# dgaddy/silent_speech

Measured on AMD Instinct MI355X. Metric: EMG frames/s training (transduction_model.py), higher is better.
Workload: dtype bf16

## Files before the change

include/silent_speech_hip.h:

```cpp
#ifndef SILENT_SPEECH_HIP_H
#define SILENT_SPEECH_HIP_H
#include <stdint.h>
#ifdef __cplusplus
extern "C" {
#endif

#define SS_F32 0
#define SS_BF16 1
#define SS_F32X3 3

const char* ss_last_error(void);
#define SS_ABI_VERSION 10
int ss_abi_version(void);
const char* ss_target_arch(void);

typedef struct ss_rowmap {
    int64_t base;
    int64_t batch_stride;
    int64_t row_stride;
    int32_t rows_per_batch;
} ss_rowmap;

typedef struct ss_gemm_epilogue {
    const float* bias;
    const void* gate;
    float gate_scale;
    float alpha;
    int32_t relu;
    float dropout_p;
    uint64_t seed;
    uint32_t rng_stream;
    int32_t mode;
    int32_t col_mod, col_mul, col_div_mul;
    float log_clamp;
    void* c2;
    ss_rowmap cmap2;
    int64_t col_stride2;
    float* col_sum;
    float* col_sumsq;
    const float* col_shift;
    void* planes_hi;
    void* planes_lo;
    int32_t planes_only;
    void* sign_out;
    int64_t sign_pitch;
    const void* gate_bits;
    int64_t gate_bits_pitch;
} ss_gemm_epilogue;

#define SS_OP_KC 0
#define SS_OP_OC 1

int ss_gemm(int dtype_in, int dtype_out, int a_mode, int b_mode, const void* A, const void* B, void* C,
            int M, int N, int K, const ss_rowmap* amap, const ss_rowmap* bmap, const ss_rowmap* cmap,
            const ss_gemm_epilogue* epilogue, int split_k, void* stream);

int ss_split_planes(const float* x, void* hi, void* lo, int64_t n, void* stream);
int ss_gemm_planes(int dtype_out, const void* A_hi, const void* A_lo, const void* B_hi, const void* B_lo, void* C, int M, int N, int K,
                   const ss_rowmap* amap, const ss_rowmap* bmap, const ss_rowmap* cmap, const ss_gemm_epilogue* epilogue, void* stream);
int ss_gemm_sign_bits_supported(int dtype_in, int dtype_out, int a_mode, int b_mode, const void* C, int M, int N, int K, const ss_rowmap* amap,
                                const ss_rowmap* bmap, const ss_rowmap* cmap, const ss_gemm_epilogue* epilogue, int split_k);
int ss_gemm_planes_supported(int dtype_out, const void* C, int M, int N, int K, const ss_rowmap* amap, const ss_rowmap* bmap, const ss_rowmap* cmap,
                             const ss_gemm_epilogue* epilogue);

int ss_gemm_set_blocks_per_cu(int n);
int ss_gemm_last_kernel(void);
int ss_gemm_fuses_column_stats(int dtype_in, int dtype_out, int a_mode, int b_mode, const void* C, int M, int N, int K, const ss_rowmap* amap,
                               const ss_rowmap* bmap, const ss_rowmap* cmap, const ss_gemm_epilogue* epilogue, int split_k);
int ss_gemm_set_option(int what, int value);

typedef struct ss_dw_job {
    const void* A;
    const void* B;
    float* C;
    ss_rowmap amap, bmap;
    int64_t ldc;
    int32_t M, N, K;
    int32_t flags;
} ss_dw_job;
int ss_gemm_dw_grouped(int n_jobs, const ss_dw_job* jobs , void* stream);
int ss_gemm_dw_set_option(int what, int value);

int ss_permute3d(const void* in, int in_dtype, void* out, int out_dtype, int d0, int d1, int d2,
                 int64_t s0, int64_t s1, int64_t s2, int valid1, int valid2, float scale, int accumulate,
                 void* stream);

int ss_permute3d_batch(const void* jobs_dev, const int32_t* job_of_block_dev, int total_blocks, int all_f32, void* stream);

int ss_dtw_source(int n, int m, int64_t stride_i, int64_t stride_j);
int64_t ss_dtw_workspace_bytes(int n, int m, int64_t* sk_bytes, int64_t* dirs_bytes, int64_t* bnd_bytes);
int ss_dtw_align(const float* costs, const int64_t* desc_dev, int n, int max_n, int max_m, void* workspace,
                 int32_t* results, void* stream);
int ss_dtw_align_skewed(const int64_t* desc_dev, int n, void* workspace, int32_t* results, void* stream);
int ss_dtw_cumulative(int dtype, const void* costs, int64_t stride_i, int64_t stride_j, int N, int M, void* dtw_out,
                      int32_t* results, void* stream);

int64_t ss_bn_scratch_floats(int B, int T, int C);
int ss_bn_stats_sums(int dtype, const void* x, int B, int T, int C, int pad, float* scratch, const float* shift, float* sums, void* stream);
int ss_bn_finalize(const float* sums, double n_total, int C, float* mean, float* invstd, float* running_mean, float* running_var,
                   float momentum, float eps, int training, void* stream);
int ss_bn_finalize_shift(const float* sums, const float* shift, double n_total, int C, float* mean, float* invstd, float* running_mean,
                         float* running_var, float momentum, float eps, int training, void* stream);
int ss_bn_apply(int dtype, const void* xa, const float* mean_a, const float* invstd_a, const float* gamma_a, const float* beta_a, int pad_xa,
                const void* xb, const float* mean_b, const float* invstd_b, const float* gamma_b, const float* beta_b, int pad_xb,
                void* y, int pad_y, int B, int T, int C, int relu, void* stream);
int ss_bn_backward_sums(int dtype, const void* dy, int pad_dy, const void* y, int pad_y,
                        const void* xa, int pad_xa, const float* mean_a, const float* invstd_a,
                        const void* xb, int pad_xb, const float* mean_b, const float* invstd_b,
                        float* dgamma_a, float* dbeta_a, float* dgamma_b, float* dbeta_b,
                        float* scratch, float* sums, int B, int T, int C, int relu,
                        const float* gate_gamma_a, const float* gate_beta_a, const float* gate_gamma_b, const float* gate_beta_b, void* stream);
int ss_bn_backward_apply(int dtype, const void* dy, int pad_dy, const void* y, int pad_y,
                         const void* xa, int pad_xa, const float* mean_a, const float* invstd_a, const float* gamma_a,
                         const void* xb, int pad_xb, const float* mean_b, const float* invstd_b, const float* gamma_b,
                         const float* sums, double n_total, void* dxa, int pad_dxa, void* dxb, int pad_dxb,
                         int B, int T, int C, int relu, const float* gate_beta_a, const float* gate_beta_b, void* stream);
int64_t ss_colsum_scratch_floats(int rows, int C);
int ss_colsum(int dtype, const void* x, int rows, int C, int64_t ld, float* scratch, float* out_accum, void* stream);

int ss_add_dropout_layernorm_forward(int dtype, const void* x, void* branch_inout, const float* gamma, const float* beta, void* y,
                                     float* mean, float* rstd, int rows, int C, float eps, float dropout_p, uint64_t seed,
                                     uint32_t rng_stream, void* stream);
int ss_layernorm_backward(int dtype, const void* dy, const void* z, const float* mean, const float* rstd, const float* gamma,
                          void* dres, void* dbranch, float* dgamma, float* dbeta, int rows, int C, float dropout_p, uint64_t seed,
                          uint32_t rng_stream, void* stream);

int ss_layernorm_backward_bias(int dtype, const void* dy, const void* z, const float* mean, const float* rstd, const float* gamma,
                               void* dres, void* dbranch, float* dgamma, float* dbeta, float* dbranch_colsum, int rows, int C, float dropout_p,
                               uint64_t seed, uint32_t rng_stream, void* stream);
int64_t ss_layernorm_backward_scratch_floats(int rows, int C);
int ss_layernorm_backward_ws(int dtype, const void* dy, const void* z, const float* mean, const float* rstd, const float* gamma,
                             void* dres, void* dbranch, float* dgamma, float* dbeta, float* dbranch_colsum, float* scratch, int64_t scratch_floats,
                             int rows, int C, float dropout_p, uint64_t seed, uint32_t rng_stream, void* stream);
int ss_add_dropout_layernorm_forward_planes(int dtype, const void* x, void* branch_inout, const float* gamma, const float* beta, void* y, void* y_hi, void* y_lo,
                                            float* mean, float* rstd, int rows, int C, float eps, float dropout_p, uint64_t seed, uint32_t rng_stream, void* stream);
int ss_layernorm_backward_ws_planes(int dtype, const void* dy, const void* z, const float* mean, const float* rstd, const float* gamma,
                                    void* dres, void* dbranch, void* dbranch_hi, void* dbranch_lo, float* dgamma, float* dbeta, float* dbranch_colsum, float* scratch,
                                    int64_t scratch_floats, int rows, int C, float dropout_p, uint64_t seed, uint32_t rng_stream, void* stream);

int ss_emg_prepare(int dtype, const float* x_raw, void* out_padded, float* shifted_copy, int B, int T0, int Cin, int shift, void* stream);

int ss_loss_index_tables(const int64_t* utt_dev, int n_utt, int32_t* vo_pred, int32_t* vo_tgt, int32_t* si_tgt, int32_t* si_base,
                         int32_t* si_res, void* stream);
int ss_frame_lse(const float* head, int64_t ld, int col0, int ncls, int rows, float* lse, int32_t* argmax, void* stream);
int ss_voiced_loss(const float* head, int64_t ld, int n_mel, int n_phone, const float* lse, const int32_t* argmax, const float* Y,
                   const int64_t* phones, const int32_t* pred_row, const int32_t* tgt_row, int nframes, float lam, float inv_total,
                   float* dhead, float* loss_accum, int32_t* correct_accum, void* stream);
int ss_silent_cost_skewed(const float* head, int64_t ld, int n_mel, const float* lse, const float* Y, const int64_t* phones,
                          const int64_t* desc_dev, int n, int max_n, int max_m, float lam, void* workspace, int32_t* results, void* stream);
int ss_silent_loss(const float* head, int64_t ld, int n_mel, int n_phone, const float* lse, const int32_t* argmax, const float* Y,
                   const int64_t* phones, const int32_t* results, const int32_t* tgt_row, const int32_t* pred_base,
                   const int32_t* res_idx, int nframes, float lam, float inv_total, float* dhead, float* loss_accum,
                   int32_t* correct_accum, void* stream);
int ss_phoneme_confusion(const int32_t* argmax, const int64_t* phones, const int32_t* results, const int32_t* vo_pred, const int32_t* vo_tgt,
                         int n_voiced, const int32_t* si_tgt, const int32_t* si_base, const int32_t* si_res, int n_silent_frames,
                         int32_t* confusion, int n_phone, void* stream);

int ss_ctc_loss(const float* logits, int64_t ld, int V, int blank, const float* lse, const int64_t* desc_dev, int n_utt, int max_target_len,
                int64_t rows, const int32_t* targets, float* alpha_ws, float* beta_ws, float* nll, float* dlogits, float* loss, void* stream);

int ss_adamw_step(float* p, const float* g, float* m, float* v, int64_t n, float lr, float beta1, float beta2, float eps,
                  float weight_decay, int step, float grad_scale, void* stream);
int ss_cast_f32(const float* in, void* out, int out_dtype, int64_t n, void* stream);
int ss_soft_clip(const float* x, float* out, int64_t n, int C, const float* mean, const float* stdv, float pre_div, float limit, void* stream);

int ss_concat_pad(const void* table_dev, int n, void* out, int64_t total_bytes, int granule, void* stream);

int ss_reflect_pad(const float* y, float* out, int B, int L, int pad, int64_t ld_out, void* stream);
int ss_reflect_pad_ragged(const float* y, const int64_t* offsets_dev, const int32_t* lengths_dev, float* out, int B, int min_len,
                          int pad, int64_t ld_out, int clip, void* stream);
int ss_stft_magnitude(const float* spec, int64_t ld_spec, int n_bins, float* mag, int64_t ld_mag, int rows, void* stream);
int ss_stft_logmel_fft(const float* y, const int64_t* offsets_dev, const int32_t* lengths_dev, int64_t uniform_len, int B, int F, int pad, int clip,
                       int n_fft, int hop, const float* window,
                       const int32_t* band_lo, const int32_t* band_cnt, const int32_t* band_off, const float* band_w, const int32_t* lane_bands, int n_mels, int n_w,
                       float log_clamp, float* out, int64_t stride_b, int64_t stride_f, int64_t stride_m, void* stream);

int ss_relpos_attention_needs_transposed(int dtype, int T, int dp, int D);
int ss_relpos_attention_family(int dtype, int T, int dp, int D);
int64_t ss_relpos_attention_table_bytes(int H, int dp, int D);
int ss_relpos_attention_prepare_tables(const float* emb, void* tab, int H, int D, int dh, int dp, float scale, void* stream);
int ss_relpos_attention_forward(int dtype, const void* qkv, const void* qkvT, const void* E, const void* tab, void* out, float* lse,
                                int B, int H, int T, int Tp, int dp, int D, float scale, float dropout_p, uint64_t seed,
                                uint32_t rng_stream, void* stream);
int ss_relpos_attention_backward(int dtype, const void* qkv, const void* qkvT, const void* E, const void* ET, const void* tab, const void* out,
                                 const float* lse, const void* dO, const void* dOT, float* Dscratch, void* dqkv,
                                 int B, int H, int T, int Tp, int dp, int D, float scale, float dropout_p, uint64_t seed,
                                 uint32_t rng_stream, void* stream);

int64_t ss_relpos_attention_saved_bytes(int dtype, int B, int H, int T, int dp, int D);
int ss_relpos_attention_forward_p(int dtype, const void* qkv, const void* qkvT, const void* E, const void* tab, void* out, float* lse, void* pimg,
                                  int B, int H, int T, int Tp, int dp, int D, float scale, float dropout_p, uint64_t seed,
                                  uint32_t rng_stream, void* stream);
int ss_relpos_attention_backward_p(int dtype, const void* qkv, const void* qkvT, const void* E, const void* ET, const void* tab, const void* out,
                                   const float* lse, const void* dO, const void* dOT, float* Dscratch, void* dqkv, const void* pimg,
                                   int B, int H, int T, int Tp, int dp, int D, float scale, float dropout_p, uint64_t seed,
                                   uint32_t rng_stream, void* stream);

int ss_relpos_attention_x3_supported(int T, int dp, int D);
int64_t ss_relpos_attention_x3_saved_bytes(int B, int H, int T, int dp, int D);
int64_t ss_relpos_attention_x3_table_bytes(int H, int dp, int D);
int ss_relpos_attention_x3_prepare_tables(const float* emb, void* tab, int H, int D, int dh, int dp, float scale, void* stream);
int ss_relpos_attention_x3_forward(const void* qkv_hi, const void* qkv_lo, const void* tab, void* out_hi, void* out_lo, float* lse, void* pimg,
                                   int B, int H, int T, int dp, int D, float scale, float dropout_p, uint64_t seed, uint32_t rng_stream, void* stream);
int ss_relpos_attention_x3_backward(const void* qkv_hi, const void* qkv_lo, const void* tab, const void* out_hi, const void* out_lo, const void* dO_hi, const void* dO_lo,
                                    float* Dscratch, void* dqkv_hi, void* dqkv_lo, const void* pimg,
                                    int B, int H, int T, int dp, int D, float scale, float dropout_p, uint64_t seed, uint32_t rng_stream, void* stream);

int64_t ss_iir_filtfilt_workspace_bytes(int T, int C, int max_padlen);
int ss_iir_filtfilt(const double* x, double* y, int T, int C, int n_filt, const double* coef, void* workspace, int64_t workspace_bytes, void* stream);
int ss_linear_resample(const double* x, double* y, int T, int C, double old_freq, double new_freq, int T_out, void* stream);
int64_t ss_iir_filtfilt_batch_workspace_bytes(const int32_t* lengths_host, int R, int C, int max_padlen, int n_filt);
int ss_iir_filtfilt_batch(const double* x, double* y, const int32_t* lengths_host, int R, int C, int n_filt, const double* coef,
                          void* workspace, int64_t workspace_bytes, void* stream);
int ss_linear_resample_batch(const double* x, double* y, const int64_t* table_dev, int R, int C, double old_freq, double new_freq,
                             int64_t total_out_rows, void* stream);
int ss_emg_features_batch(const double* x, float* out, const int64_t* table_dev, int R, int C, int64_t total_frames, void* stream);

typedef struct ss_model_dims {
    int32_t d_model, n_layers, n_head, d_qkv, dp , max_rel , ff;
    int32_t n_head_cols , dtype;
    float ln_eps;
} ss_model_dims;
typedef struct ss_plan ss_plan;
typedef double (*ss_reduce_hook)(void* user, float* sums_dev, int n_floats, double n_local, void* stream);
typedef void (*ss_event_hook)(void* user, int what, void* stream);
ss_plan* ss_plan_create(const ss_model_dims* dims);
void ss_plan_destroy(ss_plan* plan);
int ss_plan_slot_count(const ss_plan* plan);
const char* ss_plan_slot_name(const ss_plan* plan, int slot);
int ss_plan_bind(ss_plan* plan, int slot, void* device_ptr_or_value);
int ss_plan_set_option(ss_plan* plan, int what, int value);
int ss_plan_set_reduce_hook(ss_plan* plan, ss_reduce_hook fn, void* user);
int ss_plan_set_event_hook(ss_plan* plan, ss_event_hook fn, void* user);
int64_t ss_plan_ctx_bytes(void);
int64_t ss_plan_workspace_bytes(ss_plan* plan, int B, int T0, int training);
int ss_plan_forward(ss_plan* plan, const float* x_raw, float* shifted_scratch, void* workspace, int64_t workspace_bytes, int B, int T0,
                    int training, int shift_r, float dropout_p, uint64_t seed, float* head, void* ctx_out, void* stream);
int ss_plan_backward(ss_plan* plan, void* ctx, const float* dhead, void* stream, void* side_stream);
typedef struct ss_profile_row { char name[64]; int64_t calls; double seconds, flops , bytes ; } ss_profile_row;
int ss_plan_profile(ss_plan* plan, int enable);
int ss_plan_profile_read(ss_plan* plan, ss_profile_row* rows, int max_rows);
int ss_counters_add(int n, int64_t** counters , int64_t delta, void* stream);

#ifdef __cplusplus
}
#endif
#endif
```

silent_speech_amd/_lib.py:

```python
import ctypes
import os

import torch

_HERE = os.path.dirname(os.path.abspath(__file__))
_LIB_PATH = os.environ.get('SS_AMD_LIBRARY') or os.path.join(_HERE, 'lib', 'libsilent_speech_hip.so')

SS_F32, SS_BF16, SS_F64, SS_F32X3 = 0, 1, 2, 3
ABI_VERSION = 10
OP_KC, OP_OC = 0, 1


class RowMap(ctypes.Structure):
    _fields_ = [('base', ctypes.c_int64), ('batch_stride', ctypes.c_int64), ('row_stride', ctypes.c_int64),
                ('rows_per_batch', ctypes.c_int32)]


class GemmEpilogue(ctypes.Structure):
    _fields_ = [('bias', ctypes.c_void_p), ('gate', ctypes.c_void_p), ('gate_scale', ctypes.c_float),
                ('alpha', ctypes.c_float), ('relu', ctypes.c_int32), ('dropout_p', ctypes.c_float),
                ('seed', ctypes.c_uint64), ('rng_stream', ctypes.c_uint32), ('mode', ctypes.c_int32),
                ('col_mod', ctypes.c_int32), ('col_mul', ctypes.c_int32), ('col_div_mul', ctypes.c_int32),
                ('log_clamp', ctypes.c_float), ('c2', ctypes.c_void_p), ('cmap2', RowMap), ('col_stride2', ctypes.c_int64),
                ('col_sum', ctypes.c_void_p), ('col_sumsq', ctypes.c_void_p), ('col_shift', ctypes.c_void_p),
                ('planes_hi', ctypes.c_void_p), ('planes_lo', ctypes.c_void_p), ('planes_only', ctypes.c_int32),
                ('sign_out', ctypes.c_void_p), ('sign_pitch', ctypes.c_int64), ('gate_bits', ctypes.c_void_p), ('gate_bits_pitch', ctypes.c_int64)]


class DwJob(ctypes.Structure):
    _fields_ = [('A', ctypes.c_void_p), ('B', ctypes.c_void_p), ('C', ctypes.c_void_p), ('amap', RowMap), ('bmap', RowMap),
                ('ldc', ctypes.c_int64), ('M', ctypes.c_int32), ('N', ctypes.c_int32), ('K', ctypes.c_int32), ('flags', ctypes.c_int32)]


class ProfileRow(ctypes.Structure):
    _fields_ = [('name', ctypes.c_char * 64), ('calls', ctypes.c_int64), ('seconds', ctypes.c_double), ('flops', ctypes.c_double), ('bytes', ctypes.c_double)]


class PermuteJob(ctypes.Structure):
    _fields_ = [('inp', ctypes.c_void_p), ('out', ctypes.c_void_p), ('s0', ctypes.c_int64), ('s1', ctypes.c_int64), ('s2', ctypes.c_int64),
                ('o0', ctypes.c_int64), ('o1', ctypes.c_int64), ('d0', ctypes.c_int32), ('d1', ctypes.c_int32), ('d2', ctypes.c_int32),
                ('valid1', ctypes.c_int32), ('valid2', ctypes.c_int32), ('in_dtype', ctypes.c_int32), ('out_dtype', ctypes.c_int32),
                ('accumulate', ctypes.c_int32), ('scale', ctypes.c_float), ('first_block', ctypes.c_int32), ('nblocks', ctypes.c_int32),
                ('pad_', ctypes.c_int32)]


_P, _I, _F, _L = ctypes.c_void_p, ctypes.c_int, ctypes.c_float, ctypes.c_int64
_U64, _U32 = ctypes.c_uint64, ctypes.c_uint32

SIGNATURES = {
    'ss_gemm': [_I, _I, _I, _I, _P, _P, _P, _I, _I, _I, ctypes.POINTER(RowMap), ctypes.POINTER(RowMap),
                ctypes.POINTER(RowMap), ctypes.POINTER(GemmEpilogue), _I, _P],
    'ss_gemm_dw_grouped': [_I, ctypes.POINTER(DwJob), _P],
    'ss_split_planes': [_P, _P, _P, _L, _P],
    'ss_gemm_planes': [_I, _P, _P, _P, _P, _P, _I, _I, _I, ctypes.POINTER(RowMap), ctypes.POINTER(RowMap), ctypes.POINTER(RowMap), ctypes.POINTER(GemmEpilogue), _P],
    'ss_permute3d': [_P, _I, _P, _I, _I, _I, _I, _L, _L, _L, _I, _I, _F, _I, _P],
    'ss_permute3d_batch': [_P, _P, _I, _I, _P],
    'ss_dtw_align': [_P, _P, _I, _I, _I, _P, _P, _P],
    'ss_dtw_align_skewed': [_P, _I, _P, _P, _P],
    'ss_reflect_pad_ragged': [_P, _P, _P, _P, _I, _I, _I, _L, _I, _P],
    'ss_concat_pad': [_P, _I, _P, _L, _I, _P],
    'ss_dtw_cumulative': [_I, _P, _L, _L, _I, _I, _P, _P, _P],
    'ss_relpos_attention_forward': [_I, _P, _P, _P, _P, _P, _P, _I, _I, _I, _I, _I, _I, _F, _F, _U64, _U32, _P],
    'ss_relpos_attention_backward': [_I, _P, _P, _P, _P, _P, _P, _P, _P, _P, _P, _P, _I, _I, _I, _I, _I, _I, _F, _F, _U64, _U32, _P],
    'ss_relpos_attention_forward_p': [_I, _P, _P, _P, _P, _P, _P, _P, _I, _I, _I, _I, _I, _I, _F, _F, _U64, _U32, _P],
    'ss_relpos_attention_backward_p': [_I, _P, _P, _P, _P, _P, _P, _P, _P, _P, _P, _P, _P, _I, _I, _I, _I, _I, _I, _F, _F, _U64, _U32, _P],
    'ss_relpos_attention_prepare_tables': [_P, _P, _I, _I, _I, _I, _F, _P],
    'ss_relpos_attention_x3_prepare_tables': [_P, _P, _I, _I, _I, _I, _F, _P],
    'ss_relpos_attention_x3_forward': [_P, _P, _P, _P, _P, _P, _P, _I, _I, _I, _I, _I, _F, _F, _U64, _U32, _P],
    'ss_relpos_attention_x3_backward': [_P, _P, _P, _P, _P, _P, _P, _P, _P, _P, _P, _I, _I, _I, _I, _I, _F, _F, _U64, _U32, _P],
    'ss_bn_stats_sums': [_I, _P, _I, _I, _I, _I, _P, _P, _P, _P],
    'ss_bn_finalize': [_P, ctypes.c_double, _I, _P, _P, _P, _P, _F, _F, _I, _P],
    'ss_bn_finalize_shift': [_P, _P, ctypes.c_double, _I, _P, _P, _P, _P, _F, _F, _I, _P],
    'ss_bn_apply': [_I, _P, _P, _P, _P, _P, _I, _P, _P, _P, _P, _P, _I, _P, _I, _I, _I, _I, _I, _P],
    'ss_bn_backward_sums': [_I, _P, _I, _P, _I, _P, _I, _P, _P, _P, _I, _P, _P, _P, _P, _P, _P, _P, _P, _I, _I, _I, _I, _P, _P, _P, _P, _P],
    'ss_bn_backward_apply': [_I, _P, _I, _P, _I, _P, _I, _P, _P, _P, _P, _I, _P, _P, _P, _P, ctypes.c_double, _P, _I, _P, _I, _I, _I, _I, _I, _P, _P, _P],
    'ss_colsum': [_I, _P, _I, _I, _L, _P, _P, _P],
    'ss_add_dropout_layernorm_forward': [_I, _P, _P, _P, _P, _P, _P, _P, _I, _I, _F, _F, _U64, _U32, _P],
    'ss_add_dropout_layernorm_forward_planes': [_I, _P, _P, _P, _P, _P, _P, _P, _P, _P, _I, _I, _F, _F, _U64, _U32, _P],
    'ss_layernorm_backward': [_I, _P, _P, _P, _P, _P, _P, _P, _P, _P, _I, _I, _F, _U64, _U32, _P],
    'ss_layernorm_backward_bias': [_I, _P, _P, _P, _P, _P, _P, _P, _P, _P, _P, _I, _I, _F, _U64, _U32, _P],
    'ss_layernorm_backward_ws': [_I, _P, _P, _P, _P, _P, _P, _P, _P, _P, _P, _P, _L, _I, _I, _F, _U64, _U32, _P],
    'ss_layernorm_backward_ws_planes': [_I, _P, _P, _P, _P, _P, _P, _P, _P, _P, _P, _P, _P, _P, _L, _I, _I, _F, _U64, _U32, _P],
    'ss_emg_prepare': [_I, _P, _P, _P, _I, _I, _I, _I, _P],
    'ss_frame_lse': [_P, _L, _I, _I, _I, _P, _P, _P],
    'ss_loss_index_tables': [_P, _I, _P, _P, _P, _P, _P, _P],
    'ss_voiced_loss': [_P, _L, _I, _I, _P, _P, _P, _P, _P, _P, _I, _F, _F, _P, _P, _P, _P],
    'ss_silent_cost_skewed': [_P, _L, _I, _P, _P, _P, _P, _I, _I, _I, _F, _P, _P, _P],
    'ss_silent_loss': [_P, _L, _I, _I, _P, _P, _P, _P, _P, _P, _P, _P, _I, _F, _F, _P, _P, _P, _P],
    'ss_phoneme_confusion': [_P, _P, _P, _P, _P, _I, _P, _P, _P, _I, _P, _I, _P],
    'ss_ctc_loss': [_P, _L, _I, _I, _P, _P, _I, _I, _L, _P, _P, _P, _P, _P, _P, _P],
    'ss_adamw_step': [_P, _P, _P, _P, _L, _F, _F, _F, _F, _F, _I, _F, _P],
    'ss_cast_f32': [_P, _P, _I, _L, _P],
    'ss_soft_clip': [_P, _P, _L, _I, _P, _P, _F, _F, _P],
    'ss_reflect_pad': [_P, _P, _I, _I, _I, _L, _P],
    'ss_iir_filtfilt': [_P, _P, _I, _I, _I, _P, _P, _L, _P],
    'ss_linear_resample': [_P, _P, _I, _I, ctypes.c_double, ctypes.c_double, _I, _P],
    'ss_iir_filtfilt_batch': [_P, _P, _P, _I, _I, _I, _P, _P, _L, _P],
    'ss_linear_resample_batch': [_P, _P, _P, _I, _I, ctypes.c_double, ctypes.c_double, _L, _P],
    'ss_emg_features_batch': [_P, _P, _P, _I, _I, _L, _P],
    'ss_stft_magnitude': [_P, _L, _I, _P, _L, _I, _P],
    'ss_stft_logmel_fft': [_P, _P, _P, _L, _I, _I, _I, _I, _I, _I, _P, _P, _P, _P, _P, _P, _I, _I, _F, _P, _L, _L, _L, _P],
}
_LP = ctypes.POINTER(ctypes.c_int64)
_HOST_FUNCS = {'ss_dtw_workspace_bytes': ([_I, _I, _LP, _LP, _LP], ctypes.c_int64),
               'ss_dtw_source': ([_I, _I, _L, _L], ctypes.c_int),
               'ss_bn_scratch_floats': ([_I, _I, _I], ctypes.c_int64),
               'ss_iir_filtfilt_workspace_bytes': ([_I, _I, _I], ctypes.c_int64),
               'ss_iir_filtfilt_batch_workspace_bytes': ([_P, _I, _I, _I, _I], ctypes.c_int64),
               'ss_colsum_scratch_floats': ([_I, _I], ctypes.c_int64),
               'ss_gemm_set_blocks_per_cu': ([_I], ctypes.c_int),
               'ss_gemm_last_kernel': ([], ctypes.c_int),
               'ss_gemm_set_option': ([_I, _I], ctypes.c_int),
               'ss_gemm_fuses_column_stats': ([_I, _I, _I, _I, _P, _I, _I, _I, ctypes.POINTER(RowMap), ctypes.POINTER(RowMap), ctypes.POINTER(RowMap),
                                               ctypes.POINTER(GemmEpilogue), _I], ctypes.c_int),
               'ss_gemm_sign_bits_supported': ([_I, _I, _I, _I, _P, _I, _I, _I, ctypes.POINTER(RowMap), ctypes.POINTER(RowMap), ctypes.POINTER(RowMap),
                                                ctypes.POINTER(GemmEpilogue), _I], ctypes.c_int),
               'ss_gemm_planes_supported': ([_I, _P, _I, _I, _I, ctypes.POINTER(RowMap), ctypes.POINTER(RowMap), ctypes.POINTER(RowMap), ctypes.POINTER(GemmEpilogue)], ctypes.c_int),
               'ss_gemm_dw_set_option': ([_I, _I], ctypes.c_int),
               'ss_plan_create': ([_P], _P), 'ss_plan_destroy': ([_P], None), 'ss_plan_slot_count': ([_P], ctypes.c_int),
               'ss_plan_slot_name': ([_P, _I], ctypes.c_char_p), 'ss_plan_bind': ([_P, _I, _P], ctypes.c_int),
               'ss_plan_set_option': ([_P, _I, _I], ctypes.c_int), 'ss_plan_set_reduce_hook': ([_P, _P, _P], ctypes.c_int),
               'ss_plan_set_event_hook': ([_P, _P, _P], ctypes.c_int), 'ss_plan_ctx_bytes': ([], ctypes.c_int64),
               'ss_plan_workspace_bytes': ([_P, _I, _I, _I], ctypes.c_int64),
               'ss_plan_forward': ([_P, _P, _P, _P, _L, _I, _I, _I, _I, _F, _U64, _P, _P, _P], ctypes.c_int),
               'ss_plan_backward': ([_P, _P, _P, _P, _P], ctypes.c_int),
               'ss_counters_add': ([_I, _P, _L, _P], ctypes.c_int),
               'ss_plan_profile': ([_P, _I], ctypes.c_int), 'ss_plan_profile_read': ([_P, _P, _I], ctypes.c_int),
               'ss_relpos_attention_needs_transposed': ([_I, _I, _I, _I], ctypes.c_int),
               'ss_relpos_attention_family': ([_I, _I, _I, _I], ctypes.c_int),
               'ss_relpos_attention_table_bytes': ([_I, _I, _I], ctypes.c_int64),
               'ss_relpos_attention_x3_supported': ([_I, _I, _I], ctypes.c_int),
               'ss_relpos_attention_x3_saved_bytes': ([_I, _I, _I, _I, _I], ctypes.c_int64),
               'ss_relpos_attention_x3_table_bytes': ([_I, _I, _I], ctypes.c_int64),
               'ss_relpos_attention_saved_bytes': ([_I, _I, _I, _I, _I, _I], ctypes.c_int64),
               'ss_layernorm_backward_scratch_floats': ([_I, _I], ctypes.c_int64)}
_RESTYPES = {'ss_last_error': ctypes.c_char_p, 'ss_target_arch': ctypes.c_char_p, 'ss_abi_version': ctypes.c_int}

_lib = None
_is_emulator = False


def _declare(lib):
    for name, restype in _RESTYPES.items():
        fn = getattr(lib, name)
        fn.restype = restype
        fn.argtypes = []
    for name, argtypes in SIGNATURES.items():
        fn = getattr(lib, name)
        fn.argtypes = argtypes
        fn.restype = ctypes.c_int
    for name, (argtypes, restype) in _HOST_FUNCS.items():
        fn = getattr(lib, name)
        fn.argtypes = argtypes
        fn.restype = restype
    return lib


def load(path=None, _testing=False):
    global _lib, _is_emulator
    path = path or _LIB_PATH
    if not os.path.exists(path):
        raise RuntimeError('silent_speech_amd: %s not found -- build the gfx950 kernels first '
                           '(python -c "import __graft_entry__ as g; g.build()" or make -C silent_speech_amd/csrc). '
                           'There is no CPU fallback.' % path)
    cdll = ctypes.CDLL(path)
    cdll.ss_abi_version.restype = ctypes.c_int
    have = cdll.ss_abi_version()
    if have != ABI_VERSION:
        raise RuntimeError('silent_speech_amd: %s has ABI version %d, this binding needs %d -- rebuild it '
                           '(make -C silent_speech_amd/csrc); struct layouts differ between versions' % (path, have, ABI_VERSION))
    cdll.ss_target_arch.restype = ctypes.c_char_p
    arch = cdll.ss_target_arch()
    if arch != b'gfx950' and not _testing:
        raise RuntimeError('silent_speech_amd: %s targets %r, not gfx950 -- the package only loads the MI355X build '
                           '(SS_AMD_LIBRARY selects between gfx950 builds; the emulator library is for tests/ only)' % (path, arch))
    _lib = _declare(cdll)
    _is_emulator = arch != b'gfx950'
    return _lib


def use_library_for_testing(path):
    return load(path, _testing=True)


def lib():
    if _lib is None:
        load()
    return _lib


def is_emulator():
    lib()
    return _is_emulator


def kernels_can_read(t):
    return bool(t.is_cuda) != is_emulator()


def kernel_device_for(t):
    return t.device if kernels_can_read(t) else torch.device('cuda')


def check(rc, what=''):
    if rc != 0:
        raise RuntimeError('%s failed: %s' % (what or 'silent_speech_hip call', lib().ss_last_error().decode()))


def dtype_code(dt):
    if dt == torch.float32:
        return SS_F32
    if dt == torch.bfloat16:
        return SS_BF16
    if dt == torch.float64:
        return SS_F64
    raise TypeError('unsupported dtype %s (float32, bfloat16; float64 for ss_dtw_cumulative only)' % dt)


def ptr(t):
    if t is None:
        return None
    if not kernels_can_read(t):
        if is_emulator():
            raise RuntimeError('emulator backend (tests only) needs CPU tensors')
        raise RuntimeError('silent_speech_amd: tensor is on %s; the HIP kernels need an AMD GPU tensor '
                           '(no CPU fallback exists)' % t.device)
# ... 8 lines not shown
```

silent_speech_amd/csrc/norm.hip:

```cpp
#include "common.h"
#include <stdlib.h>
#include "silent_speech_hip.h"

namespace {
struct Seq {
    int T, pad;
    __device__ __forceinline__ long long row(int r) const { int b = r / T, t = r - b * T; return (long long)b * (T + 2 * pad) + pad + t; }
    __device__ __forceinline__ long long at(int b, int t) const { return (long long)b * (T + 2 * pad) + pad + t; }
};

__device__ __forceinline__ void ld8(const float* __restrict__ p, float (&v)[8]) {
    const f32x4 a = *(const f32x4*)p, b = *(const f32x4*)(p + 4);
    v[0] = a[0]; v[1] = a[1]; v[2] = a[2]; v[3] = a[3]; v[4] = b[0]; v[5] = b[1]; v[6] = b[2]; v[7] = b[3];
}

struct ColMap {
    int CV, CVb, RY, cx0, ry; bool active;
    __device__ __forceinline__ ColMap(int C, int tid, int nthreads) {
        CV = C >> 3; CVb = CV < nthreads ? CV : nthreads; RY = nthreads / CVb;
        cx0 = tid % CVb; ry = tid / CVb; active = ry < RY;
    }
};
constexpr int RED_THREADS = 256;

template <int NQ>
__device__ __forceinline__ bool chunk_reduce(const float* __restrict__ partial, int nchunks, int C, float (&out)[NQ], int& c_out)
{
    __shared__ float red[NQ][8][32];
    const int cl = threadIdx.x & 31, ln = threadIdx.x >> 5, c = blockIdx.x * 32 + cl;
    float acc[NQ];
#pragma unroll
    for (int q = 0; q < NQ; ++q) acc[q] = 0.f;
    if (c < C) {
        int k = ln;
        for (; k + 56 < nchunks; k += 64) {
            float v[8][NQ];
#pragma unroll
            for (int u = 0; u < 8; ++u)
#pragma unroll
                for (int q = 0; q < NQ; ++q) v[u][q] = partial[((long long)(k + 8 * u) * NQ + q) * C + c];
#pragma unroll
            for (int u = 0; u < 8; ++u)
#pragma unroll
                for (int q = 0; q < NQ; ++q) acc[q] += v[u][q];
        }
        for (; k < nchunks; k += 8)
#pragma unroll
            for (int q = 0; q < NQ; ++q) acc[q] += partial[((long long)k * NQ + q) * C + c];
    }
#pragma unroll
    for (int q = 0; q < NQ; ++q) red[q][ln][cl] = acc[q];
    __syncthreads();
    c_out = c;
    if (ln != 0 || c >= C) return false;
#pragma unroll
    for (int q = 0; q < NQ; ++q) { float t = 0.f; for (int y = 0; y < 8; ++y) t += red[q][y][cl]; out[q] = t; }
    return true;
}
}

template <class T>
__global__ __launch_bounds__(RED_THREADS) void bn_partial_kernel(const T* __restrict__ x, Seq sx, int rows, int C, int rows_per_chunk, const float* __restrict__ shift, float* __restrict__ partial)
{
    __shared__ float red[2][RED_THREADS * 8];
    ColMap m(C, threadIdx.x, (int)blockDim.x);
    const int r0 = blockIdx.x * rows_per_chunk, r1 = min(rows, r0 + rows_per_chunk);
    for (int cb = 0; cb < m.CV; cb += m.CVb) {
        const int cx = cb + m.cx0;
        float s1[8], s2[8], sh[8];
#pragma unroll
        for (int e = 0; e < 8; ++e) { s1[e] = 0.f; s2[e] = 0.f; sh[e] = 0.f; }
        const bool cv = m.active && cx < m.CV;
        if (cv) {
            if (shift) {
#pragma unroll
                for (int e = 0; e < 8; ++e) sh[e] = shift[cx * 8 + e];
            } else Vec8<T>::load(x + sx.row(0) * C + cx * 8, sh);
            int r = r0 + m.ry;
            for (; r + 3 * m.RY < r1; r += 4 * m.RY) {
                float v[4][8];
#pragma unroll
                for (int u = 0; u < 4; ++u) Vec8<T>::load(x + sx.row(r + u * m.RY) * C + cx * 8, v[u]);
#pragma unroll
                for (int u = 0; u < 4; ++u)
#pragma unroll
                    for (int e = 0; e < 8; ++e) { float d = v[u][e] - sh[e]; s1[e] += d; s2[e] += d * d; }
            }
            for (; r < r1; r += m.RY) {
                float v[8]; Vec8<T>::load(x + sx.row(r) * C + cx * 8, v);
#pragma unroll
                for (int e = 0; e < 8; ++e) { float d = v[e] - sh[e]; s1[e] += d; s2[e] += d * d; }
            }
        }
        __syncthreads();
#pragma unroll
        for (int e = 0; e < 8; ++e) { red[0][threadIdx.x * 8 + e] = s1[e]; red[1][threadIdx.x * 8 + e] = s2[e]; }
        __syncthreads();
        if (cv && m.ry == 0) {
            for (int y = 1; y < m.RY; ++y)
#pragma unroll
                for (int e = 0; e < 8; ++e) { s1[e] += red[0][(y * m.CVb + m.cx0) * 8 + e]; s2[e] += red[1][(y * m.CVb + m.cx0) * 8 + e]; }
#pragma unroll
            for (int e = 0; e < 8; ++e) {
                partial[((long long)blockIdx.x * 2 + 0) * C + cx * 8 + e] = s1[e];
                partial[((long long)blockIdx.x * 2 + 1) * C + cx * 8 + e] = s2[e];
            }
        }
    }
}

template <class T>
__global__ __launch_bounds__(256) void bn_sums_kernel(const T* __restrict__ x, Seq sx, const float* __restrict__ partial, int nchunks, int C, const float* __restrict__ shift, float* __restrict__ sums)
{
    float t[2]; int c;
    if (!chunk_reduce<2>(partial, nchunks, C, t, c)) return;
    sums[c] = t[0]; sums[C + c] = t[1]; sums[2 * C + c] = shift ? shift[c] : ldf(x + sx.row(0) * C + c);
}

__global__ void bn_finalize_kernel(const float* __restrict__ sums, const float* shift, float n, int C, float* mean, float* invstd, float* running_mean, float* running_var,
                                   float momentum, float eps, int training)
{
    const int c = blockIdx.x * blockDim.x + threadIdx.x;
    if (c >= C) return;
    if (!training) { mean[c] = running_mean[c]; invstd[c] = rsqrtf(running_var[c] + eps); return; }
    const float d = sums[c] / n, mu = (shift ? shift[c] : sums[2 * C + c]) + d;
    float var = sums[C + c] / n - d * d; var = var < 0.f ? 0.f : var;
    mean[c] = mu; invstd[c] = rsqrtf(var + eps);
    if (running_mean) {
        running_mean[c] = (1.f - momentum) * running_mean[c] + momentum * mu;
        running_var[c] = (1.f - momentum) * running_var[c] + momentum * var * (n > 1.f ? n / (n - 1.f) : 1.f);
    }
}

static int red_threads(int C) {
    static const int forced = getenv("SS_BN_RED_THREADS") ? atoi(getenv("SS_BN_RED_THREADS")) : 0;
    if (forced > 0) return forced < RED_THREADS ? forced : RED_THREADS;
    const int cv = C >> 3;
    if (cv >= RED_THREADS || cv <= 0) return RED_THREADS;
    const int t = RED_THREADS / cv * cv;
    return t >= 64 ? t : RED_THREADS;
}
static int red_chunks(int rows) { static const int cap = getenv("SS_BN_CHUNKS") ? atoi(getenv("SS_BN_CHUNKS")) : 768; int c = (rows + 63) / 64; if (c > cap) c = cap; if (c < 1) c = 1; return c; }

extern "C" int64_t ss_bn_scratch_floats(int B, int T, int C) { return (int64_t)red_chunks(B * T) * 4 * C + 8 * (int64_t)C; }

extern "C" int ss_bn_stats_sums(int dtype, const void* x, int B, int T, int C, int pad, float* scratch, const float* shift, float* sums, void* stream)
{
    SS_CHECK(x && scratch && sums, "ss_bn_stats_sums: null pointer");
    SS_CHECK(C % 8 == 0 && C > 0, "ss_bn_stats_sums: C=%d must be a positive multiple of 8", C);
    SS_CHECK(B > 0 && T > 0, "ss_bn_stats_sums: empty batch");
    const int rows = B * T, nch = red_chunks(rows), rpc = (rows + nch - 1) / nch;
    Seq sx = {T, pad};
    if (dtype == SS_BF16) {
        SS_LAUNCH(bn_partial_kernel<bf16_t>, dim3(nch), dim3(red_threads(C)), 0, stream, (const bf16_t*)x, sx, rows, C, rpc, shift, scratch);
        SS_LAUNCH(bn_sums_kernel<bf16_t>, dim3((C + 31) / 32), dim3(256), 0, stream, (const bf16_t*)x, sx, (const float*)scratch, nch, C, shift, sums);
    } else {
        SS_LAUNCH(bn_partial_kernel<float>, dim3(nch), dim3(red_threads(C)), 0, stream, (const float*)x, sx, rows, C, rpc, shift, scratch);
        SS_LAUNCH(bn_sums_kernel<float>, dim3((C + 31) / 32), dim3(256), 0, stream, (const float*)x, sx, (const float*)scratch, nch, C, shift, sums);
    }
    SS_LAUNCH_CHECK("ss_bn_stats_sums");
    return 0;
}

extern "C" int ss_bn_finalize(const float* sums, double n_total, int C, float* mean, float* invstd, float* running_mean, float* running_var,
                              float momentum, float eps, int training, void* stream)
{
    SS_CHECK(mean && invstd && C > 0, "ss_bn_finalize: null pointer");
    SS_CHECK(training ? (sums != nullptr && n_total >= 1.0) : (running_mean && running_var), "ss_bn_finalize: missing sums (training) or running statistics (eval)");
    SS_LAUNCH(bn_finalize_kernel, dim3((C + 255) / 256), dim3(256), 0, stream, sums, (const float*)nullptr, (float)n_total, C, mean, invstd, running_mean, running_var, momentum, eps, training);
    SS_LAUNCH_CHECK("ss_bn_finalize");
    return 0;
}
extern "C" int ss_bn_finalize_shift(const float* sums, const float* shift, double n_total, int C, float* mean, float* invstd, float* running_mean, float* running_var,
                                    float momentum, float eps, int training, void* stream)
{
    SS_CHECK(mean && invstd && C > 0, "ss_bn_finalize_shift: null pointer");
    SS_CHECK(training ? (sums != nullptr && shift != nullptr && n_total >= 1.0) : (running_mean && running_var), "ss_bn_finalize_shift: missing sums / shift (training) or running statistics (eval)");
    SS_LAUNCH(bn_finalize_kernel, dim3((C + 255) / 256), dim3(256), 0, stream, sums, shift, (float)n_total, C, mean, invstd, running_mean, running_var, momentum, eps, training);
    SS_LAUNCH_CHECK("ss_bn_finalize_shift");
    return 0;
}

struct RowWalk {
    unsigned ro, b, tp, rstep, db, dtp, TP; int cx;
    __device__ __forceinline__ RowWalk(unsigned gtid, unsigned step, unsigned CV, unsigned TP_) {
        TP = TP_; ro = gtid / CV; cx = (int)(gtid - ro * CV); rstep = step / CV;
        b = ro / TP; tp = ro - b * TP; db = rstep / TP; dtp = rstep - db * TP;
    }
    __device__ __forceinline__ void next() { ro += rstep; b += db; tp += dtp; if (tp >= TP) { tp -= TP; ++b; } }
};

template <class T>
__global__ void bn_apply_kernel(const T* __restrict__ xa, Seq sa, const float* __restrict__ mean_a, const float* __restrict__ invstd_a, const float* __restrict__ gamma_a, const float* __restrict__ beta_a,
                                const T* __restrict__ xb, Seq sb, const float* __restrict__ mean_b, const float* __restrict__ invstd_b, const float* __restrict__ gamma_b, const float* __restrict__ beta_b,
                                T* __restrict__ y, Seq sy, int B, int C, int relu)
{
    const int CV = C >> 3, TT = sy.T;
    const unsigned TP = (unsigned)(TT + 2 * sy.pad), rows_out = (unsigned)B * TP, step32 = gridDim.x * blockDim.x;
    if (step32 % (unsigned)CV == 0) {
        RowWalk w(blockIdx.x * blockDim.x + threadIdx.x, step32, (unsigned)CV, TP);
        float ma[8], sca[8], ba[8], mb[8], scb[8], bb[8];
#pragma unroll
        for (int e = 0; e < 8; ++e) { mb[e] = 0.f; scb[e] = 0.f; bb[e] = 0.f; }
        {
            float t[8];
            ld8(mean_a + w.cx * 8, ma); ld8(gamma_a + w.cx * 8, sca); ld8(invstd_a + w.cx * 8, t); ld8(beta_a + w.cx * 8, ba);
#pragma unroll
            for (int e = 0; e < 8; ++e) sca[e] *= t[e];
            if (xb) {
                ld8(mean_b + w.cx * 8, mb); ld8(gamma_b + w.cx * 8, scb); ld8(invstd_b + w.cx * 8, t); ld8(beta_b + w.cx * 8, bb);
#pragma unroll
                for (int e = 0; e < 8; ++e) scb[e] *= t[e];
            }
        }
        typedef typename RawVec8<T>::type Raw;
        Raw nv = RawVec8<T>::zero(), nu = RawVec8<T>::zero();
        auto fetch = [&](unsigned b, unsigned tp) {
            const int t = (int)tp - sy.pad;
            if (t >= 0 && t < TT) {
                nv = RawVec8<T>::load(xa + sa.at((int)b, t) * C + w.cx * 8);
                if (xb) nu = RawVec8<T>::load(xb + sb.at((int)b, t) * C + w.cx * 8);
            }
        };
        if (w.ro < rows_out) fetch(w.b, w.tp);
        for (; w.ro < rows_out; w.next()) {
            const int t = (int)w.tp - sy.pad;
            const Raw cv = nv, cu = nu;
            {
                unsigned nb = w.b + w.db, ntp = w.tp + w.dtp;
                if (ntp >= w.TP) { ntp -= w.TP; ++nb; }
                if (w.ro + w.rstep < rows_out) fetch(nb, ntp);
            }
            float o[8];
#pragma unroll
            for (int e = 0; e < 8; ++e) o[e] = 0.f;
            if (t >= 0 && t < TT) {
                float v[8], u[8];
                RawVec8<T>::unpack(cv, v);
                if (xb) RawVec8<T>::unpack(cu, u);
#pragma unroll
                for (int e = 0; e < 8; ++e) o[e] = (v[e] - ma[e]) * sca[e] + ba[e];
                if (xb) {
#pragma unroll
                    for (int e = 0; e < 8; ++e) o[e] += (u[e] - mb[e]) * scb[e] + bb[e];
                }
                if (relu) {
#pragma unroll
                    for (int e = 0; e < 8; ++e) o[e] = fmaxf(o[e], 0.f);
                }
            }
            Vec8<T>::store(y + (long long)w.ro * C + w.cx * 8, o);
        }
        return;
    }
    const unsigned total32 = rows_out * (unsigned)CV;
    for (unsigned i = blockIdx.x * blockDim.x + threadIdx.x; i < total32; i += step32) {
        const unsigned ro = i / (unsigned)CV; const int cx = (int)(i - ro * (unsigned)CV);
        const unsigned bq = ro / TP; const int b = (int)bq, tp = (int)(ro - bq * TP), t = tp - sy.pad;
        float o[8];
        if (t < 0 || t >= TT) {
#pragma unroll
            for (int e = 0; e < 8; ++e) o[e] = 0.f;
        } else {
            float v[8]; Vec8<T>::load(xa + sa.at(b, t) * C + cx * 8, v);
#pragma unroll
            for (int e = 0; e < 8; ++e) { const int c = cx * 8 + e; const float s = gamma_a[c] * invstd_a[c]; o[e] = (v[e] - mean_a[c]) * s + beta_a[c]; }
            if (xb) {
                float u[8]; Vec8<T>::load(xb + sb.at(b, t) * C + cx * 8, u);
#pragma unroll
                for (int e = 0; e < 8; ++e) { const int c = cx * 8 + e; const float s = gamma_b[c] * invstd_b[c]; o[e] += (u[e] - mean_b[c]) * s + beta_b[c]; }
            }
            if (relu) {
#pragma unroll
                for (int e = 0; e < 8; ++e) o[e] = fmaxf(o[e], 0.f);
            }
        }
        Vec8<T>::store(y + (long long)ro * C + cx * 8, o);
    }
}

static dim3 ew_grid(long long total, int block, int CV = 0) {
    static const long long cap_cols = getenv("SS_BN_GRID") ? atoll(getenv("SS_BN_GRID")) : 768;
    long long g = (total + block - 1) / block;
    const long long cap = CV > 0 ? cap_cols : 8192;
    if (g > cap) g = cap;
    if (g < 1) g = 1;
    if (CV > 0) {
        long long a = CV, bb = block; while (bb) { const long long t = a % bb; a = bb; bb = t; }
        const long long m = CV / a;
        if (g >= 4 * m) g = g / m * m;
    }
    return dim3((unsigned)g);
}

extern "C" int ss_bn_apply(int dtype, const void* xa, const float* mean_a, const float* invstd_a, const float* gamma_a, const float* beta_a, int pad_xa,
                           const void* xb, const float* mean_b, const float* invstd_b, const float* gamma_b, const float* beta_b, int pad_xb,
                           void* y, int pad_y, int B, int T, int C, int relu, void* stream)
{
    SS_CHECK(xa && mean_a && invstd_a && gamma_a && beta_a && y, "ss_bn_apply: null pointer");
    SS_CHECK(!xb || (mean_b && invstd_b && gamma_b && beta_b), "ss_bn_apply: second branch incomplete");
    SS_CHECK(C % 8 == 0 && C > 0 && B > 0 && T > 0, "ss_bn_apply: bad shape B=%d T=%d C=%d", B, T, C);
    Seq sa = {T, pad_xa}, sb = {T, pad_xb}, sy = {T, pad_y};
    const long long total = (long long)B * (T + 2 * pad_y) * (C / 8);
    SS_CHECK(total < (1LL << 31) - (1LL << 22), "ss_bn_apply: tensor too large for 32-bit chunk indices");
    if (dtype == SS_BF16) SS_LAUNCH(bn_apply_kernel<bf16_t>, ew_grid(total, 256, C / 8), dim3(256), 0, stream, (const bf16_t*)xa, sa, mean_a, invstd_a, gamma_a, beta_a, (const bf16_t*)xb, sb, mean_b, invstd_b, gamma_b, beta_b, (bf16_t*)y, sy, B, C, relu);
    else SS_LAUNCH(bn_apply_kernel<float>, ew_grid(total, 256, C / 8), dim3(256), 0, stream, (const float*)xa, sa, mean_a, invstd_a, gamma_a, beta_a, (const float*)xb, sb, mean_b, invstd_b, gamma_b, beta_b, (float*)y, sy, B, C, relu);
    SS_LAUNCH_CHECK("ss_bn_apply");
    return 0;
}

template <class T, bool REGATE>
__global__ __launch_bounds__(RED_THREADS, sizeof(T) == 2 ? 3 : 2) void bn_bwd_partial_kernel(const T* __restrict__ dy, Seq sdy, const T* __restrict__ y, Seq sy,
                                                                     const T* __restrict__ xa, Seq sa, const float* __restrict__ mean_a, const float* __restrict__ invstd_a,
                                                                     const T* __restrict__ xb, Seq sb, const float* __restrict__ mean_b, const float* __restrict__ invstd_b,
                                                                     const float* __restrict__ gamma_a, const float* __restrict__ beta_a, const float* __restrict__ gamma_b, const float* __restrict__ beta_b,
                                                                     int rows, int C, int rows_per_chunk, int relu, float* __restrict__ partial)
{
    __shared__ float red[3][RED_THREADS * 8];
    ColMap m(C, threadIdx.x, (int)blockDim.x);
    const int r0 = blockIdx.x * rows_per_chunk, r1 = min(rows, r0 + rows_per_chunk);
    for (int cb = 0; cb < m.CV; cb += m.CVb) {
        const int cx = cb + m.cx0;
        float sg[8], sga[8], sgb[8], ma[8], ka[8], mb[8], kb[8], bs[8];
#pragma unroll
        for (int e = 0; e < 8; ++e) { sg[e] = sga[e] = sgb[e] = 0.f; ma[e] = ka[e] = mb[e] = kb[e] = bs[e] = 0.f; }
        const bool cv = m.active && cx < m.CV;
        if (cv) {
            {
                float t0[8], t1[8], t2[8], t3[8];
                ld8(mean_a + cx * 8, ma); ld8(invstd_a + cx * 8, ka);
                ld8((xb ? mean_b : mean_a) + cx * 8, mb); ld8((xb ? invstd_b : invstd_a) + cx * 8, kb);
                if (REGATE) {
                    ld8(gamma_a + cx * 8, t0); ld8(beta_a + cx * 8, t1); ld8((xb ? gamma_b : gamma_a) + cx * 8, t2); ld8((xb ? beta_b : beta_a) + cx * 8, t3);
#pragma unroll
                    for (int e = 0; e < 8; ++e) { ka[e] *= t0[e]; kb[e] *= t2[e]; bs[e] = t1[e] + (xb ? t3[e] : 0.f); }
                }
                if (!xb) {
#pragma unroll
                    for (int e = 0; e < 8; ++e) { mb[e] = 0.f; kb[e] = 0.f; }
                }
            }
            typedef typename RawVec8<T>::type Raw;
            Raw ng[2], no[2], na[2], nb[2];
            auto fetch = [&](int r, Raw (&fg)[2], Raw (&fo)[2], Raw (&fa)[2], Raw (&fb)[2]) {
                const int rc0 = r < r1 ? r : r1 - 1, rc1 = r + m.RY < r1 ? r + m.RY : r1 - 1;
                const int b0 = rc0 / sdy.T, t0 = rc0 - b0 * sdy.T, b1 = rc1 / sdy.T, t1 = rc1 - b1 * sdy.T;
                fg[0] = RawVec8<T>::load(dy + sdy.at(b0, t0) * C + cx * 8); fg[1] = RawVec8<T>::load(dy + sdy.at(b1, t1) * C + cx * 8);
                if (relu && !REGATE) { fo[0] = RawVec8<T>::load(y + sy.at(b0, t0) * C + cx * 8); fo[1] = RawVec8<T>::load(y + sy.at(b1, t1) * C + cx * 8); }
                fa[0] = RawVec8<T>::load(xa + sa.at(b0, t0) * C + cx * 8); fa[1] = RawVec8<T>::load(xa + sa.at(b1, t1) * C + cx * 8);
                if (xb) { fb[0] = RawVec8<T>::load(xb + sb.at(b0, t0) * C + cx * 8); fb[1] = RawVec8<T>::load(xb + sb.at(b1, t1) * C + cx * 8); }
            };
            if (r0 + m.ry < r1) fetch(r0 + m.ry, ng, no, na, nb);
            for (int r = r0 + m.ry; r < r1; r += 2 * m.RY) {
                const bool two = r + m.RY < r1;
                Raw cg[2] = {ng[0], ng[1]}, co[2] = {no[0], no[1]}, ca[2] = {na[0], na[1]}, cb[2] = {nb[0], nb[1]};
                if (r + 2 * m.RY < r1) fetch(r + 2 * m.RY, ng, no, na, nb);
#pragma unroll
                for (int u = 0; u < 2; ++u) {
                    if (u == 1 && !two) break;
                    float g[8], o[8], va[8], vb[8];
                    RawVec8<T>::unpack(cg[u], g); RawVec8<T>::unpack(ca[u], va);
                    if (relu && !REGATE) RawVec8<T>::unpack(co[u], o);
                    if (xb) RawVec8<T>::unpack(cb[u], vb);
#pragma unroll
                    for (int e = 0; e < 8; ++e) {
                        if (REGATE) {
                            const float da = va[e] - ma[e], db = xb ? vb[e] - mb[e] : 0.f;
                            const float gg = (!relu || da * ka[e] + db * kb[e] + bs[e] > 0.f) ? g[e] : 0.f;
                            sg[e] += gg; sga[e] += gg * da;
                            if (xb) sgb[e] += gg * db;
                        } else {
                            const float gg = (!relu || o[e] > 0.f) ? g[e] : 0.f;
                            sg[e] += gg; sga[e] += gg * (va[e] - ma[e]) * ka[e];
                            if (xb) sgb[e] += gg * (vb[e] - mb[e]) * kb[e];
                        }
                    }
                }
            }
            if (REGATE) {
                float ia[8], ib[8];
                ld8(invstd_a + cx * 8, ia); ld8((xb ? invstd_b : invstd_a) + cx * 8, ib);
#pragma unroll
                for (int e = 0; e < 8; ++e) { sga[e] *= ia[e]; sgb[e] *= ib[e]; }
            }
        }
        __syncthreads();
#pragma unroll
        for (int e = 0; e < 8; ++e) { red[0][threadIdx.x * 8 + e] = sg[e]; red[1][threadIdx.x * 8 + e] = sga[e]; red[2][threadIdx.x * 8 + e] = sgb[e]; }
        __syncthreads();
        if (cv && m.ry == 0) {
            for (int yy = 1; yy < m.RY; ++yy)
#pragma unroll
                for (int e = 0; e < 8; ++e) { const int o = (yy * m.CVb + m.cx0) * 8 + e; sg[e] += red[0][o]; sga[e] += red[1][o]; sgb[e] += red[2][o]; }
            Vec8<float>::store(partial + ((long long)blockIdx.x * 3 + 0) * C + cx * 8, sg);
            Vec8<float>::store(partial + ((long long)blockIdx.x * 3 + 1) * C + cx * 8, sga);
            Vec8<float>::store(partial + ((long long)blockIdx.x * 3 + 2) * C + cx * 8, sgb);
        }
    }
}

__global__ __launch_bounds__(256) void bn_bwd_finalize_kernel(const float* __restrict__ partial, int nchunks, int C, float* __restrict__ coef ,
                                                              float* dgamma_a, float* dbeta_a, float* dgamma_b, float* dbeta_b)
{
    float t[3]; int c;
    if (!chunk_reduce<3>(partial, nchunks, C, t, c)) return;
    coef[c] = t[0]; coef[C + c] = t[1]; coef[2 * C + c] = t[2];
    if (dgamma_a) dgamma_a[c] += t[1];
    if (dbeta_a) dbeta_a[c] += t[0];
    if (dgamma_b) dgamma_b[c] += t[2];
    if (dbeta_b) dbeta_b[c] += t[0];
}

template <class T, bool REGATE>
__global__ void bn_bwd_apply_kernel(const T* __restrict__ dy, Seq sdy, const T* __restrict__ y, Seq sy,
                                    const T* __restrict__ xa, Seq sa, const float* __restrict__ mean_a, const float* __restrict__ invstd_a, const float* __restrict__ gamma_a,
                                    const T* __restrict__ xb, Seq sb, const float* __restrict__ mean_b, const float* __restrict__ invstd_b, const float* __restrict__ gamma_b,
                                    const float* __restrict__ coef, float inv_n, T* __restrict__ dxa, Seq sda, T* __restrict__ dxb, Seq sdb, int B, int C, int relu,
                                    const float* __restrict__ beta_a, const float* __restrict__ beta_b)
{
    constexpr bool regate = REGATE;
    const int CV = C >> 3, TT = sdy.T;
    const int padmax = sda.pad > sdb.pad ? sda.pad : sdb.pad;
    const long long total = (long long)B * (TT + 2 * padmax) * CV;
    const unsigned TP = (unsigned)(TT + 2 * padmax), total32 = (unsigned)total, step32 = gridDim.x * blockDim.x;
    if (step32 % (unsigned)CV == 0) {
        RowWalk w(blockIdx.x * blockDim.x + threadIdx.x, step32, (unsigned)CV, TP);
        float ma[8], ka[8], qa[8], c0[8], mb[8], kb[8], qb[8], bs[8];
#pragma unroll
        for (int e = 0; e < 8; ++e) { mb[e] = 0.f; kb[e] = 0.f; qb[e] = 0.f; bs[e] = 0.f; }
        {
            float ia[8], t[8];
            ld8(mean_a + w.cx * 8, ma); ld8(gamma_a + w.cx * 8, ka); ld8(invstd_a + w.cx * 8, ia); ld8(coef + C + w.cx * 8, qa); ld8(coef + w.cx * 8, c0);
            if (regate) ld8(beta_a + w.cx * 8, bs);
#pragma unroll
            for (int e = 0; e < 8; ++e) { ka[e] *= ia[e]; qa[e] = ia[e] * (qa[e] * inv_n); c0[e] *= inv_n; }
            if (xb) {
                ld8(mean_b + w.cx * 8, mb); ld8(gamma_b + w.cx * 8, kb); ld8(invstd_b + w.cx * 8, ia); ld8(coef + 2 * C + w.cx * 8, qb);
#pragma unroll
                for (int e = 0; e < 8; ++e) { kb[e] *= ia[e]; qb[e] = ia[e] * (qb[e] * inv_n); }
                if (regate) {
                    ld8(beta_b + w.cx * 8, t);
#pragma unroll
                    for (int e = 0; e < 8; ++e) bs[e] += t[e];
                }
            }
        }
        const unsigned rows_out = (unsigned)B * TP;
        for (; w.ro < rows_out; w.next()) {
            const int b = (int)w.b, t = (int)w.tp - padmax, cx = w.cx;
            float oa[8], ob[8];
#pragma unroll
            for (int e = 0; e < 8; ++e) { oa[e] = 0.f; ob[e] = 0.f; }
            if (t >= 0 && t < TT) {
                float g[8], o[8], v[8], u[8];
                Vec8<T>::load(dy + sdy.at(b, t) * C + cx * 8, g);
                if (relu && !regate) Vec8<T>::load(y + sy.at(b, t) * C + cx * 8, o);
                Vec8<T>::load(xa + sa.at(b, t) * C + cx * 8, v);
                if (xb) Vec8<T>::load(xb + sb.at(b, t) * C + cx * 8, u);
                if (regate) {
#pragma unroll
// ... 635 lines not shown
```

silent_speech_amd/csrc/plan.hip:

```cpp
#include "common.h"
#include "silent_speech_hip.h"
#include <math.h>
#include <stdlib.h>
#include <string>
#include <vector>

namespace {

struct BnP { float *gamma = 0, *beta = 0, *rmean = 0, *rvar = 0, *dgamma = 0, *dbeta = 0; long long* nbt = 0; };
struct PermB { void* jobs = 0; void* blocks = 0; long long total = 0, all_f32 = 0; };
struct BlockP {
    void *w1f = 0, *w2f = 0, *wr = 0, *wrT = 0, *w2b = 0, *w1b_even = 0, *w1b_odd = 0;
    float *b1 = 0, *br = 0, *b2 = 0;
    BnP bn1, bn2, bnr;
    float *c2_stage = 0, *c1_stage = 0, *wr_grad = 0;
    PermB unpack;
    int O = 0, I = 0;
};
struct LayerP {
    void *wqkv = 0, *wqkvT = 0, *wo = 0, *woT = 0, *E = 0, *ET = 0, *EF = 0, *w1 = 0, *w2 = 0, *w1T = 0, *w2T = 0;
    float *b1 = 0, *b2 = 0, *g1 = 0, *be1 = 0, *g2 = 0, *be2 = 0;
    float *dg1 = 0, *dbe1 = 0, *dg2 = 0, *dbe2 = 0, *dw1 = 0, *db1 = 0, *dw2 = 0, *db2 = 0, *wo_stage = 0, *wqkv_stage = 0;
    PermB unpack;
};

struct BlockCtx { void *xin, *c1, *cr, *h1, *c2, *y; float *m1, *i1, *m2, *i2, *mr, *ir, *scratch; int Tin, Cin, Tout, O, pad_y; };
struct LayerCtx { void *x, *qkv, *qkvT, *o, *z1, *y1, *hid, *z2, *pimg; float *lse, *mean1, *rstd1, *mean2, *rstd2; unsigned char* hid_sign; };
constexpr int MAX_LAYERS = 16;
constexpr int MAX_PLANES = 384;
struct PlaneCache { int n; const void* key[MAX_PLANES]; void* hi[MAX_PLANES]; long long elems[MAX_PLANES]; };
struct Ctx {
    int B, T0, T, M, Tp, need_T, n_layers;
    float p_drop, scale; unsigned long long seed;
    BlockCtx blk[3];
    LayerCtx layer[MAX_LAYERS];
    void *conv_out, *x_final;
    PlaneCache planes;
    unsigned long long ws_used;
    char* ws; unsigned long long ws_bytes;
};

struct Exec {
    bool dry; char* base; size_t off, cap; void* stream; void* side;
    void* alloc(size_t bytes) { off = (off + 255) & ~(size_t)255; char* p = base + off; off += bytes; return p; }
};

static ss_rowmap RM(long long row_stride, int rows_per_batch = 0, long long batch_stride = 0, long long base = 0) {
    ss_rowmap m; m.base = base; m.batch_stride = batch_stride; m.row_stride = row_stride; m.rows_per_batch = rows_per_batch; return m;
}
static ss_gemm_epilogue EPI() { ss_gemm_epilogue e; memset(&e, 0, sizeof(e)); e.alpha = 1.f; e.gate_scale = 1.f; return e; }
static int round_up(int x, int m) { return (x + m - 1) / m * m; }

typedef double (*reduce_fn)(void* user, float* sums, int n_floats, double n_local, void* stream);
typedef void (*event_fn)(void* user, int what, void* stream);

struct Plan {
    ss_model_dims D;
    std::vector<std::string> names; std::vector<void**> targets;
    BlockP blk[3]; std::vector<LayerP> layers;
    void *w_raw_in = 0, *w_raw_in_T = 0, *w_head = 0, *w_head_T = 0;
    float *b_raw_in = 0, *dw_raw_in = 0, *db_raw_in = 0, *b_head = 0, *head_w_stage = 0, *head_b_stage = 0, *stage_arena = 0;
    long long stage_arena_bytes = 0;
    PermB unpack_enc, unpack_all;
    reduce_fn hook = 0; void* hook_user = 0;
    event_fn on_event = 0; void* event_user = 0;
    int side_enabled = 1, dw_grouped = 1, side_blocks = 2, fuse_stats = 1, regate_on = 1, f32_x3 = 0;
    int x3_attn = 0;
    int sign_gate = 1;
    int x3_emit = 1;
    int x3_planes = 1;
    Ctx* cur = nullptr;
    bool use_planes() const { return D.dtype == SS_F32 && f32_x3 && x3_planes; }
    bool use_x3_attention(int T) const { return use_planes() && x3_attn && dw_grouped && ss_relpos_attention_x3_supported(T, D.dp, D.max_rel); }
    void adopt_planes(const void* key, void* hi, long long n) {
        PlaneCache& pc = cur->planes;
        if (key && pc.n < MAX_PLANES) { pc.key[pc.n] = key; pc.hi[pc.n] = hi; pc.elems[pc.n] = n; ++pc.n; }
    }
    int keep_input = 0;
    hipEvent_t ev_fork = 0, ev_join = 0;
    size_t esz() const { return D.dtype == SS_BF16 ? 2 : 4; }

    struct ProfRec { const char* tag; int sub; double flops, bytes; hipEvent_t e0, e1; };
    bool profiling = false;
    std::vector<ProfRec> recs; std::vector<hipEvent_t> ev_pool; size_t ev_used = 0;
    hipEvent_t prof_event() {
#if !defined(SS_EMU)
        if (ev_used == ev_pool.size()) { hipEvent_t e; hipEventCreate(&e); ev_pool.push_back(e); }
        return ev_pool[ev_used++];
#else
        return 0;
#endif
    }
    template <class F>
    int timed(Exec& X, const char* tag, double flops, double bytes, void* stream, F&& f, bool gemm_sub = false) {
        if (X.dry) return f();
#if !defined(SS_EMU)
        if (profiling) {
            ProfRec r{tag, 0, flops, bytes, prof_event(), prof_event()};
            hipEventRecord(r.e0, (hipStream_t)stream);
            const int rc = f();
            hipEventRecord(r.e1, (hipStream_t)stream);
            if (gemm_sub) r.sub = ss_gemm_last_kernel();
            recs.push_back(r);
            return rc;
        }
#endif
        return f();
    }

    void slot(const std::string& n, void** t) { names.push_back(n); targets.push_back(t); }
    void slot_bn(const std::string& p, BnP& b) {
        slot(p + ".weight", (void**)&b.gamma); slot(p + ".bias", (void**)&b.beta); slot(p + ".running_mean", (void**)&b.rmean); slot(p + ".running_var", (void**)&b.rvar);
        slot(p + ".weight.grad", (void**)&b.dgamma); slot(p + ".bias.grad", (void**)&b.dbeta); slot(p + ".num_batches_tracked", (void**)&b.nbt);
    }
    void slot_perm(const std::string& p, PermB& b) { slot(p + ".jobs", &b.jobs); slot(p + ".blocks", &b.blocks); slot(p + ".total", (void**)&b.total); slot(p + ".all_f32", (void**)&b.all_f32); }

    explicit Plan(const ss_model_dims& d) : D(d), layers(d.n_layers) {
        for (int i = 0; i < 3; ++i) {
            const std::string p = "conv_blocks." + std::to_string(i) + ".";
            BlockP& b = blk[i];
            b.O = D.d_model; b.I = i == 0 ? 8 : D.d_model;
            slot(p + "w1f", &b.w1f); slot(p + "w2f", &b.w2f); slot(p + "wr", &b.wr); slot(p + "wrT", &b.wrT); slot(p + "w2b", &b.w2b);
            if (i > 0) { slot(p + "w1b_even", &b.w1b_even); slot(p + "w1b_odd", &b.w1b_odd); }
            slot(p + "conv1.bias", (void**)&b.b1); slot(p + "residual_path.bias", (void**)&b.br); slot(p + "conv2.bias", (void**)&b.b2);
            slot_bn(p + "bn1", b.bn1); slot_bn(p + "bn2", b.bn2); slot_bn(p + "res_norm", b.bnr);
            slot(p + "conv2.weight.stage", (void**)&b.c2_stage); slot(p + "conv1.weight.stage", (void**)&b.c1_stage); slot(p + "residual_path.weight.grad", (void**)&b.wr_grad);
            slot_perm(p + "unpack", b.unpack);
        }
        slot("w_raw_in", &w_raw_in); slot("w_raw_in_T", &w_raw_in_T); slot("w_raw_in.bias", (void**)&b_raw_in);
        slot("w_raw_in.weight.grad", (void**)&dw_raw_in); slot("w_raw_in.bias.grad", (void**)&db_raw_in);
        for (int l = 0; l < D.n_layers; ++l) {
            const std::string p = "transformer.layers." + std::to_string(l) + ".";
            LayerP& L = layers[l];
            slot(p + "wqkv", &L.wqkv); slot(p + "wqkvT", &L.wqkvT); slot(p + "wo", &L.wo); slot(p + "woT", &L.woT); slot(p + "E", &L.E); slot(p + "ET", &L.ET); slot(p + "EF", &L.EF);
            slot(p + "w1", &L.w1); slot(p + "w2", &L.w2); slot(p + "w1T", &L.w1T); slot(p + "w2T", &L.w2T);
            slot(p + "linear1.bias", (void**)&L.b1); slot(p + "linear2.bias", (void**)&L.b2);
            slot(p + "norm1.weight", (void**)&L.g1); slot(p + "norm1.bias", (void**)&L.be1); slot(p + "norm2.weight", (void**)&L.g2); slot(p + "norm2.bias", (void**)&L.be2);
            slot(p + "norm1.weight.grad", (void**)&L.dg1); slot(p + "norm1.bias.grad", (void**)&L.dbe1); slot(p + "norm2.weight.grad", (void**)&L.dg2); slot(p + "norm2.bias.grad", (void**)&L.dbe2);
            slot(p + "linear1.weight.grad", (void**)&L.dw1); slot(p + "linear1.bias.grad", (void**)&L.db1); slot(p + "linear2.weight.grad", (void**)&L.dw2); slot(p + "linear2.bias.grad", (void**)&L.db2);
            slot(p + "w_o.stage", (void**)&L.wo_stage); slot(p + "w_qkv.stage", (void**)&L.wqkv_stage);
            slot_perm(p + "unpack", L.unpack);
        }
        slot("w_head", &w_head); slot("w_head_T", &w_head_T); slot("b_head", (void**)&b_head);
        slot("head_w.stage", (void**)&head_w_stage); slot("head_b.stage", (void**)&head_b_stage);
        slot("stage_arena", (void**)&stage_arena); slot("stage_arena.bytes", (void**)&stage_arena_bytes);
        slot_perm("unpack_encoder", unpack_enc); slot_perm("unpack_encoder_all", unpack_all);
    }

    static long long extent(const ss_rowmap& m, int rows, int row_len) {
        const long long nb = m.rows_per_batch > 0 ? (rows - 1) / m.rows_per_batch : 0, rr = m.rows_per_batch > 0 ? (rows < m.rows_per_batch ? rows : m.rows_per_batch) - 1 : rows - 1;
        return m.base + nb * m.batch_stride + rr * m.row_stride + row_len;
    }
    struct Pl { void* hi; void* lo; };
    Pl new_planes(Exec& X, const void* key, long long n) {
        if (!(use_planes() && x3_emit)) return Pl{nullptr, nullptr};
        n = (n + 7) & ~7LL;
        void* hi = X.alloc((size_t)n * 4);
        adopt_planes(key, hi, n);
        return Pl{hi, (char*)hi + n * 2};
    }
    Pl planes(Exec& X, const void* key, const void* src, long long n) {
        PlaneCache& pc = cur->planes;
        if (key) for (int i = 0; i < pc.n; ++i) if (pc.key[i] == key && pc.elems[i] >= n) return Pl{pc.hi[i], (char*)pc.hi[i] + pc.elems[i] * 2};
        n = (n + 7) & ~7LL;
        void* hi = X.alloc((size_t)n * 4);
        if (key && pc.n < MAX_PLANES) { pc.key[pc.n] = key; pc.hi[pc.n] = hi; pc.elems[pc.n] = n; ++pc.n; }
        if (!X.dry) {
            if (timed(X, "split_planes", 0, (double)n * 8, X.stream, [&] { return ss_split_planes((const float*)src, hi, (char*)hi + n * 2, n, X.stream); })) return Pl{nullptr, nullptr};
        }
        return Pl{hi, (char*)hi + n * 2};
    }

    int gemm(Exec& X, int dt_out, const void* A, const void* B, void* C, int M, int N, int K, ss_rowmap am, ss_rowmap bm, ss_rowmap cm, const ss_gemm_epilogue* e = 0,
             int a_mode = SS_OP_KC, int b_mode = SS_OP_KC, int split = 1, void* stream = 0, const void* wkey = nullptr, int emit = 0) {
        void* st = stream ? stream : X.stream;
        if (use_planes() && st == X.stream && a_mode == SS_OP_KC && b_mode == SS_OP_KC && dt_out == SS_F32 && split == 1 &&
            ss_gemm_planes_supported(SS_F32, C, M, N, K, &am, &bm, &cm, e)) {
            const Pl a = planes(X, A, A, extent(am, M, K)), b = planes(X, wkey ? wkey : B, B, extent(bm, N, K));
            ss_gemm_epilogue ee = e ? *e : EPI();
            if (emit && x3_emit) {
                const long long n = (extent(cm, M, N) + 7) & ~7LL;
                void* hi = X.alloc((size_t)n * 4);
                adopt_planes(C, hi, n);
                ee.planes_hi = hi; ee.planes_lo = (char*)hi + n * 2; ee.planes_only = emit == 2;
            }
            if (X.dry) return 0;
            if (!a.hi || !b.hi) return 1;
            return timed(X, "gemm", 2.0 * M * N * K, ((double)M * K + (double)N * K) * 4 + (double)M * N * 4.0, st,
                         [&] { return ss_gemm_planes(SS_F32, a.hi, a.lo, b.hi, b.lo, C, M, N, K, &am, &bm, &cm, &ee, st); }, true);
        }
        if (X.dry) return 0;
        const double ob = dt_out == SS_BF16 ? 2.0 : 4.0;
        return timed(X, a_mode == SS_OP_OC && b_mode == SS_OP_OC ? "gemm_dw" : "gemm", 2.0 * M * N * K, ((double)M * K + (double)N * K) * esz() + (double)M * N * ob, st,
                     [&] { return ss_gemm(D.dtype == SS_F32 && f32_x3 ? SS_F32X3 : D.dtype, dt_out, a_mode, b_mode, A, B, C, M, N, K, &am, &bm, &cm, e, split, st); }, true);
    }
    int colsum(Exec& X, const void* x, int rows, int C, float* out, void* stream) {
        float* scratch = (float*)X.alloc((size_t)ss_colsum_scratch_floats(rows, C) * 4);
        if (X.dry) return 0;
        return timed(X, "colsum", 0, (double)rows * C * esz(), stream, [&] { return ss_colsum(D.dtype, x, rows, C, C, scratch, out, stream); });
    }
    int permute_batch(Exec& X, const PermB& b, void* stream) {
        if (X.dry || !b.jobs || b.total <= 0) return 0;
        return timed(X, "grad_unlayout", 0, 0, stream, [&] { return ss_permute3d_batch(b.jobs, (const int32_t*)b.blocks, (int)b.total, (int)b.all_f32, stream); });
    }
    int bn_stats(Exec& X, const void* x, int B, int T, int C, float* scratch, BnP& bn, bool training, float** mean, float** invstd, float* fused = nullptr, double reduced_n = 0.0) {
        *mean = (float*)X.alloc((size_t)C * 4); *invstd = (float*)X.alloc((size_t)C * 4);
        float* sums = (training && !fused) ? (float*)X.alloc((size_t)3 * C * 4) : fused;
        if (X.dry) return 0;
        double n_total = (double)B * T;
        if (training) {
            if (!fused && timed(X, "bn_stats", 0, (double)B * T * C * esz(), X.stream, [&] { return ss_bn_stats_sums(D.dtype, x, B, T, C, 0, scratch, hook ? bn.rmean : nullptr, sums, X.stream); })) return 1;
            if (reduced_n > 0.0) n_total = reduced_n;
            else if (hook) n_total = hook(hook_user, sums, 2 * C, n_total, X.stream);
        }
        if (fused) return timed(X, "bn_finalize", 0, 0, X.stream, [&] { return ss_bn_finalize_shift(sums, bn.rmean, n_total, C, *mean, *invstd, bn.rmean, bn.rvar, 0.1f, 1e-5f, 1, X.stream); });
        return timed(X, "bn_finalize", 0, 0, X.stream, [&] { return ss_bn_finalize(sums, n_total, C, *mean, *invstd, bn.rmean, bn.rvar, 0.1f, 1e-5f, training ? 1 : 0, X.stream); });
    }
    float* conv_gemm(Exec& X, const void* A, const void* Bw, void* C, int M, int N, int K, ss_rowmap am, ss_rowmap bm, const float* bias, BnP& bn, float* stat_slot, int* rc) {
        ss_gemm_epilogue e = EPI(); e.bias = bias;
        ss_rowmap cm = RM(N);
        float* fused = nullptr;
        if (!X.dry && stat_slot && fuse_stats) {
            ss_gemm_epilogue es = e; es.col_sum = stat_slot; es.col_sumsq = stat_slot + N; es.col_shift = bn.rmean;
            const bool ok = use_planes() ? ss_gemm_planes_supported(SS_F32, C, M, N, K, &am, &bm, &cm, &es) != 0
                                         : ss_gemm_fuses_column_stats(D.dtype, D.dtype, SS_OP_KC, SS_OP_KC, C, M, N, K, &am, &bm, &cm, &e, 1) != 0;
            if (ok) { fused = stat_slot; e = es; }
        }
        *rc = gemm(X, D.dtype, A, Bw, C, M, N, K, am, bm, cm, &e);
        return fused;
    }
    void fork(Exec& X) {
#if !defined(SS_EMU)
        if (X.dry || !X.side || X.side == X.stream) return;
        hipEventRecord(ev_fork, (hipStream_t)X.stream); hipStreamWaitEvent((hipStream_t)X.side, ev_fork, 0);
#endif
    }
    void join(Exec& X) {
#if !defined(SS_EMU)
        if (X.dry || !X.side || X.side == X.stream) return;
        hipEventRecord(ev_join, (hipStream_t)X.side); hipStreamWaitEvent((hipStream_t)X.stream, ev_join, 0);
#endif
    }
    int split_k(int M, int N, int K, bool overlapped) const {
        const int tiles = ((M + 127) / 128) * ((N + 127) / 128);
        int s = (overlapped ? 400 : 512) / (tiles > 0 ? tiles : 1); s = s < 1 ? 1 : (s > 64 ? 64 : s);
        const int cap = K >= 512 ? K / 512 : 1;
        return s < cap ? s : (cap < 1 ? 1 : cap);
    }

    struct DwGroup {
        Plan* P; Exec* X; bool grouped; int n = 0; ss_dw_job jobs[24];
        int add(const void* dy, const void* x, float* grad, int N, int K, int rows, ss_rowmap am, ss_rowmap bm, void* stream) {
            if (grouped && P->use_planes()) {
                if (n + 3 > 24 && launch(stream)) return 1;
                const Pl a = P->planes(*X, dy, dy, extent(am, rows, N)), b = P->planes(*X, x, x, extent(bm, rows, K));
                if (X->dry) return 0;
                if (!a.hi || !b.hi) return 1;
                const void* as[3] = {a.lo, a.hi, a.hi}; const void* bs[3] = {b.hi, b.lo, b.hi};
                for (int t = 0; t < 3; ++t) {
                    ss_dw_job& j = jobs[n++]; memset(&j, 0, sizeof(j));
                    j.A = as[t]; j.B = bs[t]; j.C = grad; j.amap = am; j.bmap = bm; j.ldc = K; j.M = N; j.N = K; j.K = rows; j.flags = 1;
                }
                return 0;
            }
            if (grouped) {
                if (n == 8 && launch(stream)) return 1;
                ss_dw_job& j = jobs[n++]; memset(&j, 0, sizeof(j));
                j.A = dy; j.B = x; j.C = grad; j.amap = am; j.bmap = bm; j.ldc = K; j.M = N; j.N = K; j.K = rows;
                return 0;
            }
            ss_gemm_epilogue e = EPI(); e.mode = 2;
            const bool ov = X->side && X->side != X->stream;
            P->fork(*X);
            if (ov) ss_gemm_set_blocks_per_cu(P->side_blocks);
            const int rc = P->gemm(*X, SS_F32, dy, x, grad, N, K, rows, am, bm, RM(K), &e, SS_OP_OC, SS_OP_OC, P->split_k(N, K, rows, ov), stream);
            if (ov) ss_gemm_set_blocks_per_cu(2);
            return rc;
        }
        int launch(void* stream) {
            int rc = 0;
            if (n && !X->dry) {
                double fl = 0, by = 0;
                const double pl = P->use_planes() ? 3.0 : 1.0;
                for (int i = 0; i < n; ++i) { fl += 2.0 * jobs[i].M * jobs[i].N * jobs[i].K / pl; by += ((double)jobs[i].M + jobs[i].N) * jobs[i].K * 2.0 + (double)jobs[i].M * jobs[i].N * 4.0 / pl; }
                rc = P->timed(*X, "gemm_dw_grouped", fl, by, stream, [&] { return ss_gemm_dw_grouped(n, jobs, stream); });
            }
            n = 0; return rc;
        }
    };

    int forward(Exec& X, const float* x_raw, float* shifted, int B, int T0, int training, int shift_r, float p_drop, unsigned long long seed, float* head, Ctx* c);
    int backward(Exec& X, Ctx* c, const float* dhead);
};

#define L_(call) do { if (call) return 1; } while (0)

static double band_pairs(int T, int D) { double n = 0; for (int q = 0; q < T; ++q) { const int lo = q - (D - 1) < 0 ? 0 : q - (D - 1), hi = q + (D - 1) > T - 1 ? T - 1 : q + (D - 1); n += hi - lo + 1; } return n; }

int Plan::forward(Exec& X, const float* x_raw, float* shifted, int B, int T0, int training, int shift_r, float p_drop, unsigned long long seed, float* head, Ctx* c)
{
    const int dt = D.dtype, d = D.d_model; const size_t es = esz();
    const int Cin0 = 8;
    SS_CHECK(T0 % 8 == 0, "raw EMG length %d must be a multiple of 8 (three stride-2 convolutions)", T0);
    SS_CHECK(D.n_layers <= MAX_LAYERS, "at most %d encoder layers", MAX_LAYERS);
    void* stream = X.stream;
    cur = c; c->planes.n = 0;
    if (!training) p_drop = 0.f;
    c->B = B; c->T0 = T0; c->p_drop = p_drop; c->seed = seed; c->n_layers = D.n_layers;

    void* xin = X.alloc((size_t)B * (T0 + 2) * Cin0 * es);
    if (!X.dry) {
        L_(timed(X, "emg_prepare", 0, (double)B * T0 * Cin0 * (4 + es), stream, [&] { return ss_emg_prepare(dt, x_raw, xin, (training && shift_r > 0) ? shifted : nullptr, B, T0, Cin0, training ? shift_r : 0, stream); }));
        if (training && shift_r > 0 && shifted && !keep_input)
            if (!ss_copy_d2d_async((void*)x_raw, shifted, (size_t)B * T0 * Cin0 * 4, stream)) { ss_set_error("forward: input write-back failed"); return 1; }
    }
    float* bnsums = training ? (float*)X.alloc((size_t)9 * 2 * d * 4) : nullptr;
    if (bnsums && !X.dry) {
        if (!ss_memset_async(bnsums, 0, (size_t)9 * 2 * d * 4, stream)) { ss_set_error("forward: memset failed"); return 1; }
    }
    int Tin = T0, Cin = Cin0;
    for (int i = 0; i < 3; ++i) {
        BlockP& w = blk[i]; BlockCtx& s = c->blk[i];
        const int O = w.O, Tout = Tin / 2, rows = B * Tout;
        s.xin = xin; s.Tin = Tin; s.Cin = Cin; s.Tout = Tout; s.O = O;
        s.scratch = (float*)X.alloc((size_t)ss_bn_scratch_floats(B, Tout, O) * 4);
        const long long in_bs = (long long)(Tin + 2) * Cin;
        int rc = 0;
        float* slot = bnsums ? bnsums + (size_t)i * 3 * 2 * d : nullptr;
        void* c1 = X.alloc((size_t)rows * O * es);
        float* f1 = conv_gemm(X, xin, w.w1f, c1, rows, O, 3 * Cin, RM(2 * Cin, Tout, in_bs), RM(3 * Cin), w.b1, w.bn1, slot, &rc); L_(rc);
        void* cr = X.alloc((size_t)rows * O * es);
        float* fr = conv_gemm(X, xin, w.wr, cr, rows, O, Cin, RM(2 * Cin, Tout, in_bs, Cin), RM(Cin), w.br, w.bnr, slot ? slot + 2 * d : nullptr, &rc); L_(rc);
        double nred = 0.0;
        if (training && hook && f1 && fr == f1 + 2 * d && O == d && !X.dry) nred = hook(hook_user, f1, 4 * O, (double)B * Tout, stream);
        L_(bn_stats(X, c1, B, Tout, O, s.scratch, w.bn1, training, &s.m1, &s.i1, f1, nred));
        void* h1 = X.alloc((size_t)B * (Tout + 2) * O * es);
        if (!X.dry) L_(timed(X, "bn_apply", 0, (double)B * Tout * O * es * 2, stream, [&] { return ss_bn_apply(dt, c1, s.m1, s.i1, w.bn1.gamma, w.bn1.beta, 0, nullptr, nullptr, nullptr, nullptr, nullptr, 0, h1, 1, B, Tout, O, 1, stream); }));
        void* c2 = X.alloc((size_t)rows * O * es);
        float* f2 = conv_gemm(X, h1, w.w2f, c2, rows, O, 3 * O, RM(O, Tout, (long long)(Tout + 2) * O), RM(3 * O), w.b2, w.bn2, slot ? slot + 4 * d : nullptr, &rc); L_(rc);
        L_(bn_stats(X, c2, B, Tout, O, s.scratch, w.bn2, training, &s.m2, &s.i2, f2));
        L_(bn_stats(X, cr, B, Tout, O, s.scratch, w.bnr, training, &s.mr, &s.ir, fr, nred));
        const int pad_y = i == 2 ? 0 : 1;
        void* y = X.alloc((size_t)B * (Tout + 2 * pad_y) * O * es);
        if (!X.dry) L_(timed(X, "bn_apply", 0, (double)B * Tout * O * es * 3, stream, [&] { return ss_bn_apply(dt, c2, s.m2, s.i2, w.bn2.gamma, w.bn2.beta, 0, cr, s.mr, s.ir, w.bnr.gamma, w.bnr.beta, 0, y, pad_y, B, Tout, O, 1, stream); }));
        s.c1 = c1; s.cr = cr; s.h1 = h1; s.c2 = c2; s.y = y; s.pad_y = pad_y;
        xin = y; Tin = Tout; Cin = O;
    }
    if (training && !X.dry) {
        long long* ctrs[9];
        for (int i = 0; i < 3; ++i) { ctrs[3 * i] = blk[i].bn1.nbt; ctrs[3 * i + 1] = blk[i].bn2.nbt; ctrs[3 * i + 2] = blk[i].bnr.nbt; }
        L_(timed(X, "counters", 0, 0, stream, [&] { return ss_counters_add(9, (int64_t**)ctrs, 1, stream); }));
    }
    const int T = Tin, M = B * T;
    c->T = T; c->M = M; c->conv_out = xin;
    void* x = X.alloc((size_t)M * d * es);
    { ss_gemm_epilogue e = EPI(); e.bias = b_raw_in; L_(gemm(X, dt, xin, w_raw_in, x, M, d, d, RM(d), RM(d), RM(d), &e, SS_OP_KC, SS_OP_KC, 1, 0, nullptr, 1)); }

    const int H = D.n_head, dp = D.dp, Dr = D.max_rel, ff = D.ff, HD = H * dp;
    const int Tp = round_up(T, 8);
    const float scale = 1.0f / sqrtf((float)D.d_qkv);
    c->Tp = Tp; c->scale = scale;
    const bool x3att = use_x3_attention(T);
    c->need_T = x3att ? 0 : ss_relpos_attention_needs_transposed(dt, T, dp, Dr);
    for (int l = 0; l < D.n_layers; ++l) {
        LayerP& w = layers[l]; LayerCtx& s = c->layer[l];
        s.x = x;
        void* qkv = X.alloc((size_t)M * 3 * HD * es);
        void* qkvT = nullptr;
        if (c->need_T) {
            qkvT = X.alloc((size_t)B * 3 * HD * Tp * es);
            ss_gemm_epilogue e = EPI(); e.c2 = qkvT; e.cmap2 = RM(1, T, (long long)3 * HD * Tp); e.col_stride2 = Tp;
            L_(gemm(X, dt, x, w.wqkv, qkv, M, 3 * HD, d, RM(d), RM(d), RM(3 * HD), &e));
        } else L_(gemm(X, dt, x, w.wqkv, qkv, M, 3 * HD, d, RM(d), RM(d), RM(3 * HD), nullptr, SS_OP_KC, SS_OP_KC, 1, 0, nullptr, x3att ? 2 : 0));
        void* o = X.alloc((size_t)M * HD * es);
        float* lse = (float*)X.alloc((size_t)B * H * T * 4);
        const size_t pimg_bytes = training ? (size_t)(x3att ? ss_relpos_attention_x3_saved_bytes(B, H, T, dp, Dr) : ss_relpos_attention_saved_bytes(dt, B, H, T, dp, Dr)) : 0;
        void* pimg = pimg_bytes ? X.alloc(pimg_bytes) : nullptr;
        if (x3att) {
            const Pl q = planes(X, qkv, qkv, (long long)M * 3 * HD);
            adopt_planes(o, o, (long long)M * HD);
            if (!X.dry) {
                if (!q.hi) return 1;
                L_(timed(X, "attn_fwd", 2.0 * B * H * band_pairs(T, Dr) * dp * 3.0, (double)M * 4 * HD * es, stream, [&] { return ss_relpos_attention_x3_forward(q.hi, q.lo, w.EF, o, (char*)o + (size_t)M * HD * 2, lse, pimg, B, H, T, dp, Dr, scale, p_drop, seed, 4 * l, stream); }));
            }
        } else
        if (!X.dry) L_(timed(X, "attn_fwd", 2.0 * B * H * band_pairs(T, Dr) * dp * 3.0, (double)M * 4 * HD * es, stream, [&] { return ss_relpos_attention_forward_p(dt == SS_F32 && f32_x3 ? SS_F32X3 : dt, qkv, qkvT, w.E, w.EF, o, lse, pimg, B, H, T, Tp, dp, Dr, scale, p_drop, seed, 4 * l, stream); }));
        s.pimg = pimg;
        void* a = X.alloc((size_t)M * d * es);
        L_(gemm(X, dt, o, w.wo, a, M, d, HD, RM(HD), RM(HD), RM(d)));
        void* y1 = X.alloc((size_t)M * d * es);
        float* mean1 = (float*)X.alloc((size_t)M * 4); float* rstd1 = (float*)X.alloc((size_t)M * 4);
        const Pl y1p = new_planes(X, y1, (long long)M * d);
        if (!X.dry) L_(timed(X, "add_dropout_ln_fwd", 0, (double)M * d * es * 5, stream, [&] { return ss_add_dropout_layernorm_forward_planes(dt, x, a, w.g1, w.be1, y1, y1p.hi, y1p.lo, mean1, rstd1, M, d, D.ln_eps, p_drop, seed, 4 * l + 1, stream); }));
        void* hid = X.alloc((size_t)M * ff * es);
        unsigned char* hid_sign = nullptr;
        { ss_gemm_epilogue e = EPI(); e.bias = w.b1; e.relu = 1; e.dropout_p = p_drop; e.seed = seed; e.rng_stream = 4 * l + 2;
          ss_rowmap am_ = RM(d), bm_ = RM(d), cm_ = RM(ff);
          if (training && dt == SS_BF16 && sign_gate && ff % 8 == 0 && ss_gemm_sign_bits_supported(dt, dt, SS_OP_KC, SS_OP_KC, hid, M, ff, d, &am_, &bm_, &cm_, &e, 1)) {
              hid_sign = (unsigned char*)X.alloc((size_t)M * (ff / 8));
              e.sign_out = hid_sign; e.sign_pitch = ff / 8;
          }
          L_(gemm(X, dt, y1, w.w1, hid, M, ff, d, am_, bm_, cm_, &e, SS_OP_KC, SS_OP_KC, 1, 0, nullptr, 1)); }
        void* f = X.alloc((size_t)M * d * es);
        { ss_gemm_epilogue e = EPI(); e.bias = w.b2; L_(gemm(X, dt, hid, w.w2, f, M, d, ff, RM(ff), RM(ff), RM(d), &e)); }
        void* y2 = X.alloc((size_t)M * d * es);
        float* mean2 = (float*)X.alloc((size_t)M * 4); float* rstd2 = (float*)X.alloc((size_t)M * 4);
        const Pl y2p = new_planes(X, y2, (long long)M * d);
        if (!X.dry) L_(timed(X, "add_dropout_ln_fwd", 0, (double)M * d * es * 5, stream, [&] { return ss_add_dropout_layernorm_forward_planes(dt, y1, f, w.g2, w.be2, y2, y2p.hi, y2p.lo, mean2, rstd2, M, d, D.ln_eps, p_drop, seed, 4 * l + 3, stream); }));
        s.qkv = qkv; s.qkvT = qkvT; s.o = o; s.lse = lse; s.z1 = a; s.mean1 = mean1; s.rstd1 = rstd1; s.y1 = y1;
        s.hid = hid; s.hid_sign = hid_sign; s.z2 = f; s.mean2 = mean2; s.rstd2 = rstd2;
        x = y2;
    }
    c->x_final = x;
    const int nh = D.n_head_cols;
    { ss_gemm_epilogue e = EPI(); e.bias = b_head; L_(gemm(X, SS_F32, x, w_head, head, M, nh, d, RM(d), RM(d), RM(nh), &e)); }
    c->ws_used = X.off;
    return 0;
}

int Plan::backward(Exec& X, Ctx* c, const float* dhead)
{
    const int dt = D.dtype, d = D.d_model; const size_t es = esz();
    const int B = c->B, T = c->T, M = c->M, H = D.n_head, dp = D.dp, Dr = D.max_rel, ff = D.ff, HD = H * dp, Tp = c->Tp, nh = D.n_head_cols;
    const float p_drop = c->p_drop, keep_scale = 1.0f / (1.0f - p_drop);
    const unsigned long long seed = c->seed;
    void* stream = X.stream;
    void* side = (side_enabled && X.side) ? X.side : X.stream;
    const bool overlapped = side != stream;
    X.side = side;
    Exec& XS = X;
    const bool grouped = (dt == SS_BF16 || use_planes()) && dw_grouped;
    cur = c;
    const bool x3att = use_x3_attention(T);

    const void* dh_t = dhead;
    if (dt != SS_F32) { void* t = X.alloc((size_t)M * nh * es); if (!X.dry) L_(timed(X, "cast", 0, (double)M * nh * (4 + es), stream, [&] { return ss_cast_f32(dhead, t, dt, (long long)M * nh, stream); })); dh_t = t; }
    if (!X.dry && stage_arena && stage_arena_bytes > 0) {
        if (!ss_memset_async(stage_arena, 0, (size_t)stage_arena_bytes, stream)) { ss_set_error("backward: memset failed"); return 1; }
    }
    const int old_blocks = ss_gemm_set_blocks_per_cu(overlapped ? side_blocks : 2);
    struct Restore { int v; ~Restore() { ss_gemm_set_blocks_per_cu(v); } } restore{old_blocks};
    ss_gemm_set_blocks_per_cu(2);
#define SIDE_BEGIN() do { fork(X); if (overlapped) ss_gemm_set_blocks_per_cu(side_blocks); } while (0)
#define SIDE_END() do { if (overlapped) ss_gemm_set_blocks_per_cu(2); } while (0)

    DwGroup grp{this, &XS, grouped};
    L_(grp.add(dh_t, c->x_final, head_w_stage, nh, d, M, RM(nh), RM(d), side));
    SIDE_BEGIN(); L_(colsum(X, dh_t, M, nh, head_b_stage, side)); SIDE_END();
    void* G = X.alloc((size_t)M * d * es);
    L_(gemm(X, dt, dh_t, w_head_T, G, M, d, nh, RM(nh), RM(nh), RM(d)));

    const int64_t ln_floats = ss_layernorm_backward_scratch_floats(M, d);
    float* ln_scratch = ln_floats ? (float*)X.alloc((size_t)ln_floats * 4) : nullptr;
    const bool per_layer = on_event != nullptr || !unpack_all.jobs;
    for (int l = c->n_layers - 1; l >= 0; --l) {
        LayerP& w = layers[l]; LayerCtx& s = c->layer[l];
        void* dF = X.alloc((size_t)M * d * es);
        const Pl dFp = ln_floats ? new_planes(X, dF, (long long)M * d) : Pl{nullptr, nullptr};
        if (!X.dry) L_(timed(X, "ln_bwd", 0, (double)M * d * es * 4, stream, [&] { return ss_layernorm_backward_ws_planes(dt, G, s.z2, s.mean2, s.rstd2, w.g2, G, dF, dFp.hi, dFp.lo, w.dg2, w.dbe2, w.db2, ln_scratch, ln_floats, M, d, p_drop, seed, 4 * l + 3, stream); }));
        L_(grp.add(dF, s.hid, w.dw2, d, ff, M, RM(d), RM(ff), side));
        void* dHid = X.alloc((size_t)M * ff * es);
        bool db1_fused = false;
        { ss_gemm_epilogue e = EPI(); e.gate = s.hid; e.gate_scale = keep_scale;
          ss_rowmap am_ = RM(d), bm_ = RM(d), cm_ = RM(ff);
          if (!X.dry && fuse_stats) {
              ss_gemm_epilogue es = e; es.col_sum = w.db1;
              if (s.hid_sign && !use_planes()) {
                  ss_gemm_epilogue eb = es; eb.gate = nullptr; eb.gate_bits = s.hid_sign; eb.gate_bits_pitch = ff / 8;
                  if (ss_gemm_fuses_column_stats(dt, dt, SS_OP_KC, SS_OP_KC, dHid, M, ff, d, &am_, &bm_, &cm_, &eb, 1) != 0) { e = eb; db1_fused = true; }
              }
              if (db1_fused) {}
              else if (use_planes() ? ss_gemm_planes_supported(SS_F32, dHid, M, ff, d, &am_, &bm_, &cm_, &es) != 0 : ss_gemm_fuses_column_stats(dt, dt, SS_OP_KC, SS_OP_KC, dHid, M, ff, d, &am_, &bm_, &cm_, &e, 1) != 0) { e = es; db1_fused = true; }
          }
          L_(gemm(X, dt, dF, w.w2T, dHid, M, ff, d, am_, bm_, cm_, &e, SS_OP_KC, SS_OP_KC, 1, 0, nullptr, db1_fused ? 2 : 1)); }
        L_(grp.add(dHid, s.y1, w.dw1, ff, d, M, RM(ff), RM(d), side));
        if (!db1_fused) { SIDE_BEGIN(); L_(colsum(X, dHid, M, ff, w.db1, side)); SIDE_END(); }
        { ss_gemm_epilogue e = EPI(); e.mode = 1; L_(gemm(X, dt, dHid, w.w1T, G, M, d, ff, RM(ff), RM(ff), RM(d), &e)); }
        void* dA = X.alloc((size_t)M * d * es);
        const Pl dAp = ln_floats ? new_planes(X, dA, (long long)M * d) : Pl{nullptr, nullptr};
        if (!X.dry) L_(timed(X, "ln_bwd", 0, (double)M * d * es * 4, stream, [&] { return ss_layernorm_backward_ws_planes(dt, G, s.z1, s.mean1, s.rstd1, w.g1, G, dA, dAp.hi, dAp.lo, w.dg1, w.dbe1, nullptr, ln_scratch, ln_floats, M, d, p_drop, seed, 4 * l + 1, stream); }));
        L_(grp.add(dA, s.o, w.wo_stage, d, HD, M, RM(d), RM(HD), side));
        void* dO = X.alloc((size_t)M * HD * es);
        void* dOT = nullptr;
        if (c->need_T) {
            dOT = X.alloc((size_t)B * HD * Tp * es);
            ss_gemm_epilogue e = EPI(); e.c2 = dOT; e.cmap2 = RM(1, T, (long long)HD * Tp); e.col_stride2 = Tp;
            L_(gemm(X, dt, dA, w.woT, dO, M, HD, d, RM(d), RM(d), RM(HD), &e));
        } else L_(gemm(X, dt, dA, w.woT, dO, M, HD, d, RM(d), RM(d), RM(HD), nullptr, SS_OP_KC, SS_OP_KC, 1, 0, nullptr, x3att ? 2 : 0));
        void* dqkv = X.alloc((size_t)M * 3 * HD * es);
        float* dsc = (float*)X.alloc((size_t)B * H * T * 4);
        if (x3att) {
            const Pl q = planes(X, s.qkv, s.qkv, (long long)M * 3 * HD), ol = planes(X, s.o, s.o, (long long)M * HD), dop = planes(X, dO, dO, (long long)M * HD);
            adopt_planes(dqkv, dqkv, (long long)M * 3 * HD);
            if (!X.dry) {
                if (!q.hi || !ol.hi || !dop.hi) return 1;
                L_(timed(X, "attn_bwd", 2.0 * B * H * band_pairs(T, Dr) * dp * 5.0, (double)M * 8 * HD * es, stream, [&] { return ss_relpos_attention_x3_backward(q.hi, q.lo, w.EF, ol.hi, ol.lo, dop.hi, dop.lo, dsc, dqkv, (char*)dqkv + (size_t)M * 3 * HD * 2, s.pimg, B, H, T, dp, Dr, c->scale, p_drop, seed, 4 * l, stream); }));
            }
        } else
        if (!X.dry) L_(timed(X, "attn_bwd", 2.0 * B * H * band_pairs(T, Dr) * dp * 5.0, (double)M * 8 * HD * es, stream, [&] { return ss_relpos_attention_backward_p(dt == SS_F32 && f32_x3 ? SS_F32X3 : dt, s.qkv, s.qkvT, w.E, w.ET, w.EF, s.o, s.lse, dO, dOT, dsc, dqkv, s.pimg, B, H, T, Tp, dp, Dr, c->scale, p_drop, seed, 4 * l, stream); }));
        L_(grp.add(dqkv, s.x, w.wqkv_stage, 3 * HD, d, M, RM(3 * HD), RM(d), side));
        { ss_gemm_epilogue e = EPI(); e.mode = 1; L_(gemm(X, dt, dqkv, w.wqkvT, G, M, d, 3 * HD, RM(3 * HD), RM(3 * HD), RM(d), &e)); }
        if (l > 0) {
            SIDE_BEGIN(); L_(grp.launch(side)); if (per_layer) L_(permute_batch(X, w.unpack, side)); SIDE_END();
            if (on_event && !X.dry) on_event(event_user, 4 + l, side);
        }
    }
    L_(grp.add(G, c->conv_out, dw_raw_in, d, d, M, RM(d), RM(d), side));
    SIDE_BEGIN(); L_(grp.launch(side)); L_(colsum(X, G, M, d, db_raw_in, side));
    if (per_layer) {
        if (c->n_layers > 0) L_(permute_batch(X, layers[0].unpack, side));
        L_(permute_batch(X, unpack_enc, side));
    } else L_(permute_batch(X, unpack_all, side));
    SIDE_END();
    if (on_event && !X.dry) {
        if (c->n_layers > 0) on_event(event_user, 4, side);
        on_event(event_user, 0, side);
    }
    void* dy = X.alloc((size_t)M * d * es);
    L_(gemm(X, dt, G, w_raw_in_T, dy, M, d, d, RM(d), RM(d), RM(d)));

    const bool regate = regate_on != 0;
    for (int i = 2; i >= 0; --i) {
        BlockP& w = blk[i]; BlockCtx& s = c->blk[i];
        const int O = s.O, Cin = s.Cin, Tin = s.Tin, Tout = s.Tout, rows = B * Tout;
        const long long pbs = (long long)(Tout + 2) * O;
        void* dc2 = X.alloc((size_t)B * (Tout + 2) * O * es);
        void* dcr = X.alloc((size_t)rows * O * es);
        float* sums = (float*)X.alloc((size_t)3 * O * 4);
        if (!X.dry) {
            L_(timed(X, "bn_bwd_sums", 0, (double)B * Tout * O * es * (regate ? 3 : 4), stream, [&] { return ss_bn_backward_sums(dt, dy, 0, s.y, s.pad_y, s.c2, 0, s.m2, s.i2, s.cr, 0, s.mr, s.ir, w.bn2.dgamma, w.bn2.dbeta, w.bnr.dgamma, w.bnr.dbeta, s.scratch, sums, B, Tout, O, 1, regate ? w.bn2.gamma : nullptr, regate ? w.bn2.beta : nullptr, regate ? w.bnr.gamma : nullptr, regate ? w.bnr.beta : nullptr, stream); }));
            double n_total = (double)B * Tout;
            if (hook) n_total = hook(hook_user, sums, 3 * O, n_total, stream);
            L_(timed(X, "bn_bwd_apply", 0, (double)B * Tout * O * es * (regate ? 5 : 6), stream, [&] { return ss_bn_backward_apply(dt, dy, 0, s.y, s.pad_y, s.c2, 0, s.m2, s.i2, w.bn2.gamma, s.cr, 0, s.mr, s.ir, w.bnr.gamma, sums, n_total, dc2, 1, dcr, 0, B, Tout, O, 1, regate ? w.bn2.beta : nullptr, regate ? w.bnr.beta : nullptr, stream); }));
        }
        DwGroup cg{this, &XS, grouped};
        L_(cg.add(dc2, s.h1, w.c2_stage, O, 3 * O, rows, RM(O, Tout, pbs, O), RM(O, Tout, pbs), side));
        void* dh1 = X.alloc((size_t)rows * O * es);
        L_(gemm(X, dt, dc2, w.w2b, dh1, rows, O, 3 * O, RM(O, Tout, pbs), RM(3 * O), RM(O)));
        void* dc1 = X.alloc((size_t)B * (Tout + 2) * O * es);
        float* sums1 = (float*)X.alloc((size_t)3 * O * 4);
        if (!X.dry) {
            L_(timed(X, "bn_bwd_sums", 0, (double)B * Tout * O * es * (regate ? 2 : 3), stream, [&] { return ss_bn_backward_sums(dt, dh1, 0, s.h1, 1, s.c1, 0, s.m1, s.i1, nullptr, 0, nullptr, nullptr, w.bn1.dgamma, w.bn1.dbeta, nullptr, nullptr, s.scratch, sums1, B, Tout, O, 1, regate ? w.bn1.gamma : nullptr, regate ? w.bn1.beta : nullptr, nullptr, nullptr, stream); }));
            double n_total = (double)B * Tout;
            if (hook) n_total = hook(hook_user, sums1, 3 * O, n_total, stream);
            L_(timed(X, "bn_bwd_apply", 0, (double)B * Tout * O * es * (regate ? 3 : 4), stream, [&] { return ss_bn_backward_apply(dt, dh1, 0, s.h1, 1, s.c1, 0, s.m1, s.i1, w.bn1.gamma, nullptr, 0, nullptr, nullptr, nullptr, sums1, n_total, dc1, 1, nullptr, 0, B, Tout, O, 1, regate ? w.bn1.beta : nullptr, nullptr, stream); }));
        }
        const long long in_bs = (long long)(Tin + 2) * Cin;
        L_(cg.add(dc1, s.xin, w.c1_stage, O, 3 * Cin, rows, RM(O, Tout, pbs, O), RM(2 * Cin, Tout, in_bs), side));
        L_(cg.add(dcr, s.xin, w.wr_grad, O, Cin, rows, RM(O, Tout, (long long)Tout * O), RM(2 * Cin, Tout, in_bs, Cin), side));
        SIDE_BEGIN(); L_(cg.launch(side)); L_(permute_batch(X, w.unpack, side)); SIDE_END();
        if (on_event && !X.dry) on_event(event_user, 1 + (2 - i), side);
        if (i > 0) {
            void* dx = X.alloc((size_t)B * Tin * Cin * es);
            const ss_rowmap out_even = RM(2 * Cin, Tout, (long long)Tin * Cin), out_odd = RM(2 * Cin, Tout, (long long)Tin * Cin, Cin);
            L_(gemm(X, dt, dc1, w.w1b_even, dx, rows, Cin, O, RM(O, Tout, pbs, O), RM(O), out_even));
            { ss_gemm_epilogue e = EPI(); e.mode = 1; L_(gemm(X, dt, dcr, w.wrT, dx, rows, Cin, O, RM(O), RM(O), out_even, &e)); }
            L_(gemm(X, dt, dc1, w.w1b_odd, dx, rows, Cin, 2 * O, RM(O, Tout, pbs, O), RM(2 * O), out_odd));
            dy = dx;
        }
    }
    join(X);
#undef SIDE_BEGIN
#undef SIDE_END
    c->ws_used = X.off;
    return 0;
}

}

struct ss_plan { Plan* p; };

extern "C" ss_plan* ss_plan_create(const ss_model_dims* dims)
{
    if (!dims || dims->n_layers < 0 || dims->n_layers > MAX_LAYERS || dims->d_model % 8 || (dims->dtype != SS_F32 && dims->dtype != SS_BF16)) { ss_set_error("ss_plan_create: bad model dimensions"); return nullptr; }
    ss_plan* h = new ss_plan; h->p = new Plan(*dims);
#if !defined(SS_EMU)
    hipEventCreateWithFlags(&h->p->ev_fork, hipEventDisableTiming); hipEventCreateWithFlags(&h->p->ev_join, hipEventDisableTiming);
#endif
    return h;
}
extern "C" void ss_plan_destroy(ss_plan* h)
{
    if (!h) return;
#if !defined(SS_EMU)
    if (h->p->ev_fork) hipEventDestroy(h->p->ev_fork);
    if (h->p->ev_join) hipEventDestroy(h->p->ev_join);
#endif
    delete h->p; delete h;
}
extern "C" int ss_plan_slot_count(const ss_plan* h) { return h ? (int)h->p->names.size() : 0; }
extern "C" const char* ss_plan_slot_name(const ss_plan* h, int i) { return (h && i >= 0 && i < (int)h->p->names.size()) ? h->p->names[i].c_str() : nullptr; }
// ... 99 lines not shown
```

silent_speech_amd/csrc/runtime.hip:

```cpp
#include "common.h"
#include "silent_speech_hip.h"
#include <stdarg.h>

static thread_local char g_err[512] = "";

void ss_set_error(const char* fmt, ...) {
    va_list ap; va_start(ap, fmt);
    vsnprintf(g_err, sizeof(g_err), fmt, ap);
    va_end(ap);
}
extern "C" const char* ss_last_error(void) { return g_err; }
extern "C" int ss_abi_version(void) { return SS_ABI_VERSION; }
extern "C" const char* ss_target_arch(void) {
#if defined(SS_EMU)
    return "host-emulator";
#else
    return "gfx950";
#endif
}
int ss_check_launch(const char* what) {
    hipError_t e = hipGetLastError();
    if (e != hipSuccess) { ss_set_error("%s: kernel launch failed: %s", what, hipGetErrorString(e)); return 2; }
    return 0;
}

#if !defined(SS_EMU)
#include <mutex>
namespace {
struct PinnedRing {
    static constexpr int N = 8;
    void* buf[N] = {}; size_t cap[N] = {}; hipEvent_t ev[N] = {}; bool used[N] = {}; int at = 0; std::mutex mu;
};
PinnedRing g_ring;
}
#endif
int ss_upload_table(void* dst_dev, const void* src_host, size_t bytes, void* stream)
{
    if (bytes == 0) return 0;
#if defined(SS_EMU)
    memcpy(dst_dev, src_host, bytes);
    return 0;
#else
    std::lock_guard<std::mutex> lock(g_ring.mu);
    const int i = g_ring.at; g_ring.at = (i + 1) % PinnedRing::N;
    if (g_ring.used[i] && hipEventSynchronize(g_ring.ev[i]) != hipSuccess) { ss_set_error("table upload: event wait failed"); return 1; }
    if (g_ring.cap[i] < bytes) {
        if (g_ring.buf[i]) (void)hipHostFree(g_ring.buf[i]);
        size_t cap = 1 << 16; while (cap < bytes) cap <<= 1;
        if (hipHostMalloc(&g_ring.buf[i], cap, hipHostMallocDefault) != hipSuccess) { g_ring.buf[i] = nullptr; g_ring.cap[i] = 0; ss_set_error("table upload: pinned allocation of %zu bytes failed", cap); return 1; }
        g_ring.cap[i] = cap;
    }
    if (!g_ring.ev[i] && hipEventCreateWithFlags(&g_ring.ev[i], hipEventDisableTiming) != hipSuccess) { ss_set_error("table upload: event creation failed"); return 1; }
    memcpy(g_ring.buf[i], src_host, bytes);
    if (hipMemcpyAsync(dst_dev, g_ring.buf[i], bytes, hipMemcpyHostToDevice, (hipStream_t)stream) != hipSuccess) { ss_set_error("table upload failed"); return 1; }
    if (hipEventRecord(g_ring.ev[i], (hipStream_t)stream) != hipSuccess) { ss_set_error("table upload: event record failed"); return 1; }
    g_ring.used[i] = true;
    return 0;
#endif
}

template <class TI, class TO>
__global__ void permute3d_kernel(const TI* __restrict__ in, TO* __restrict__ out, int d0, int d1, int d2,
                                 long long s0, long long s1, long long s2, int valid1, int valid2, float scale, int accumulate)
{
    long long total = (long long)d0 * d1 * d2;
    for (long long i = (long long)blockIdx.x * blockDim.x + threadIdx.x; i < total; i += (long long)gridDim.x * blockDim.x) {
        int c = (int)(i % d2); long long t = i / d2; int b = (int)(t % d1); int a = (int)(t / d1);
        float v = (b < valid1 && c < valid2) ? ldf(in + a * s0 + b * s1 + c * s2) * scale : 0.f;
        if (accumulate) v += ldf(out + i);
        stf(out + i, v);
    }
}

extern "C" int ss_permute3d(const void* in, int in_dtype, void* out, int out_dtype, int d0, int d1, int d2,
                            int64_t s0, int64_t s1, int64_t s2, int valid1, int valid2, float scale, int accumulate, void* stream)
{
    SS_CHECK(in && out, "ss_permute3d: null pointer");
    SS_CHECK(d0 >= 0 && d1 >= 0 && d2 >= 0, "ss_permute3d: negative extent");
    long long total = (long long)d0 * d1 * d2;
    if (total == 0) return 0;
    int block = 256; long long g = (total + block - 1) / block; if (g > 4096) g = 4096;
    dim3 grid((unsigned)g), blk(block);
#define SS_P3(TI, TO) SS_LAUNCH(SS_KERNEL(permute3d_kernel<TI, TO>), grid, blk, 0, stream, (const TI*)in, (TO*)out, d0, d1, d2, (long long)s0, (long long)s1, (long long)s2, valid1, valid2, scale, accumulate)
    if (in_dtype == SS_F32 && out_dtype == SS_F32) SS_P3(float, float);
    else if (in_dtype == SS_F32 && out_dtype == SS_BF16) SS_P3(float, bf16_t);
    else if (in_dtype == SS_BF16 && out_dtype == SS_F32) SS_P3(bf16_t, float);
    else if (in_dtype == SS_BF16 && out_dtype == SS_BF16) SS_P3(bf16_t, bf16_t);
    else SS_CHECK(false, "ss_permute3d: bad dtype");
#undef SS_P3
    SS_LAUNCH_CHECK("ss_permute3d");
    return 0;
}

struct PermuteJob {
    const void* in; void* out;
    long long s0, s1, s2, o0, o1;
    int d0, d1, d2, valid1, valid2, in_dtype, out_dtype, accumulate;
    float scale; int first_block, nblocks, pad_;
};

template <class TI> struct Vec4;
template <> struct Vec4<float> { static __device__ __forceinline__ void load(const float* p, float (&v)[4]) { const f32x4 a = *(const f32x4*)p; v[0] = a[0]; v[1] = a[1]; v[2] = a[2]; v[3] = a[3]; } };
template <> struct Vec4<bf16_t> { static __device__ __forceinline__ void load(const bf16_t* p, float (&v)[4]) { const u32x2 a = *(const u32x2*)p; v[0] = __uint_as_float(a[0] << 16); v[1] = __uint_as_float(a[0] & 0xffff0000u); v[2] = __uint_as_float(a[1] << 16); v[3] = __uint_as_float(a[1] & 0xffff0000u); } };

template <class TI, class TO, bool GROUPED_RMW = false>
__device__ __forceinline__ void permute_job(const PermuteJob& j, int lb, int nthreads, int tid, float* tile)
{
    const long long total = (long long)j.d0 * j.d1 * j.d2;
    const TI* in = (const TI*)j.in; TO* out = (TO*)j.out;
    const long long as0 = j.s0 < 0 ? -j.s0 : j.s0, as1 = j.s1 < 0 ? -j.s1 : j.s1, as2 = j.s2 < 0 ? -j.s2 : j.s2;
    const bool c0 = j.d0 > 1 && as0 >= 1 && as0 <= 4, c1 = j.d1 > 1 && as1 >= 1 && as1 <= 4;
    const bool fx1 = c1 && (!c0 || j.d1 >= j.d0), fx0 = c0 && !fx1;
    const int dXq = fx1 ? j.d1 : j.d0;
    const bool al16 = ((uintptr_t)in % 16) == 0 && ((uintptr_t)out % 16) == 0;
    if (!GROUPED_RMW && !j.accumulate && j.s2 == 1 && j.s1 == j.d2 && j.o1 == j.d2 && (j.d0 == 1 || (j.s0 == (long long)j.d1 * j.d2 && j.o0 == j.s0)) &&
        j.valid1 >= j.d1 && j.valid2 >= j.d2 && (total & 7) == 0 && al16 && total < (1LL << 34)) {
        const unsigned n8 = (unsigned)(total >> 3), step = (unsigned)j.nblocks * nthreads;
        for (unsigned i = (unsigned)lb * nthreads + tid; i < n8; i += step) {
            float v[8]; Vec8<TI>::load(in + (size_t)i * 8, v);
#pragma unroll
            for (int e = 0; e < 8; ++e) v[e] *= j.scale;
            Vec8<TO>::store(out + (size_t)i * 8, v);
        }
        return;
    }
    if (!GROUPED_RMW && sizeof(TO) == 2 && !j.accumulate && as2 >= 8 && (fx0 || fx1) && nthreads == 256 && al16) {
        const int dX = fx1 ? j.d1 : j.d0, dO = fx1 ? j.d0 : j.d1;
        const long long sX = fx1 ? j.s1 : j.s0, sO = fx1 ? j.s0 : j.s1, oX = fx1 ? j.o1 : j.o0, oO = fx1 ? j.o0 : j.o1;
        const int vX = fx1 ? (j.valid1 < j.d1 ? j.valid1 : j.d1) : dX, vO = fx1 ? dO : (j.valid1 < j.d1 ? j.valid1 : j.d1), vC = j.valid2 < j.d2 ? j.valid2 : j.d2;
        if (sX == 1 && !(dX & 7) && !(j.d2 & 7) && !(sO & 7) && !(j.s2 & 7) && !(oX & 7) && !(oO & 7) && !(vX & 7) && !(vC & 7) && dX >= 64 && j.d2 >= 64) {
            unsigned short* t16 = (unsigned short*)tile;
            const int tiles_x = (dX + 63) >> 6, tiles_c = (j.d2 + 63) >> 6;
            const long long ntiles = (long long)dO * tiles_x * tiles_c;
            for (long long t = lb; t < ntiles; t += j.nblocks) {
                const int oi = (int)(t / (tiles_x * tiles_c)), rem = (int)(t - (long long)oi * (tiles_x * tiles_c));
                const int tx = rem / tiles_c, tc = rem - tx * tiles_c;
#pragma unroll
                for (int k = 0; k < 2; ++k) {
                    const int f = k * 256 + tid, cc = f >> 3, x0 = (f & 7) * 8, gx = tx * 64 + x0, gc = tc * 64 + cc;
                    float v[8] = {0.f, 0.f, 0.f, 0.f, 0.f, 0.f, 0.f, 0.f};
                    if (gx < vX && gc < vC && oi < vO) { Vec8<TI>::load(in + oi * sO + gx + (long long)gc * j.s2, v);
#pragma unroll
                        for (int e = 0; e < 8; ++e) v[e] *= j.scale; }
                    unsigned* d = (unsigned*)(t16 + cc * 66 + x0);
#pragma unroll
                    for (int e = 0; e < 4; ++e) d[e] = pack_bf16(v[2 * e], v[2 * e + 1]);
                }
                __syncthreads();
#pragma unroll
                for (int k = 0; k < 2; ++k) {
                    const int f = k * 256 + tid, x = f >> 3, c0 = (f & 7) * 8, gx = tx * 64 + x, gc = tc * 64 + c0;
                    if (gx < dX && gc < j.d2) {
                        u32x4 r;
#pragma unroll
                        for (int e = 0; e < 4; ++e) r[e] = (unsigned)t16[(c0 + 2 * e) * 66 + x] | ((unsigned)t16[(c0 + 2 * e + 1) * 66 + x] << 16);
                        *(u32x4*)(out + oi * oO + gx * oX + gc) = r;
                    }
                }
                __syncthreads();
            }
            return;
        }
    }
    if (sizeof(TI) == 4 && sizeof(TO) == 4 && as2 >= 4 && (fx0 || fx1) && nthreads == 256 && al16) {
        const int dX = fx1 ? j.d1 : j.d0, dO = fx1 ? j.d0 : j.d1;
        const long long sX = fx1 ? j.s1 : j.s0, sO = fx1 ? j.s0 : j.s1, oX = fx1 ? j.o1 : j.o0, oO = fx1 ? j.o0 : j.o1;
        const int vX = fx1 ? (j.valid1 < j.d1 ? j.valid1 : j.d1) : dX, vO = fx1 ? dO : (j.valid1 < j.d1 ? j.valid1 : j.d1), vC = j.valid2 < j.d2 ? j.valid2 : j.d2;
        if (sX == 1 && !(dX & 3) && !(j.d2 & 3) && !(sO & 3) && !(j.s2 & 3) && !(oX & 3) && !(oO & 3) && !(vX & 3) && !(vC & 3) && dX >= 32 && j.d2 >= 32) {
            const int tiles_x = (dX + 63) >> 6, tiles_c = (j.d2 + 63) >> 6;
            const long long ntiles = (long long)dO * tiles_x * tiles_c;
            for (long long t = lb; t < ntiles; t += j.nblocks) {
                const int oi = (int)(t / (tiles_x * tiles_c)), rem = (int)(t - (long long)oi * (tiles_x * tiles_c));
                const int tx = rem / tiles_c, tc = rem - tx * tiles_c;
                f32x4 v[4];
#pragma unroll
                for (int k = 0; k < 4; ++k) {
                    const int f = k * 256 + tid, cc = f >> 4, x0 = (f & 15) * 4, gx = tx * 64 + x0, gc = tc * 64 + cc;
                    const f32x4 z = {0.f, 0.f, 0.f, 0.f};
                    v[k] = (gx < vX && gc < vC && oi < vO) ? *(const f32x4*)((const float*)in + oi * sO + gx + (long long)gc * j.s2) : z;
                }
#pragma unroll
                for (int k = 0; k < 4; ++k) {
                    const int f = k * 256 + tid, cc = f >> 4, x0 = (f & 15) * 4;
#pragma unroll
                    for (int e = 0; e < 4; ++e) tile[cc * 65 + x0 + e] = v[k][e] * j.scale;
                }
                __syncthreads();
                f32x4 w[4]; float* op[4];
#pragma unroll
                for (int k = 0; k < 4; ++k) {
                    const int f = k * 256 + tid, x = f >> 4, c0 = (f & 15) * 4, gx = tx * 64 + x, gc = tc * 64 + c0;
                    op[k] = (gx < dX && gc < j.d2) ? (float*)out + oi * oO + gx * oX + gc : nullptr;
                    const f32x4 z = {0.f, 0.f, 0.f, 0.f};
                    w[k] = (op[k] && j.accumulate) ? *(const f32x4*)op[k] : z;
                }
#pragma unroll
                for (int k = 0; k < 4; ++k) {
                    const int f = k * 256 + tid, x = f >> 4, c0 = (f & 15) * 4;
                    if (op[k]) {
#pragma unroll
                        for (int e = 0; e < 4; ++e) w[k][e] += tile[(c0 + e) * 65 + x];
                        *(f32x4*)op[k] = w[k];
                    }
                }
                __syncthreads();
            }
            return;
        }
    }
    if (as2 > 4 && (fx0 || fx1) && nthreads == 256 && total >= 4096 && (long long)(dXq < 64 ? dXq : 64) * (j.d2 < 64 ? j.d2 : 64) >= 192) {
        const int dX = fx1 ? j.d1 : j.d0, dO = fx1 ? j.d0 : j.d1;
        const long long sX = fx1 ? j.s1 : j.s0, sO = fx1 ? j.s0 : j.s1, oX = fx1 ? j.o1 : j.o0, oO = fx1 ? j.o0 : j.o1;
        const int lx = dX <= 4 ? 2 : (dX <= 16 ? 4 : (j.d2 <= 4 ? 10 : (j.d2 <= 16 ? 8 : 6)));
        const int TX = 1 << lx, lc = 12 - lx, TC = 1 << lc, P = TX + 1;
        const int tiles_x = (dX + TX - 1) >> lx, tiles_c = (j.d2 + TC - 1) >> lc;
        const long long ntiles = (long long)dO * tiles_x * tiles_c;
        for (long long t = lb; t < ntiles; t += j.nblocks) {
            const int oi = (int)(t / (tiles_x * tiles_c)), rem = (int)(t - (long long)oi * (tiles_x * tiles_c));
            const int tx = rem / tiles_c, tc = rem - tx * tiles_c;
            {
                float v[16];
#pragma unroll
                for (int k = 0; k < 16; ++k) {
                    const int f = k * 256 + tid, x = f & (TX - 1), cc = f >> lx;
                    const int gx = tx * TX + x, gc = tc * TC + cc, bb = fx1 ? gx : oi;
                    v[k] = 0.f;
                    if (gx < dX && gc < j.d2 && bb < j.valid1 && gc < j.valid2) v[k] = ldf(in + oi * sO + gx * sX + (long long)gc * j.s2) * j.scale;
                }
#pragma unroll
                for (int k = 0; k < 16; ++k) { const int f = k * 256 + tid; tile[(f >> lx) * P + (f & (TX - 1))] = v[k]; }
            }
            __syncthreads();
            if (!GROUPED_RMW || !j.accumulate) {
#pragma unroll
                for (int k = 0; k < 16; ++k) {
                    const int f = k * 256 + tid, x = f >> lc, cc = f & (TC - 1);
                    const int gx = tx * TX + x, gc = tc * TC + cc;
                    if (gx < dX && gc < j.d2) {
                        TO* o = out + oi * oO + gx * oX + gc;
                        float w = tile[cc * P + x];
                        if (j.accumulate) w += ldf(o);
                        stf(o, w);
                    }
                }
            } else {
#pragma unroll
                for (int h = 0; h < 2; ++h) {
                    float w[8];
#pragma unroll
                    for (int k = 0; k < 8; ++k) {
                        const int f = (h * 8 + k) * 256 + tid, x = f >> lc, cc = f & (TC - 1);
                        const int gx = tx * TX + x, gc = tc * TC + cc;
                        w[k] = tile[cc * P + x];
                        if (gx < dX && gc < j.d2) w[k] += ldf(out + oi * oO + gx * oX + gc);
                    }
#pragma unroll
                    for (int k = 0; k < 8; ++k) {
                        const int f = (h * 8 + k) * 256 + tid, x = f >> lc, cc = f & (TC - 1);
                        const int gx = tx * TX + x, gc = tc * TC + cc;
                        if (gx < dX && gc < j.d2) stf(out + oi * oO + gx * oX + gc, w[k]);
                    }
                }
            }
            __syncthreads();
        }
        return;
    }
    if (j.s2 == 1 && !(j.d2 & 3) && !(j.s0 & 3) && !(j.s1 & 3) && !(j.o0 & 3) && !(j.o1 & 3) && !(j.valid2 & 3) &&
        ((uintptr_t)in % (4 * sizeof(TI))) == 0 && ((uintptr_t)out % (4 * sizeof(TO))) == 0) {
        const int c4n = j.d2 >> 2;
        for (long long i = (long long)lb * nthreads + tid; i < (total >> 2); i += (long long)j.nblocks * nthreads) {
            const int c = (int)(i % c4n) * 4; const long long t = i / c4n; const int b = (int)(t % j.d1); const int a = (int)(t / j.d1);
            float v[4] = {0.f, 0.f, 0.f, 0.f};
            if (b < j.valid1 && c < j.valid2) { Vec4<TI>::load(in + a * j.s0 + b * j.s1 + c, v); v[0] *= j.scale; v[1] *= j.scale; v[2] *= j.scale; v[3] *= j.scale; }
            TO* o = out + a * j.o0 + b * j.o1 + c;
            if (j.accumulate) { float w[4]; Vec4<TO>::load(o, w); v[0] += w[0]; v[1] += w[1]; v[2] += w[2]; v[3] += w[3]; }
            if (sizeof(TO) == 4) { const f32x4 r = {v[0], v[1], v[2], v[3]}; *(f32x4*)o = r; }
            else { const u32x2 r = {pack_bf16(v[0], v[1]), pack_bf16(v[2], v[3])}; *(u32x2*)o = r; }
        }
        return;
    }
    for (long long i = (long long)lb * nthreads + tid; i < total; i += (long long)j.nblocks * nthreads) {
        const int c = (int)(i % j.d2); const long long t = i / j.d2; const int b = (int)(t % j.d1); const int a = (int)(t / j.d1);
        float v = (b < j.valid1 && c < j.valid2) ? ldf(in + a * j.s0 + b * j.s1 + c * j.s2) * j.scale : 0.f;
        TO* o = out + a * j.o0 + b * j.o1 + c;
        if (j.accumulate) v += ldf(o);
        stf(o, v);
    }
}

__global__ void permute3d_batch_kernel(const PermuteJob* __restrict__ jobs, const int* __restrict__ job_of_block)
{
    __shared__ float tile[1024 * 5];
    const PermuteJob j = jobs[job_of_block[blockIdx.x]];
    const int lb = blockIdx.x - j.first_block;
    if (j.in_dtype == SS_F32 && j.out_dtype == SS_F32) permute_job<float, float>(j, lb, blockDim.x, threadIdx.x, tile);
    else if (j.in_dtype == SS_F32) permute_job<float, bf16_t>(j, lb, blockDim.x, threadIdx.x, tile);
    else if (j.out_dtype == SS_F32) permute_job<bf16_t, float>(j, lb, blockDim.x, threadIdx.x, tile);
    else permute_job<bf16_t, bf16_t>(j, lb, blockDim.x, threadIdx.x, tile);
}

__global__ __launch_bounds__(256) void permute3d_batch_f32_kernel(const PermuteJob* __restrict__ jobs, const int* __restrict__ job_of_block)
{
    __shared__ float tile[1024 * 5];
    const PermuteJob j = jobs[job_of_block[blockIdx.x]];
    permute_job<float, float, true>(j, blockIdx.x - j.first_block, blockDim.x, threadIdx.x, tile);
}

extern "C" int ss_permute3d_batch(const void* jobs_dev, const int32_t* job_of_block_dev, int total_blocks, int all_f32, void* stream)
{
    SS_CHECK(total_blocks >= 0, "ss_permute3d_batch: negative block count");
    if (total_blocks == 0) return 0;
    SS_CHECK(jobs_dev && job_of_block_dev, "ss_permute3d_batch: null pointer");
    if (all_f32) SS_LAUNCH(permute3d_batch_f32_kernel, dim3(total_blocks), dim3(256), 0, stream, (const PermuteJob*)jobs_dev, (const int*)job_of_block_dev);
    else SS_LAUNCH(permute3d_batch_kernel, dim3(total_blocks), dim3(256), 0, stream, (const PermuteJob*)jobs_dev, (const int*)job_of_block_dev);
    SS_LAUNCH_CHECK("ss_permute3d_batch");
    return 0;
}
```

silent_speech_amd/engine.py:

```python
import ctypes
import math
import os

import torch

from . import _lib, ops
from ._lib import OP_KC, OP_OC

RM = ops.rowmap


def _round_up(x, m):
    return (x + m - 1) // m * m


class Prepared(object):

    def __init__(self, model):
        self.build(model)

    @staticmethod
    def layout_signature(model):
        return (tuple(p.data_ptr() for p in model.all_parameters()), model.compute_dtype, str(model.w_out.weight.device))

    @staticmethod
    def version_signature(model):
        return (model._weights_version, tuple(p._version for p in model.all_parameters()))

    def build(self, model):
        dt, dev = model.compute_dtype, model.w_out.weight.device
        d = model.d_model
        b1, b2 = ops.PermuteBatch(), ops.PermuteBatch()
        self.b1, self.b2, self.dev = b1, b2, dev

        def new(*shape, dtype=dt, zero=False):
            return (torch.zeros if zero else torch.empty)(*shape, dtype=dtype, device=dev)

        def cast(w):
            w = w.detach()
            if dt == torch.float32:
                return w
            return b1.add(w, new(*w.shape), (1, w.shape[0], w.shape[1]), (0, w.shape[1], 1))

        def transposed(src, n, k):
            return b2.add(src, new(k, n), (k, 1, n), (1, 0, k))

        self.blocks = []
        for blk in model.conv_blocks:
            O, I, _ = blk.conv1.weight.shape
            e = {}
            w1, w2 = blk.conv1.weight.detach(), blk.conv2.weight.detach()
            e['w1f'] = b1.add(w1, new(O, 3 * I), (O, 3, I), (3 * I, 1, 3))
            e['w2f'] = b1.add(w2, new(O, 3 * O), (O, 3, O), (3 * O, 1, 3))
            e['wr'] = b1.add(blk.residual_path.weight.detach(), new(O, I), (O, 1, I), (I, 0, 1))
            e['wrT'] = transposed(e['wr'], O, I)
            e['w2b'] = b1.add(w2.view(-1)[2:], new(O, 3 * O), (O, 3, O), (3, -1, 3 * O))
            if I % 8 == 0:
                e['w1b_even'] = b1.add(w1.view(-1)[1:], new(I, O), (I, 1, O), (3, 0, 3 * I))
                e['w1b_odd'] = b1.add(w1.view(-1)[2:], new(I, 2 * O), (I, 2, O), (3, -2, 3 * I))
            self.blocks.append(e)

        self.w_raw_in = cast(model.w_raw_in.weight)
        self.w_raw_in_T = transposed(self.w_raw_in, d, d)
        H, dh, dp, D = model.n_head, model.d_qkv, model.dp, model.max_rel
        MPt = _round_up(2 * D - 1, 32)
        self.layers = []
        for layer in model.transformer.layers:
            a = layer.self_attn
            e = {}
            wqkv = new(3, H, dp, d)
            for i, w in enumerate((a.w_q, a.w_k, a.w_v)):
                b1.add(w.detach(), wqkv[i], (H, dp, d), (d * dh, 1, dh), valid1=dh)
            e['wqkv'] = wqkv.view(3 * H * dp, d)
            e['wqkvT'] = transposed(e['wqkv'], 3 * H * dp, d)
            e['wo'] = b1.add(a.w_o.detach(), new(d, H * dp), (d, H, dp), (1, dh * d, d), valid2=dh)
            e['woT'] = transposed(e['wo'], d, H * dp)
            emb = a.relative_positional.embeddings.detach()
            e['E'] = b1.add(emb, new(H, 2 * D - 1, dp), (H, 2 * D - 1, dp), ((2 * D - 1) * dh, dh, 1), valid2=dh)
            e['ET'] = b1.add(emb, new(H, dp, MPt), (H, dp, MPt), ((2 * D - 1) * dh, 1, dh), valid1=dh, valid2=2 * D - 1)
            nb = int(_lib.lib().ss_relpos_attention_table_bytes(H, dp, D)) if dt == torch.bfloat16 else int(_lib.lib().ss_relpos_attention_x3_table_bytes(H, dp, D))
            e['EF.x3'] = dt != torch.bfloat16 and nb > 0
            e['EF'] = new(max(nb // 2, 8), dtype=torch.bfloat16)
            e['EF.src'], e['EF.version'], e['EF.scale'] = a.relative_positional.embeddings, None, 1.0 / math.sqrt(dh)
            e['w1'] = cast(layer.linear1.weight)
            e['w2'] = cast(layer.linear2.weight)
            e['w1T'] = transposed(e['w1'], layer.linear1.weight.shape[0], d)
            e['w2T'] = transposed(e['w2'], d, layer.linear2.weight.shape[1])
            self.layers.append(e)
        n_out = model.w_out.weight.shape[0]
        n_aux = model.w_aux.weight.shape[0] if model.has_aux_out else 0
        nh = _round_up(n_out + n_aux, 8)
        wh = new(nh, d, zero=True)
        bh = new(nh, dtype=torch.float32, zero=True)
        b1.add(model.w_out.weight.detach(), wh[:n_out], (1, n_out, d), (0, d, 1))
        b1.add(model.w_out.bias.detach(), bh[:n_out], (1, 1, n_out), (0, 0, 1))
        if n_aux:
            b1.add(model.w_aux.weight.detach(), wh[n_out:n_out + n_aux], (1, n_aux, d), (0, d, 1))
            b1.add(model.w_aux.bias.detach(), bh[n_out:n_out + n_aux], (1, 1, n_aux), (0, 0, 1))
        self.w_head, self.b_head, self.n_head_cols = wh, bh, nh
        self.w_head_T = transposed(wh, nh, d)
        self.layout_sig = self.layout_signature(model)
        self.refresh(model)

    def refresh(self, model):
        self.b1.run(self.dev)
        self.b2.run(self.dev)
        for e in self.layers:
            src = e['EF.src']
            if e['EF'].numel() > 8 and e['EF.version'] != (src._version, src.data_ptr()):
                (ops.relpos_attention_x3_tables if e['EF.x3'] else ops.relpos_attention_tables)(src, model.dp, e['EF.scale'], out=e['EF'])
                e['EF.version'] = (src._version, src.data_ptr())
        self.version_sig = self.version_signature(model)


def prepared(model):
    pr = getattr(model, '_prepared', None)
    if pr is None or pr.layout_sig != Prepared.layout_signature(model):
        pr = Prepared(model)
        model._prepared = pr
    elif pr.version_sig != Prepared.version_signature(model):
        pr.refresh(model)
    return pr


class ModelDims(ctypes.Structure):
    _fields_ = [('d_model', ctypes.c_int32), ('n_layers', ctypes.c_int32), ('n_head', ctypes.c_int32), ('d_qkv', ctypes.c_int32),
                ('dp', ctypes.c_int32), ('max_rel', ctypes.c_int32), ('ff', ctypes.c_int32), ('n_head_cols', ctypes.c_int32),
                ('dtype', ctypes.c_int32), ('ln_eps', ctypes.c_float)]


class GradUnpack(object):

    def __init__(self, model, dev):
        d, H, dh, dp = model.d_model, model.n_head, model.d_qkv, model.dp
        pr = prepared(model)
        nh = pr.n_head_cols
        sizes = [('head_w', nh * d), ('head_b', nh)]
        for l in range(len(model.transformer.layers)):
            sizes += [('wo%d' % l, d * H * dp), ('wqkv%d' % l, 3 * H * dp * d)]
        for i, blk in enumerate(model.conv_blocks):
            O, I, _ = blk.conv1.weight.shape
            sizes += [('c2_%d' % i, O * 3 * O), ('c1_%d' % i, O * 3 * I)]
        total = sum((n + 3) // 4 * 4 for _, n in sizes)
        self.arena = torch.zeros(total, dtype=torch.float32, device=dev)
        self.buf, off = {}, 0
        for k, n in sizes:
            self.buf[k] = self.arena[off:off + n]
            off += (n + 3) // 4 * 4
        ub = ops.PermuteBatch()
        n_out = model.w_out.weight.shape[0]
        n_aux = model.w_aux.weight.shape[0] if model.has_aux_out else 0
        hw, hb = self.buf['head_w'].view(nh, d), self.buf['head_b']
        ub.add(hw[:n_out], model.w_out.weight.grad, (1, n_out, d), (0, d, 1), accumulate=True)
        ub.add(hb[:n_out], model.w_out.bias.grad, (1, 1, n_out), (0, 0, 1), accumulate=True)
        if n_aux:
            ub.add(hw[n_out:n_out + n_aux], model.w_aux.weight.grad, (1, n_aux, d), (0, d, 1), accumulate=True)
            ub.add(hb[n_out:n_out + n_aux], model.w_aux.bias.grad, (1, 1, n_aux), (0, 0, 1), accumulate=True)
        self.head_batch = ub
        ua = ops.PermuteBatch()
        ua.add(hw[:n_out], model.w_out.weight.grad, (1, n_out, d), (0, d, 1), accumulate=True)
        ua.add(hb[:n_out], model.w_out.bias.grad, (1, 1, n_out), (0, 0, 1), accumulate=True)
        if n_aux:
            ua.add(hw[n_out:n_out + n_aux], model.w_aux.weight.grad, (1, n_aux, d), (0, d, 1), accumulate=True)
            ua.add(hb[n_out:n_out + n_aux], model.w_aux.bias.grad, (1, 1, n_aux), (0, 0, 1), accumulate=True)
        self.all_batch = ua
        self.layer_batches = []
        for l, layer in enumerate(model.transformer.layers):
            a = layer.self_attn
            lb = ops.PermuteBatch()
            lb.add(self.buf['wo%d' % l], a.w_o.grad, (H, dh, d), (dp, 1, H * dp), accumulate=True)
            for i, wp in enumerate((a.w_q, a.w_k, a.w_v)):
                lb.add(self.buf['wqkv%d' % l][i * H * dp * d:], wp.grad, (H, d, dh), (dp * d, 1, d), accumulate=True)
            self.layer_batches.append(lb)
            ua.add(self.buf['wo%d' % l], a.w_o.grad, (H, dh, d), (dp, 1, H * dp), accumulate=True)
            for i, wp in enumerate((a.w_q, a.w_k, a.w_v)):
                ua.add(self.buf['wqkv%d' % l][i * H * dp * d:], wp.grad, (H, d, dh), (dp * d, 1, d), accumulate=True)
        self.conv_batches = []
        for i, blk in enumerate(model.conv_blocks):
            O, I, _ = blk.conv1.weight.shape
            cb = ops.PermuteBatch()
            cb.add(self.buf['c2_%d' % i], blk.conv2.weight.grad, (O, O, 3), (3 * O, 1, O), accumulate=True)
            cb.add(self.buf['c1_%d' % i], blk.conv1.weight.grad, (O, I, 3), (3 * I, 1, I), accumulate=True)
            self.conv_batches.append(cb)
        self.sig = self.signature(model)

    @staticmethod
    def signature(model):
        return (model._gflat.data_ptr() if getattr(model, '_gflat', None) is not None else 0,
                tuple(p.grad.data_ptr() for p in model.optimized_parameters()), str(model.w_out.weight.device))


def grad_unpack(model, dev):
    gu = getattr(model, '_grad_unpack', None)
    if gu is None or gu.sig != GradUnpack.signature(model):
        gu = GradUnpack(model, dev)
        model._grad_unpack = gu
    return gu


SIDE_STREAM_ENABLED = True


def _split_k(M, N, K):
    tiles = ((M + 127) // 128) * ((N + 127) // 128)
    overlapped = SIDE_STREAM_ENABLED and os.environ.get('SS_AMD_SIDE_STREAM', '1') != '0'
    s = max(1, min(64, (400 if overlapped else 512) // max(tiles, 1)))
    return max(1, min(s, K // 512 if K >= 512 else 1))


_REDUCE_HOOK = ctypes.CFUNCTYPE(ctypes.c_double, ctypes.c_void_p, ctypes.c_void_p, ctypes.c_int, ctypes.c_double, ctypes.c_void_p)
_EVENT_HOOK = ctypes.CFUNCTYPE(None, ctypes.c_void_p, ctypes.c_int, ctypes.c_void_p)


class PlanBinding(object):

    def __init__(self, model):
        L = _lib.lib()
        pr = prepared(model)
        layer0 = model.transformer.layers[0] if len(model.transformer.layers) else None
        dims = ModelDims(model.d_model, len(model.transformer.layers), model.n_head, model.d_qkv, model.dp, model.max_rel,
                         layer0.linear1.weight.shape[0] if layer0 is not None else 0, pr.n_head_cols, _lib.dtype_code(model.compute_dtype),
                         float(layer0.norm1.eps) if layer0 is not None else 1e-5)
        self.handle = L.ss_plan_create(ctypes.byref(dims))
        if not self.handle:
            raise RuntimeError('ss_plan_create failed: %s' % L.ss_last_error().decode())
        self.lib = L
        self.names = [L.ss_plan_slot_name(self.handle, i).decode() for i in range(L.ss_plan_slot_count(self.handle))]
        self.sig = None
        self.layout = (model.d_model, len(model.transformer.layers), model.compute_dtype)
        self.ctx_bytes = int(L.ss_plan_ctx_bytes())
        self.keep = None
        self.ws = None
        self._hook = self._hook_fn = None
        self._event = self._event_fn = None
        self.callback_error = None

    def __del__(self):
        try:
            if self.handle:
                self.lib.ss_plan_destroy(self.handle)
        except Exception:
            pass

    @staticmethod
    def _table(model, pr, gu, dev):
        t = {}

        def bn(prefix, m, grads):
            t[prefix + '.weight'], t[prefix + '.bias'] = m.weight, m.bias
            t[prefix + '.running_mean'], t[prefix + '.running_var'], t[prefix + '.num_batches_tracked'] = m.running_mean, m.running_var, m.num_batches_tracked
            if grads:
                t[prefix + '.weight.grad'], t[prefix + '.bias.grad'] = m.weight.grad, m.bias.grad

        def batch(prefix, pb):
            jobs, jb, total = pb.device_tables(dev)
            t[prefix + '.jobs'], t[prefix + '.blocks'], t[prefix + '.total'], t[prefix + '.all_f32'] = jobs, jb, int(total), 1

        g = gu is not None
        for i, (blk, w) in enumerate(zip(model.conv_blocks, pr.blocks)):
# ... 175 lines not shown
```

silent_speech_amd/ops.py:

```python
import ctypes

import torch

from . import _lib
from ._lib import OP_KC, OP_OC, RowMap, GemmEpilogue


def rowmap(row_stride, rows_per_batch=0, batch_stride=0, base=0):
    return RowMap(int(base), int(batch_stride), int(row_stride), int(rows_per_batch))


PROFILER = None


class LaunchProfiler(object):

    def __init__(self):
        self.records = []
        self.enabled = True

    def run(self, name, flops, nbytes, fn):
        if not self.enabled or not torch.cuda.is_available():
            return fn()
        s = torch.cuda.Event(enable_timing=True)
# ... 48 lines not shown

def _s(t):
    return _lib.stream_of(t)


def _dt(t):
    return _lib.dtype_code(t.dtype)


_epi_defaults = dict(log_clamp=0.0, c2=None, cmap2=None, col_stride2=0, sign_out=None, gate_bits=None)


def gemm_ex(A, B, C, M, N, K, amap, bmap, cmap, **kw):
    extras = {k: kw.pop(k) for k in list(kw) if k in _epi_defaults}
    if not extras:
        return gemm(A, B, C, M, N, K, amap, bmap, cmap, **kw)
    return _gemm_full(A, B, C, M, N, K, amap, bmap, cmap, extras, **kw)


def _gemm_full(A, B, C, M, N, K, amap, bmap, cmap, extras, a_mode=OP_KC, b_mode=OP_KC, bias=None, relu=False, gate=None,
               gate_scale=1.0, alpha=1.0, dropout_p=0.0, seed=0, rng_stream=0, mode=0, split_k=1, col_perm=None, col_stats=None, f32_math='exact'):
    epi = GemmEpilogue()
    if col_stats is not None:
        cs, cq, sh = col_stats
        epi.col_sum, epi.col_sumsq, epi.col_shift = _p(cs).value, (_p(cq).value if cq is not None else None), (_p(sh).value if sh is not None else None)
    epi.bias = _p(bias).value if bias is not None else None
    epi.gate = _p(gate).value if gate is not None else None
    epi.gate_scale, epi.alpha, epi.relu, epi.dropout_p = gate_scale, alpha, int(bool(relu)), float(dropout_p)
    epi.seed, epi.rng_stream, epi.mode = int(seed) & 0xFFFFFFFFFFFFFFFF, int(rng_stream), int(mode)
    if col_perm is not None:
        epi.col_mod, epi.col_mul, epi.col_div_mul = col_perm
    epi.log_clamp = float(extras.get('log_clamp', 0.0))
    if extras.get('sign_out') is not None:
        assert extras['sign_out'].dtype == torch.uint8 and extras['sign_out'].numel() >= M * (N // 8)
        epi.sign_out, epi.sign_pitch = _p(extras['sign_out']).value, N // 8
    if extras.get('gate_bits') is not None:
        assert extras['gate_bits'].dtype == torch.uint8 and extras['gate_bits'].numel() >= M * (N // 8)
        epi.gate_bits, epi.gate_bits_pitch = _p(extras['gate_bits']).value, N // 8
    c2 = extras.get('c2')
    if c2 is not None:
        assert c2.dtype == C.dtype
        epi.c2 = _p(c2).value
        epi.cmap2 = extras['cmap2']
        epi.col_stride2 = int(extras['col_stride2'])
    assert A.dtype == B.dtype
    if bias is not None:
        assert bias.dtype == torch.float32 and bias.numel() >= N
    if gate is not None:
        assert gate.dtype == C.dtype

    dt_in = _dt(A)
    if f32_math != 'exact':
        if f32_math != 'bf16x3' or A.dtype != torch.float32:
            raise ValueError("f32_math is 'exact' or 'bf16x3', and 'bf16x3' needs float32 operands")
        dt_in = _lib.SS_F32X3

    def launch():
        rc = _L().ss_gemm(dt_in, _dt(C), a_mode, b_mode, _p(A), _p(B), _p(C), M, N, K, ctypes.byref(amap), ctypes.byref(bmap),
                          ctypes.byref(cmap), ctypes.byref(epi), split_k, _s(C))
        _lib.check(rc, 'ss_gemm')
    if PROFILER is not None and C.is_cuda:
        PROFILER.run('ss_gemm (from Python)', 2.0 * M * N * K, (M * K + N * K) * A.element_size() + M * N * C.element_size(), launch)
    else:
        launch()
    return C


GEMM_OPT_W2, GEMM_OPT_W2_BM, GEMM_OPT_G8, GEMM_OPT_G8_NI, GEMM_OPT_G8_PIN, GEMM_OPT_DEBUG, GEMM_OPT_SMALLK = range(7)


def gemm_set_option(what, value):
    return _L().ss_gemm_set_option(int(what), int(value))


def gemm_dw_grouped(jobs):
    flat = []
    for (dy, x, dw, M, N, K, amap, bmap, ldc) in jobs:
        if isinstance(dy, tuple):
            (dh, dl), (xh, xl) = dy, x
            flat += [(dl, xh, dw, M, N, K, amap, bmap, ldc, 1), (dh, xl, dw, M, N, K, amap, bmap, ldc, 1), (dh, xh, dw, M, N, K, amap, bmap, ldc, 1)]
        else:
            flat.append((dy, x, dw, M, N, K, amap, bmap, ldc, 0))
    cap = 24 if any(f[9] for f in flat) else 8
    for g0 in range(0, len(flat), cap):
        grp = flat[g0:g0 + cap]
        arr = (_lib.DwJob * len(grp))()
        for j, (dy, x, dw, M, N, K, amap, bmap, ldc, flags) in zip(arr, grp):
            assert dy.dtype == torch.bfloat16 and x.dtype == torch.bfloat16 and dw.dtype == torch.float32
            j.A, j.B, j.C = _p(dy).value, _p(x).value, _p(dw).value
            j.amap, j.bmap, j.ldc, j.M, j.N, j.K, j.flags = amap, bmap, int(ldc), int(M), int(N), int(K), flags
        _lib.check(_L().ss_gemm_dw_grouped(len(grp), arr, _s(grp[0][2])), 'ss_gemm_dw_grouped')


def split_planes(x):
    assert x.dtype == torch.float32 and x.is_contiguous()
    hi = torch.empty(x.shape, dtype=torch.bfloat16, device=x.device)
    lo = torch.empty(x.shape, dtype=torch.bfloat16, device=x.device)
    _lib.check(_L().ss_split_planes(_p(x), _p(hi), _p(lo), x.numel(), _s(x)), 'ss_split_planes')
    return hi, lo


def gemm_planes_supported(C, M, N, K, amap, bmap, cmap, epi=None):
    return bool(_L().ss_gemm_planes_supported(_lib.SS_F32, _p(C), M, N, K, ctypes.byref(amap), ctypes.byref(bmap), ctypes.byref(cmap), ctypes.byref(epi) if epi is not None else None))


def gemm_planes(A, B, C, M, N, K, amap, bmap, cmap, bias=None, relu=False, gate=None, gate_scale=1.0, alpha=1.0, dropout_p=0.0, seed=0, rng_stream=0,
                mode=0, col_stats=None, planes_out=None, planes_only=False):
    epi = GemmEpilogue()
    if planes_out is not None:
        assert all(t.dtype == torch.bfloat16 for t in planes_out)
        epi.planes_hi, epi.planes_lo, epi.planes_only = _p(planes_out[0]).value, _p(planes_out[1]).value, int(bool(planes_only))
    if col_stats is not None:
        cs, cq, sh = col_stats
        epi.col_sum, epi.col_sumsq, epi.col_shift = _p(cs).value, (_p(cq).value if cq is not None else None), (_p(sh).value if sh is not None else None)
    epi.bias = _p(bias).value if bias is not None else None
    epi.gate = _p(gate).value if gate is not None else None
    epi.gate_scale, epi.alpha, epi.relu, epi.dropout_p = gate_scale, alpha, int(bool(relu)), float(dropout_p)
    epi.seed, epi.rng_stream, epi.mode = int(seed) & 0xFFFFFFFFFFFFFFFF, int(rng_stream), int(mode)
    assert C.dtype == torch.float32 and all(t.dtype == torch.bfloat16 for t in (A[0], A[1], B[0], B[1]))
    rc = _L().ss_gemm_planes(_lib.SS_F32, _p(A[0]), _p(A[1]), _p(B[0]), _p(B[1]), _p(C), M, N, K, ctypes.byref(amap), ctypes.byref(bmap), ctypes.byref(cmap),
                             ctypes.byref(epi), _s(C))
    _lib.check(rc, 'ss_gemm_planes')
    return C


def bn_scratch(B, T, C, device):
    return torch.empty(int(_L().ss_bn_scratch_floats(B, T, C)), dtype=torch.float32, device=device)


def bn_stats(x, B, T, C, pad, scratch, running_mean, running_var, momentum=0.1, eps=1e-5, training=True, shift=None,
             reduce_fn=None):
    mean = torch.empty(C, dtype=torch.float32, device=x.device)
    invstd = torch.empty(C, dtype=torch.float32, device=x.device)
    n_total, sums = float(B * T), None
    if training:
        sums = torch.empty(3 * C, dtype=torch.float32, device=x.device)
        _lib.check(_L().ss_bn_stats_sums(_dt(x), _p(x), B, T, C, pad, _p(scratch), _p(shift), _p(sums), _s(x)), 'ss_bn_stats_sums')
        if reduce_fn is not None:
            n_total = reduce_fn(sums[:2 * C], n_total)
    rc = _L().ss_bn_finalize(_p(sums), n_total, C, _p(mean), _p(invstd), _p(running_mean), _p(running_var), momentum, eps, int(training), _s(x))
    _lib.check(rc, 'ss_bn_finalize')
    return mean, invstd


def bn_apply(xa, sa, pad_xa, y, pad_y, B, T, C, relu, xb=None, sb=None, pad_xb=0):
    n4 = [None] * 4
    b4 = sb if sb is not None else n4
    rc = _L().ss_bn_apply(_dt(xa), _p(xa), _p(sa[0]), _p(sa[1]), _p(sa[2]), _p(sa[3]), pad_xa,
                          _p(xb), _p(b4[0]), _p(b4[1]), _p(b4[2]), _p(b4[3]), pad_xb, _p(y), pad_y, B, T, C, int(relu), _s(xa))
    _lib.check(rc, 'ss_bn_apply')
    return y


def bn_backward(dy, pad_dy, y, pad_y, xa, pad_xa, sa, dxa, pad_dxa, dgamma_a, dbeta_a, scratch, B, T, C, relu,
                xb=None, pad_xb=0, sb=None, dxb=None, pad_dxb=0, dgamma_b=None, dbeta_b=None, reduce_fn=None, beta_a=None, beta_b=None):
    b3 = sb if sb is not None else [None] * 3
    gate = (sa[2], beta_a, b3[2], beta_b) if beta_a is not None else (None, None, None, None)
    sums = torch.empty(3 * C, dtype=torch.float32, device=dy.device)
    rc = _L().ss_bn_backward_sums(_dt(dy), _p(dy), pad_dy, _p(y), pad_y, _p(xa), pad_xa, _p(sa[0]), _p(sa[1]),
                                  _p(xb), pad_xb, _p(b3[0]), _p(b3[1]), _p(dgamma_a), _p(dbeta_a), _p(dgamma_b), _p(dbeta_b),
                                  _p(scratch), _p(sums), B, T, C, int(relu), _p(gate[0]), _p(gate[1]), _p(gate[2]), _p(gate[3]), _s(dy))
    _lib.check(rc, 'ss_bn_backward_sums')
    n_total = float(B * T)
    if reduce_fn is not None:
        n_total = reduce_fn(sums, n_total)
    rc = _L().ss_bn_backward_apply(_dt(dy), _p(dy), pad_dy, _p(y), pad_y, _p(xa), pad_xa, _p(sa[0]), _p(sa[1]), _p(sa[2]),
                                   _p(xb), pad_xb, _p(b3[0]), _p(b3[1]), _p(b3[2]), _p(sums), n_total, _p(dxa), pad_dxa, _p(dxb), pad_dxb,
                                   B, T, C, int(relu), _p(gate[1]), _p(gate[3]), _s(dy))
    _lib.check(rc, 'ss_bn_backward_apply')


def colsum(x, rows, C, ld, out_accum):
    scratch = torch.empty(int(_L().ss_colsum_scratch_floats(rows, C)), dtype=torch.float32, device=x.device)
    _lib.check(_L().ss_colsum(_dt(x), _p(x), rows, C, ld, _p(scratch), _p(out_accum), _s(x)), 'ss_colsum')


def add_dropout_layernorm(x, branch_inout, gamma, beta, y, rows, C, eps=1e-5, p=0.0, seed=0, rng_stream=0, planes=None):
    mean = torch.empty(rows, dtype=torch.float32, device=x.device)
    rstd = torch.empty(rows, dtype=torch.float32, device=x.device)
    rc = _L().ss_add_dropout_layernorm_forward_planes(_dt(x), _p(x), _p(branch_inout), _p(gamma), _p(beta), _p(y), _p(planes[0]) if planes else None, _p(planes[1]) if planes else None,
                                                      _p(mean), _p(rstd), rows, C, eps, p, int(seed) & 0xFFFFFFFFFFFFFFFF, rng_stream, _s(x))
    _lib.check(rc, 'ss_add_dropout_layernorm_forward')
    return mean, rstd


_ln_scratch = {}


def layernorm_backward(dy, z, mean, rstd, gamma, dres, dbranch, dgamma, dbeta, rows, C, p=0.0, seed=0, rng_stream=0, dbranch_colsum=None, planes=None):
    n = int(_L().ss_layernorm_backward_scratch_floats(rows, C))
    scratch = None
    if n:
        key = (str(dy.device), n, int(_s(dy).value or 0))
        scratch = _ln_scratch.get(key)
        if scratch is None:
            scratch = _ln_scratch[key] = torch.empty(n, dtype=torch.float32, device=dy.device)
    rc = _L().ss_layernorm_backward_ws_planes(_dt(dy), _p(dy), _p(z), _p(mean), _p(rstd), _p(gamma), _p(dres), _p(dbranch), _p(planes[0]) if planes else None,
                                              _p(planes[1]) if planes else None, _p(dgamma), _p(dbeta),
                                              _p(dbranch_colsum), _p(scratch), n, rows, C, p, int(seed) & 0xFFFFFFFFFFFFFFFF, rng_stream, _s(dy))
    _lib.check(rc, 'ss_layernorm_backward')


def emg_prepare(x_raw, out_padded, shifted_copy, B, T0, Cin, shift):
    rc = _L().ss_emg_prepare(_dt(out_padded), _p(x_raw), _p(out_padded), _p(shifted_copy), B, T0, Cin, shift, _s(x_raw))
    _lib.check(rc, 'ss_emg_prepare')


def adamw_step(p, g, m, v, n, lr, step, beta1=0.9, beta2=0.999, eps=1e-8, weight_decay=0.0, grad_scale=1.0):
    timed('adamw_kernel', 0, 28.0 * n,
          lambda: _lib.check(_L().ss_adamw_step(_p(p), _p(g), _p(m), _p(v), n, lr, beta1, beta2, eps, weight_decay, step, grad_scale, _s(p)), 'ss_adamw_step'))


def cast_f32(src, dst, n):
    _lib.check(_L().ss_cast_f32(_p(src), _p(dst), _dt(dst), n, _s(src)), 'ss_cast_f32')


def relpos_attention_saved_bytes(dtype, B, H, T, dp, D):
    return int(_L().ss_relpos_attention_saved_bytes(dtype if isinstance(dtype, int) else _lib.dtype_code(dtype), B, H, T, dp, D))


def _attn_dt(qkv, f32_math):
    if f32_math == 'exact':
        return _dt(qkv)
    if f32_math != 'bf16x3' or qkv.dtype != torch.float32:
        raise ValueError("f32_math is 'exact' or 'bf16x3', and 'bf16x3' needs float32 tensors")
    return _lib.SS_F32X3


def relpos_attention_family(dtype, T, dp, D):
    return int(_L().ss_relpos_attention_family(dtype if isinstance(dtype, int) else _lib.dtype_code(dtype), T, dp, D))


def relpos_attention_tables(emb, dp, scale, out=None):
    emb = emb.detach().reshape(emb.shape[0], emb.shape[1], -1).float().contiguous()
    H, NE, dh = emb.shape
    D = (NE + 1) // 2
    nbytes = int(_L().ss_relpos_attention_table_bytes(H, dp, D))
    if nbytes <= 0:
        raise ValueError('no transposed-score attention tables for H=%d dp=%d' % (H, dp))
    if out is None:
        out = torch.empty(nbytes // 2, dtype=torch.bfloat16, device=emb.device)
    _lib.check(_L().ss_relpos_attention_prepare_tables(_p(emb), _p(out), H, D, dh, dp, scale, _s(emb)), 'ss_relpos_attention_prepare_tables')
    return out


def _attn_tab(qkv, E, T, dp, D, scale, f32_math, tab):
    if tab is None and f32_math == 'exact' and relpos_attention_family(_dt(qkv), T, dp, D) == 2:
        tab = relpos_attention_tables(E, dp, scale)
    return tab


def relpos_attention_forward(qkv, qkvT, E, out, lse, B, H, T, Tp, dp, D, scale, p=0.0, seed=0, rng_stream=0, saved=None, f32_math='exact', tab=None):
    tab = _attn_tab(qkv, E, T, dp, D, scale, f32_math, tab)
    rc = _L().ss_relpos_attention_forward_p(_attn_dt(qkv, f32_math), _p(qkv), _p(qkvT), _p(E), _p(tab), _p(out), _p(lse), _p(saved), B, H, T, Tp, dp, D, scale, p,
                                            int(seed) & 0xFFFFFFFFFFFFFFFF, rng_stream, _s(qkv))
    _lib.check(rc, 'ss_relpos_attention_forward')


def relpos_attention_backward(qkv, qkvT, E, ET, out, lse, dO, dOT, dscratch, dqkv, B, H, T, Tp, dp, D, scale, p=0.0, seed=0, rng_stream=0, saved=None,
                              f32_math='exact', tab=None):
    tab = _attn_tab(qkv, E, T, dp, D, scale, f32_math, tab)
    rc = _L().ss_relpos_attention_backward_p(_attn_dt(qkv, f32_math), _p(qkv), _p(qkvT), _p(E), _p(ET), _p(tab), _p(out), _p(lse), _p(dO), _p(dOT), _p(dscratch),
                                             _p(dqkv), _p(saved), B, H, T, Tp, dp, D, scale, p, int(seed) & 0xFFFFFFFFFFFFFFFF, rng_stream, _s(qkv))
    _lib.check(rc, 'ss_relpos_attention_backward')


def relpos_attention_x3_supported(T, dp, D):
    return bool(_L().ss_relpos_attention_x3_supported(T, dp, D))


def relpos_attention_x3_saved_bytes(B, H, T, dp, D):
    return int(_L().ss_relpos_attention_x3_saved_bytes(B, H, T, dp, D))


def relpos_attention_x3_tables(emb, dp, scale, out=None):
    emb = emb.detach().reshape(emb.shape[0], emb.shape[1], -1).float().contiguous()
    H, NE, dh = emb.shape
    D = (NE + 1) // 2
    nbytes = int(_L().ss_relpos_attention_x3_table_bytes(H, dp, D))
    if nbytes <= 0:
        raise ValueError('no transposed-score attention tables for H=%d dp=%d' % (H, dp))
    if out is None:
        out = torch.empty(nbytes // 2, dtype=torch.bfloat16, device=emb.device)
    _lib.check(_L().ss_relpos_attention_x3_prepare_tables(_p(emb), _p(out), H, D, dh, dp, scale, _s(emb)), 'ss_relpos_attention_x3_prepare_tables')
    return out


def relpos_attention_x3_forward(qkv, tab, out, lse, B, H, T, dp, D, scale, p=0.0, seed=0, rng_stream=0, saved=None):
    rc = _L().ss_relpos_attention_x3_forward(_p(qkv[0]), _p(qkv[1]), _p(tab), _p(out[0]), _p(out[1]), _p(lse), _p(saved), B, H, T, dp, D, scale, p,
                                             int(seed) & 0xFFFFFFFFFFFFFFFF, rng_stream, _s(lse))
    _lib.check(rc, 'ss_relpos_attention_x3_forward')


def relpos_attention_x3_backward(qkv, tab, out, dO, dscratch, dqkv, saved, B, H, T, dp, D, scale, p=0.0, seed=0, rng_stream=0):
    rc = _L().ss_relpos_attention_x3_backward(_p(qkv[0]), _p(qkv[1]), _p(tab), _p(out[0]), _p(out[1]), _p(dO[0]), _p(dO[1]), _p(dscratch), _p(dqkv[0]), _p(dqkv[1]),
                                              _p(saved), B, H, T, dp, D, scale, p, int(seed) & 0xFFFFFFFFFFFFFFFF, rng_stream, _s(dscratch))
    _lib.check(rc, 'ss_relpos_attention_x3_backward')


class PermuteBatch(object):

    def __init__(self):
        self.jobs, self.keep, self._dev = [], [], None

    def add(self, inp, out, dims, strides, valid1=None, valid2=None, scale=1.0, accumulate=False, out_strides=None):
        d0, d1, d2 = dims
        if out_strides is None:
            assert out.is_contiguous() and out.numel() >= d0 * d1 * d2
            out_strides = (d1 * d2, d2)
        j = _lib.PermuteJob()
        j.inp, j.out = _p(inp).value, _p(out).value
        j.s0, j.s1, j.s2 = [int(x) for x in strides]
        j.o0, j.o1 = int(out_strides[0]), int(out_strides[1])
        j.d0, j.d1, j.d2 = d0, d1, d2
        j.valid1 = d1 if valid1 is None else valid1
        j.valid2 = d2 if valid2 is None else valid2
        j.in_dtype, j.out_dtype, j.accumulate, j.scale = _dt(inp), _dt(out), int(accumulate), float(scale)
        total = d0 * d1 * d2
        j.nblocks = max(1, min(2048, (total + 4095) // 4096))
        self.jobs.append(j)
        self.keep.append((inp, out))
        self._dev = None
        return out

    def _finalize(self, device):
        import numpy as np
        first, job_of_block = 0, []
        for i, j in enumerate(self.jobs):
            j.first_block = first
            first += j.nblocks
            job_of_block += [i] * j.nblocks
        arr = (_lib.PermuteJob * len(self.jobs))(*self.jobs)
        raw = torch.frombuffer(bytearray(ctypes.string_at(ctypes.addressof(arr), ctypes.sizeof(arr))), dtype=torch.uint8).clone()
        self._dev = (raw.to(device), torch.tensor(job_of_block, dtype=torch.int32).to(device), first)

    def device_tables(self, device):
        if self._dev is None or self._dev[0].device != device:
            self._finalize(device)
        return self._dev

    def run(self, device):
        if not self.jobs:
            return
        if self._dev is None or self._dev[0].device != device:
            self._finalize(device)
        jobs, jb, total = self._dev
        all_f32 = int(all(j.in_dtype == 0 and j.out_dtype == 0 for j in self.jobs))
        nbytes = sum(j.d0 * j.d1 * j.d2 * ((4 if j.in_dtype == 0 else 2) + (4 if j.out_dtype == 0 else 2)) for j in self.jobs)
        timed('permute3d_batch (weight re-layout)', 0, nbytes,
              lambda: _lib.check(_L().ss_permute3d_batch(_p(jobs), _p(jb), total, all_f32, _s(jobs)), 'ss_permute3d_batch'))
```

Before: 1.695 million.

## Fuse BatchNorm finalize into apply and write weight transposes in one permute pass

Adds a BatchNorm apply variant that computes mean and invstd directly from the reduced sums, removing the separate finalize kernel. Running-statistics updates for up to 16 BatchNorms, plus step counters, are batched into a single deferred kernel. The weight re-layout permute job gains a second output so the transposed copy is written in the same pass, which drops the second permute batch. Each apply thread recomputes the per-channel statistics, adding redundant arithmetic and sum reads in exchange for fewer launches.

```diff
diff --git a/include/silent_speech_hip.h b/include/silent_speech_hip.h
--- a/include/silent_speech_hip.h
+++ b/include/silent_speech_hip.h
@@ -10,7 +10,7 @@
 #define SS_F32X3 3
 
 const char* ss_last_error(void);
-#define SS_ABI_VERSION 10
+#define SS_ABI_VERSION 11
 int ss_abi_version(void);
 const char* ss_target_arch(void);
 
@@ -104,6 +104,13 @@
 int ss_bn_apply(int dtype, const void* xa, const float* mean_a, const float* invstd_a, const float* gamma_a, const float* beta_a, int pad_xa,
                 const void* xb, const float* mean_b, const float* invstd_b, const float* gamma_b, const float* beta_b, int pad_xb,
                 void* y, int pad_y, int B, int T, int C, int relu, void* stream);
+int ss_bn_apply_sums(int dtype, const void* xa, const float* sums_a, const float* shift_a, const float* gamma_a, const float* beta_a, int pad_xa,
+                     const void* xb, const float* sums_b, const float* shift_b, const float* gamma_b, const float* beta_b, int pad_xb,
+                     double n_total, float eps, float* mean_a, float* invstd_a, float* mean_b, float* invstd_b,
+                     void* y, int pad_y, int B, int T, int C, int relu, void* stream);
+typedef struct ss_bn_running { const float* sums; float* running_mean; float* running_var; int32_t C; float n_total; } ss_bn_running;
+int ss_bn_update_running(int n, const ss_bn_running* bns , float momentum, int n_counters, int64_t** counters ,
+                         int64_t delta, void* stream);
 int ss_bn_backward_sums(int dtype, const void* dy, int pad_dy, const void* y, int pad_y,
                         const void* xa, int pad_xa, const float* mean_a, const float* invstd_a,
                         const void* xb, int pad_xb, const float* mean_b, const float* invstd_b,
diff --git a/silent_speech_amd/_lib.py b/silent_speech_amd/_lib.py
--- a/silent_speech_amd/_lib.py
+++ b/silent_speech_amd/_lib.py
@@ -7,7 +7,7 @@
 _LIB_PATH = os.environ.get('SS_AMD_LIBRARY') or os.path.join(_HERE, 'lib', 'libsilent_speech_hip.so')
 
 SS_F32, SS_BF16, SS_F64, SS_F32X3 = 0, 1, 2, 3
-ABI_VERSION = 10
+ABI_VERSION = 11
 OP_KC, OP_OC = 0, 1
 
 
@@ -36,12 +36,16 @@
     _fields_ = [('name', ctypes.c_char * 64), ('calls', ctypes.c_int64), ('seconds', ctypes.c_double), ('flops', ctypes.c_double), ('bytes', ctypes.c_double)]
 
 
+class BnRunning(ctypes.Structure):
+    _fields_ = [('sums', ctypes.c_void_p), ('running_mean', ctypes.c_void_p), ('running_var', ctypes.c_void_p), ('C', ctypes.c_int32), ('n_total', ctypes.c_float)]
+
+
 class PermuteJob(ctypes.Structure):
     _fields_ = [('inp', ctypes.c_void_p), ('out', ctypes.c_void_p), ('s0', ctypes.c_int64), ('s1', ctypes.c_int64), ('s2', ctypes.c_int64),
                 ('o0', ctypes.c_int64), ('o1', ctypes.c_int64), ('d0', ctypes.c_int32), ('d1', ctypes.c_int32), ('d2', ctypes.c_int32),
                 ('valid1', ctypes.c_int32), ('valid2', ctypes.c_int32), ('in_dtype', ctypes.c_int32), ('out_dtype', ctypes.c_int32),
                 ('accumulate', ctypes.c_int32), ('scale', ctypes.c_float), ('first_block', ctypes.c_int32), ('nblocks', ctypes.c_int32),
-                ('pad_', ctypes.c_int32)]
+                ('out2_dtype', ctypes.c_int32), ('out2', ctypes.c_void_p), ('q0', ctypes.c_int64), ('q1', ctypes.c_int64), ('q2', ctypes.c_int64)]
 
 
 _P, _I, _F, _L = ctypes.c_void_p, ctypes.c_int, ctypes.c_float, ctypes.c_int64
@@ -72,6 +76,8 @@
     'ss_bn_finalize': [_P, ctypes.c_double, _I, _P, _P, _P, _P, _F, _F, _I, _P],
     'ss_bn_finalize_shift': [_P, _P, ctypes.c_double, _I, _P, _P, _P, _P, _F, _F, _I, _P],
     'ss_bn_apply': [_I, _P, _P, _P, _P, _P, _I, _P, _P, _P, _P, _P, _I, _P, _I, _I, _I, _I, _I, _P],
+    'ss_bn_apply_sums': [_I, _P, _P, _P, _P, _P, _I, _P, _P, _P, _P, _P, _I, ctypes.c_double, _F, _P, _P, _P, _P, _P, _I, _I, _I, _I, _I, _P],
+    'ss_bn_update_running': [_I, ctypes.POINTER(BnRunning), _F, _I, ctypes.POINTER(ctypes.c_void_p), _L, _P],
     'ss_bn_backward_sums': [_I, _P, _I, _P, _I, _P, _I, _P, _P, _P, _I, _P, _P, _P, _P, _P, _P, _P, _P, _I, _I, _I, _I, _P, _P, _P, _P, _P],
     'ss_bn_backward_apply': [_I, _P, _I, _P, _I, _P, _I, _P, _P, _P, _P, _I, _P, _P, _P, _P, ctypes.c_double, _P, _I, _P, _I, _I, _I, _I, _I, _P, _P, _P],
     'ss_colsum': [_I, _P, _I, _I, _L, _P, _P, _P],
diff --git a/silent_speech_amd/csrc/norm.hip b/silent_speech_amd/csrc/norm.hip
--- a/silent_speech_amd/csrc/norm.hip
+++ b/silent_speech_amd/csrc/norm.hip
@@ -117,19 +117,54 @@
     sums[c] = t[0]; sums[C + c] = t[1]; sums[2 * C + c] = shift ? shift[c] : ldf(x + sx.row(0) * C + c);
 }
 
+__device__ __forceinline__ void bn_mean_var(float s1, float s2, float shift, float n, float& mu, float& var) {
+    const float d = s1 / n;
+    mu = shift + d;
+    var = s2 / n - d * d; var = var < 0.f ? 0.f : var;
+}
+__device__ __forceinline__ void bn_running(float* running_mean, float* running_var, int c, float mu, float var, float n, float momentum) {
+    running_mean[c] = (1.f - momentum) * running_mean[c] + momentum * mu;
+    running_var[c] = (1.f - momentum) * running_var[c] + momentum * var * (n > 1.f ? n / (n - 1.f) : 1.f);
+}
+
 __global__ void bn_finalize_kernel(const float* __restrict__ sums, const float* shift, float n, int C, float* mean, float* invstd, float* running_mean, float* running_var,
                                    float momentum, float eps, int training)
 {
     const int c = blockIdx.x * blockDim.x + threadIdx.x;
     if (c >= C) return;
     if (!training) { mean[c] = running_mean[c]; invstd[c] = rsqrtf(running_var[c] + eps); return; }
-    const float d = sums[c] / n, mu = (shift ? shift[c] : sums[2 * C + c]) + d;
-    float var = sums[C + c] / n - d * d; var = var < 0.f ? 0.f : var;
+    float mu, var;
+    bn_mean_var(sums[c], sums[C + c], shift ? shift[c] : sums[2 * C + c], n, mu, var);
     mean[c] = mu; invstd[c] = rsqrtf(var + eps);
-    if (running_mean) {
-        running_mean[c] = (1.f - momentum) * running_mean[c] + momentum * mu;
-        running_var[c] = (1.f - momentum) * running_var[c] + momentum * var * (n > 1.f ? n / (n - 1.f) : 1.f);
-    }
+    if (running_mean) bn_running(running_mean, running_var, c, mu, var, n, momentum);
+}
+
+struct BnRunningJobs { ss_bn_running bn[16]; long long* ctr[16]; };
+__global__ void bn_running_kernel(BnRunningJobs J, int n_counters, long long delta, float momentum)
+{
+    const ss_bn_running b = J.bn[blockIdx.x];
+    if (blockIdx.x == 0 && (int)threadIdx.x < n_counters && J.ctr[threadIdx.x]) J.ctr[threadIdx.x][0] += delta;
+    if (!b.sums) return;
+    for (int c = threadIdx.x; c < b.C; c += blockDim.x) {
+        float mu, var;
+        bn_mean_var(b.sums[c], b.sums[b.C + c], b.running_mean[c], b.n_total, mu, var);
+        bn_running(b.running_mean, b.running_var, c, mu, var, b.n_total, momentum);
+    }
+}
+
+extern "C" int ss_bn_update_running(int n, const ss_bn_running* bns, float momentum, int n_counters, int64_t** counters, int64_t delta, void* stream)
+{
+    SS_CHECK(n >= 0 && n <= 16 && n_counters >= 0 && n_counters <= 16 && (n == 0 || bns) && (n_counters == 0 || counters), "ss_bn_update_running: 0..16 BatchNorms and 0..16 counters");
+    if (n == 0 && n_counters == 0) return 0;
+    BnRunningJobs J; memset(&J, 0, sizeof(J));
+    for (int i = 0; i < n; ++i) {
+        SS_CHECK(bns[i].sums && bns[i].running_mean && bns[i].running_var && bns[i].C > 0 && bns[i].n_total >= 1.f, "ss_bn_update_running: incomplete entry %d", i);
+        J.bn[i] = bns[i];
+    }
+    for (int i = 0; i < n_counters; ++i) J.ctr[i] = (long long*)counters[i];
+    SS_LAUNCH(bn_running_kernel, dim3(n > 0 ? n : 1), dim3(256), 0, stream, J, n_counters, (long long)delta, momentum);
+    SS_LAUNCH_CHECK("ss_bn_update_running");
+    return 0;
 }
 
 static int red_threads(int C) {
@@ -190,10 +225,22 @@
     __device__ __forceinline__ void next() { ro += rstep; b += db; tp += dtp; if (tp >= TP) { tp -= TP; ++b; } }
 };
 
-template <class T>
-__global__ void bn_apply_kernel(const T* __restrict__ xa, Seq sa, const float* __restrict__ mean_a, const float* __restrict__ invstd_a, const float* __restrict__ gamma_a, const float* __restrict__ beta_a,
-                                const T* __restrict__ xb, Seq sb, const float* __restrict__ mean_b, const float* __restrict__ invstd_b, const float* __restrict__ gamma_b, const float* __restrict__ beta_b,
-                                T* __restrict__ y, Seq sy, int B, int C, int relu)
+struct BnDerive { const float *sums_a, *shift_a, *sums_b, *shift_b; float n, eps; };
+__device__ __forceinline__ void bn_derive8(const float* __restrict__ sums, const float* __restrict__ shift, int C, int c8, float n, float eps, float (&mu)[8], float (&is)[8]) {
+    float s1[8], s2[8], sh[8];
+    ld8(sums + c8, s1); ld8(sums + C + c8, s2); ld8(shift + c8, sh);
+#pragma unroll
+    for (int e = 0; e < 8; ++e) { float var; bn_mean_var(s1[e], s2[e], sh[e], n, mu[e], var); is[e] = rsqrtf(var + eps); }
+}
+__device__ __forceinline__ void st8(float* p, const float (&v)[8]) {
+    const f32x4 a = {v[0], v[1], v[2], v[3]}, b = {v[4], v[5], v[6], v[7]};
+    *(f32x4*)p = a; *(f32x4*)(p + 4) = b;
+}
+
+template <class T, bool SUMS = false>
+__global__ void bn_apply_kernel(const T* __restrict__ xa, Seq sa, const float* mean_a, const float* invstd_a, const float* __restrict__ gamma_a, const float* __restrict__ beta_a,
+                                const T* __restrict__ xb, Seq sb, const float* mean_b, const float* invstd_b, const float* __restrict__ gamma_b, const float* __restrict__ beta_b,
+                                T* __restrict__ y, Seq sy, int B, int C, int relu, BnDerive D)
 {
     const int CV = C >> 3, TT = sy.T;
     const unsigned TP = (unsigned)(TT + 2 * sy.pad), rows_out = (unsigned)B * TP, step32 = gridDim.x * blockDim.x;
@@ -204,11 +251,19 @@
         for (int e = 0; e < 8; ++e) { mb[e] = 0.f; scb[e] = 0.f; bb[e] = 0.f; }
         {
             float t[8];
-            ld8(mean_a + w.cx * 8, ma); ld8(gamma_a + w.cx * 8, sca); ld8(invstd_a + w.cx * 8, t); ld8(beta_a + w.cx * 8, ba);
+            if (SUMS) {
+                bn_derive8(D.sums_a, D.shift_a, C, w.cx * 8, D.n, D.eps, ma, t);
+                if (w.ro == 0) { st8((float*)mean_a + w.cx * 8, ma); st8((float*)invstd_a + w.cx * 8, t); }
+            } else { ld8(mean_a + w.cx * 8, ma); ld8(invstd_a + w.cx * 8, t); }
+            ld8(gamma_a + w.cx * 8, sca); ld8(beta_a + w.cx * 8, ba);
 #pragma unroll
             for (int e = 0; e < 8; ++e) sca[e] *= t[e];
             if (xb) {
-                ld8(mean_b + w.cx * 8, mb); ld8(gamma_b + w.cx * 8, scb); ld8(invstd_b + w.cx * 8, t); ld8(beta_b + w.cx * 8, bb);
+                if (SUMS) {
+                    bn_derive8(D.sums_b, D.shift_b, C, w.cx * 8, D.n, D.eps, mb, t);
+                    if (w.ro == 0) { st8((float*)mean_b + w.cx * 8, mb); st8((float*)invstd_b + w.cx * 8, t); }
+                } else { ld8(mean_b + w.cx * 8, mb); ld8(invstd_b + w.cx * 8, t); }
+                ld8(gamma_b + w.cx * 8, scb); ld8(beta_b + w.cx * 8, bb);
 #pragma unroll
                 for (int e = 0; e < 8; ++e) scb[e] *= t[e];
             }
@@ -258,17 +313,27 @@
         const unsigned ro = i / (unsigned)CV; const int cx = (int)(i - ro * (unsigned)CV);
         const unsigned bq = ro / TP; const int b = (int)bq, tp = (int)(ro - bq * TP), t = tp - sy.pad;
         float o[8];
+        float ma[8], ia[8], mb[8], ib[8];
+        if (SUMS) {
+            bn_derive8(D.sums_a, D.shift_a, C, cx * 8, D.n, D.eps, ma, ia);
+            if (ro == 0) { st8((float*)mean_a + cx * 8, ma); st8((float*)invstd_a + cx * 8, ia); }
+            if (xb) {
+                bn_derive8(D.sums_b, D.shift_b, C, cx * 8, D.n, D.eps, mb, ib);
+                if (ro == 0) { st8((float*)mean_b + cx * 8, mb); st8((float*)invstd_b + cx * 8, ib); }
+            }
+        }
         if (t < 0 || t >= TT) {
 #pragma unroll
             for (int e = 0; e < 8; ++e) o[e] = 0.f;
         } else {
+            if (!SUMS) { ld8(mean_a + cx * 8, ma); ld8(invstd_a + cx * 8, ia); if (xb) { ld8(mean_b + cx * 8, mb); ld8(invstd_b + cx * 8, ib); } }
             float v[8]; Vec8<T>::load(xa + sa.at(b, t) * C + cx * 8, v);
 #pragma unroll
-            for (int e = 0; e < 8; ++e) { const int c = cx * 8 + e; const float s = gamma_a[c] * invstd_a[c]; o[e] = (v[e] - mean_a[c]) * s + beta_a[c]; }
+            for (int e = 0; e < 8; ++e) { const int c = cx * 8 + e; const float s = gamma_a[c] * ia[e]; o[e] = (v[e] - ma[e]) * s + beta_a[c]; }
             if (xb) {
                 float u[8]; Vec8<T>::load(xb + sb.at(b, t) * C + cx * 8, u);
 #pragma unroll
-                for (int e = 0; e < 8; ++e) { const int c = cx * 8 + e; const float s = gamma_b[c] * invstd_b[c]; o[e] += (u[e] - mean_b[c]) * s + beta_b[c]; }
+                for (int e = 0; e < 8; ++e) { const int c = cx * 8 + e; const float s = gamma_b[c] * ib[e]; o[e] += (u[e] - mb[e]) * s + beta_b[c]; }
             }
             if (relu) {
 #pragma unroll
@@ -303,9 +368,28 @@
     Seq sa = {T, pad_xa}, sb = {T, pad_xb}, sy = {T, pad_y};
     const long long total = (long long)B * (T + 2 * pad_y) * (C / 8);
     SS_CHECK(total < (1LL << 31) - (1LL << 22), "ss_bn_apply: tensor too large for 32-bit chunk indices");
-    if (dtype == SS_BF16) SS_LAUNCH(bn_apply_kernel<bf16_t>, ew_grid(total, 256, C / 8), dim3(256), 0, stream, (const bf16_t*)xa, sa, mean_a, invstd_a, gamma_a, beta_a, (const bf16_t*)xb, sb, mean_b, invstd_b, gamma_b, beta_b, (bf16_t*)y, sy, B, C, relu);
-    else SS_LAUNCH(bn_apply_kernel<float>, ew_grid(total, 256, C / 8), dim3(256), 0, stream, (const float*)xa, sa, mean_a, invstd_a, gamma_a, beta_a, (const float*)xb, sb, mean_b, invstd_b, gamma_b, beta_b, (float*)y, sy, B, C, relu);
+    const BnDerive none = {nullptr, nullptr, nullptr, nullptr, 0.f, 0.f};
+    if (dtype == SS_BF16) SS_LAUNCH(bn_apply_kernel<bf16_t>, ew_grid(total, 256, C / 8), dim3(256), 0, stream, (const bf16_t*)xa, sa, mean_a, invstd_a, gamma_a, beta_a, (const bf16_t*)xb, sb, mean_b, invstd_b, gamma_b, beta_b, (bf16_t*)y, sy, B, C, relu, none);
+    else SS_LAUNCH(bn_apply_kernel<float>, ew_grid(total, 256, C / 8), dim3(256), 0, stream, (const float*)xa, sa, mean_a, invstd_a, gamma_a, beta_a, (const float*)xb, sb, mean_b, invstd_b, gamma_b, beta_b, (float*)y, sy, B, C, relu, none);
     SS_LAUNCH_CHECK("ss_bn_apply");
+    return 0;
+}
+
+extern "C" int ss_bn_apply_sums(int dtype, const void* xa, const float* sums_a, const float* shift_a, const float* gamma_a, const float* beta_a, int pad_xa,
+                                const void* xb, const float* sums_b, const float* shift_b, const float* gamma_b, const float* beta_b, int pad_xb,
+                                double n_total, float eps, float* mean_a, float* invstd_a, float* mean_b, float* invstd_b,
+                                void* y, int pad_y, int B, int T, int C, int relu, void* stream)
+{
+    SS_CHECK(xa && sums_a && shift_a && mean_a && invstd_a && gamma_a && beta_a && y, "ss_bn_apply_sums: null pointer");
+    SS_CHECK(!xb || (sums_b && shift_b && mean_b && invstd_b && gamma_b && beta_b), "ss_bn_apply_sums: second branch incomplete");
+    SS_CHECK(C % 8 == 0 && C > 0 && B > 0 && T > 0 && n_total >= 1.0, "ss_bn_apply_sums: bad shape B=%d T=%d C=%d", B, T, C);
+    Seq sa = {T, pad_xa}, sb = {T, pad_xb}, sy = {T, pad_y};
+    const long long total = (long long)B * (T + 2 * pad_y) * (C / 8);
+    SS_CHECK(total < (1LL << 31) - (1LL << 22), "ss_bn_apply_sums: tensor too large for 32-bit chunk indices");
+    const BnDerive D = {sums_a, shift_a, sums_b, shift_b, (float)n_total, eps};
+    if (dtype == SS_BF16) SS_LAUNCH(SS_KERNEL(bn_apply_kernel<bf16_t, true>), ew_grid(total, 256, C / 8), dim3(256), 0, stream, (const bf16_t*)xa, sa, mean_a, invstd_a, gamma_a, beta_a, (const bf16_t*)xb, sb, mean_b, invstd_b, gamma_b, beta_b, (bf16_t*)y, sy, B, C, relu, D);
+    else SS_LAUNCH(SS_KERNEL(bn_apply_kernel<float, true>), ew_grid(total, 256, C / 8), dim3(256), 0, stream, (const float*)xa, sa, mean_a, invstd_a, gamma_a, beta_a, (const float*)xb, sb, mean_b, invstd_b, gamma_b, beta_b, (float*)y, sy, B, C, relu, D);
+    SS_LAUNCH_CHECK("ss_bn_apply_sums");
     return 0;
 }
 
diff --git a/silent_speech_amd/csrc/plan.hip b/silent_speech_amd/csrc/plan.hip
--- a/silent_speech_amd/csrc/plan.hip
+++ b/silent_speech_amd/csrc/plan.hip
@@ -64,6 +64,7 @@
     PermB unpack_enc, unpack_all;
     reduce_fn hook = 0; void* hook_user = 0;
     event_fn on_event = 0; void* event_user = 0;
+    ss_bn_running bn_upd[9]; int n_bn_upd = 0;
     int side_enabled = 1, dw_grouped = 1, side_blocks = 2, fuse_stats = 1, regate_on = 1, f32_x3 = 0;
     int x3_attn = 0;
     int sign_gate = 1;
@@ -203,11 +204,17 @@
         if (X.dry || !b.jobs || b.total <= 0) return 0;
         return timed(X, "grad_unlayout", 0, 0, stream, [&] { return ss_permute3d_batch(b.jobs, (const int32_t*)b.blocks, (int)b.total, (int)b.all_f32, stream); });
     }
-    int bn_stats(Exec& X, const void* x, int B, int T, int C, float* scratch, BnP& bn, bool training, float** mean, float** invstd, float* fused = nullptr, double reduced_n = 0.0) {
+    int bn_stats(Exec& X, const void* x, int B, int T, int C, float* scratch, BnP& bn, bool training, float** mean, float** invstd, float* fused = nullptr, double reduced_n = 0.0, bool defer = false) {
         *mean = (float*)X.alloc((size_t)C * 4); *invstd = (float*)X.alloc((size_t)C * 4);
         float* sums = (training && !fused) ? (float*)X.alloc((size_t)3 * C * 4) : fused;
         if (X.dry) return 0;
         double n_total = (double)B * T;
+        if (fused && defer) {
+            SS_CHECK(n_bn_upd < 9, "forward: more than nine deferred BatchNorm updates");
+            const ss_bn_running u = {fused, bn.rmean, bn.rvar, C, (float)n_total};
+            bn_upd[n_bn_upd++] = u;
+            return 0;
+        }
         if (training) {
             if (!fused && timed(X, "bn_stats", 0, (double)B * T * C * esz(), X.stream, [&] { return ss_bn_stats_sums(D.dtype, x, B, T, C, 0, scratch, hook ? bn.rmean : nullptr, sums, X.stream); })) return 1;
             if (reduced_n > 0.0) n_total = reduced_n;
@@ -304,7 +311,7 @@
     SS_CHECK(T0 % 8 == 0, "raw EMG length %d must be a multiple of 8 (three stride-2 convolutions)", T0);
     SS_CHECK(D.n_layers <= MAX_LAYERS, "at most %d encoder layers", MAX_LAYERS);
     void* stream = X.stream;
-    cur = c; c->planes.n = 0;
+    cur = c; c->planes.n = 0; n_bn_upd = 0;
     if (!training) p_drop = 0.f;
     c->B = B; c->T0 = T0; c->p_drop = p_drop; c->seed = seed; c->n_layers = D.n_layers;
 
@@ -333,23 +340,28 @@
         float* fr = conv_gemm(X, xin, w.wr, cr, rows, O, Cin, RM(2 * Cin, Tout, in_bs, Cin), RM(Cin), w.br, w.bnr, slot ? slot + 2 * d : nullptr, &rc); L_(rc);
         double nred = 0.0;
         if (training && hook && f1 && fr == f1 + 2 * d && O == d && !X.dry) nred = hook(hook_user, f1, 4 * O, (double)B * Tout, stream);
-        L_(bn_stats(X, c1, B, Tout, O, s.scratch, w.bn1, training, &s.m1, &s.i1, f1, nred));
+        const bool defer1 = training && !hook && f1, defer2 = training && !hook;
+        L_(bn_stats(X, c1, B, Tout, O, s.scratch, w.bn1, training, &s.m1, &s.i1, f1, nred, defer1));
         void* h1 = X.alloc((size_t)B * (Tout + 2) * O * es);
-        if (!X.dry) L_(timed(X, "bn_apply", 0, (double)B * Tout * O * es * 2, stream, [&] { return ss_bn_apply(dt, c1, s.m1, s.i1, w.bn1.gamma, w.bn1.beta, 0, nullptr, nullptr, nullptr, nullptr, nullptr, 0, h1, 1, B, Tout, O, 1, stream); }));
+        if (!X.dry && defer1) L_(timed(X, "bn_apply", 0, (double)B * Tout * O * es * 2, stream, [&] { return ss_bn_apply_sums(dt, c1, f1, w.bn1.rmean, w.bn1.gamma, w.bn1.beta, 0, nullptr, nullptr, nullptr, nullptr, nullptr, 0, (double)B * Tout, 1e-5f, s.m1, s.i1, nullptr, nullptr, h1, 1, B, Tout, O, 1, stream); }));
+        else if (!X.dry) L_(timed(X, "bn_apply", 0, (double)B * Tout * O * es * 2, stream, [&] { return ss_bn_apply(dt, c1, s.m1, s.i1, w.bn1.gamma, w.bn1.beta, 0, nullptr, nullptr, nullptr, nullptr, nullptr, 0, h1, 1, B, Tout, O, 1, stream); }));
         void* c2 = X.alloc((size_t)rows * O * es);
         float* f2 = conv_gemm(X, h1, w.w2f, c2, rows, O, 3 * O, RM(O, Tout, (long long)(Tout + 2) * O), RM(3 * O), w.b2, w.bn2, slot ? slot + 4 * d : nullptr, &rc); L_(rc);
-        L_(bn_stats(X, c2, B, Tout, O, s.scratch, w.bn2, training, &s.m2, &s.i2, f2));
-        L_(bn_stats(X, cr, B, Tout, O, s.scratch, w.bnr, training, &s.mr, &s.ir, fr, nred));
+        const bool defer_y = defer2 && f2 && fr;
+        L_(bn_stats(X, c2, B, Tout, O, s.scratch, w.bn2, training, &s.m2, &s.i2, f2, 0.0, defer_y));
+        L_(bn_stats(X, cr, B, Tout, O, s.scratch, w.bnr, training, &s.mr, &s.ir, fr, nred, defer_y));
         const int pad_y = i == 2 ? 0 : 1;
         void* y = X.alloc((size_t)B * (Tout + 2 * pad_y) * O * es);
-        if (!X.dry) L_(timed(X, "bn_apply", 0, (double)B * Tout * O * es * 3, stream, [&] { return ss_bn_apply(dt, c2, s.m2, s.i2, w.bn2.gamma, w.bn2.beta, 0, cr, s.mr, s.ir, w.bnr.gamma, w.bnr.beta, 0, y, pad_y, B, Tout, O, 1, stream); }));
+        if (!X.dry && defer_y) L_(timed(X, "bn_apply", 0, (double)B * Tout * O * es * 3, stream, [&] { return ss_bn_apply_sums(dt, c2, f2, w.bn2.rmean, w.bn2.gamma, w.bn2.beta, 0, cr, fr, w.bnr.rmean, w.bnr.gamma, w.bnr.beta, 0, (double)B * Tout, 1e-5f, s.m2, s.i2, s.mr, s.ir, y, pad_y, B, Tout, O, 1, stream); }));
+        else if (!X.dry) L_(timed(X, "bn_apply", 0, (double)B * Tout * O * es * 3, stream, [&] { return ss_bn_apply(dt, c2, s.m2, s.i2, w.bn2.gamma, w.bn2.beta, 0, cr, s.mr, s.ir, w.bnr.gamma, w.bnr.beta, 0, y, pad_y, B, Tout, O, 1, stream); }));
         s.c1 = c1; s.cr = cr; s.h1 = h1; s.c2 = c2; s.y = y; s.pad_y = pad_y;
         xin = y; Tin = Tout; Cin = O;
     }
     if (training && !X.dry) {
         long long* ctrs[9];
         for (int i = 0; i < 3; ++i) { ctrs[3 * i] = blk[i].bn1.nbt; ctrs[3 * i + 1] = blk[i].bn2.nbt; ctrs[3 * i + 2] = blk[i].bnr.nbt; }
-        L_(timed(X, "counters", 0, 0, stream, [&] { return ss_counters_add(9, (int64_t**)ctrs, 1, stream); }));
+        if (n_bn_upd) L_(timed(X, "bn_running", 0, 0, stream, [&] { return ss_bn_update_running(n_bn_upd, bn_upd, 0.1f, 9, (int64_t**)ctrs, 1, stream); }));
+        else L_(timed(X, "counters", 0, 0, stream, [&] { return ss_counters_add(9, (int64_t**)ctrs, 1, stream); }));
     }
     const int T = Tin, M = B * T;
     c->T = T; c->M = M; c->conv_out = xin;
@@ -436,7 +448,8 @@
     const void* dh_t = dhead;
     if (dt != SS_F32) { void* t = X.alloc((size_t)M * nh * es); if (!X.dry) L_(timed(X, "cast", 0, (double)M * nh * (4 + es), stream, [&] { return ss_cast_f32(dhead, t, dt, (long long)M * nh, stream); })); dh_t = t; }
     if (!X.dry && stage_arena && stage_arena_bytes > 0) {
-        if (!ss_memset_async(stage_arena, 0, (size_t)stage_arena_bytes, stream)) { ss_set_error("backward: memset failed"); return 1; }
+        fork(X);
+        if (!ss_memset_async(stage_arena, 0, (size_t)stage_arena_bytes, side)) { ss_set_error("backward: memset failed"); return 1; }
     }
     const int old_blocks = ss_gemm_set_blocks_per_cu(overlapped ? side_blocks : 2);
     struct Restore { int v; ~Restore() { ss_gemm_set_blocks_per_cu(v); } } restore{old_blocks};
diff --git a/silent_speech_amd/csrc/runtime.hip b/silent_speech_amd/csrc/runtime.hip
--- a/silent_speech_amd/csrc/runtime.hip
+++ b/silent_speech_amd/csrc/runtime.hip
@@ -96,24 +96,63 @@
     const void* in; void* out;
     long long s0, s1, s2, o0, o1;
     int d0, d1, d2, valid1, valid2, in_dtype, out_dtype, accumulate;
-    float scale; int first_block, nblocks, pad_;
+    float scale; int first_block, nblocks, out2_dtype;
+    void* out2; long long q0, q1, q2;
 };
 
 template <class TI> struct Vec4;
 template <> struct Vec4<float> { static __device__ __forceinline__ void load(const float* p, float (&v)[4]) { const f32x4 a = *(const f32x4*)p; v[0] = a[0]; v[1] = a[1]; v[2] = a[2]; v[3] = a[3]; } };
 template <> struct Vec4<bf16_t> { static __device__ __forceinline__ void load(const bf16_t* p, float (&v)[4]) { const u32x2 a = *(const u32x2*)p; v[0] = __uint_as_float(a[0] << 16); v[1] = __uint_as_float(a[0] & 0xffff0000u); v[2] = __uint_as_float(a[1] << 16); v[3] = __uint_as_float(a[1] & 0xffff0000u); } };
 
-template <class TI, class TO, bool GROUPED_RMW = false>
+template <class TI, class TO, bool GROUPED_RMW = false, bool TWO = false>
 __device__ __forceinline__ void permute_job(const PermuteJob& j, int lb, int nthreads, int tid, float* tile)
 {
     const long long total = (long long)j.d0 * j.d1 * j.d2;
     const TI* in = (const TI*)j.in; TO* out = (TO*)j.out;
+    TO* out2 = TWO ? (TO*)j.out2 : nullptr;
     const long long as0 = j.s0 < 0 ? -j.s0 : j.s0, as1 = j.s1 < 0 ? -j.s1 : j.s1, as2 = j.s2 < 0 ? -j.s2 : j.s2;
     const bool c0 = j.d0 > 1 && as0 >= 1 && as0 <= 4, c1 = j.d1 > 1 && as1 >= 1 && as1 <= 4;
     const bool fx1 = c1 && (!c0 || j.d1 >= j.d0), fx0 = c0 && !fx1;
     const int dXq = fx1 ? j.d1 : j.d0;
-    const bool al16 = ((uintptr_t)in % 16) == 0 && ((uintptr_t)out % 16) == 0;
-    if (!GROUPED_RMW && !j.accumulate && j.s2 == 1 && j.s1 == j.d2 && j.o1 == j.d2 && (j.d0 == 1 || (j.s0 == (long long)j.d1 * j.d2 && j.o0 == j.s0)) &&
+    const bool al16 = ((uintptr_t)in % 16) == 0 && ((uintptr_t)out % 16) == 0 && ((uintptr_t)out2 % 16) == 0;
+    if (TWO && out2 && sizeof(TO) == 2 && !j.accumulate && j.s2 == 1 && j.q1 == 1 && nthreads == 256 && al16 && !((j.d1 | j.d2) & 7) &&
+        !((j.s0 | j.s1 | j.o0 | j.o1 | j.q0 | j.q2) & 7) && j.valid1 >= j.d1 && j.valid2 >= j.d2) {
+        unsigned short* t16 = (unsigned short*)tile;
+        const int tiles_b = (j.d1 + 63) >> 6, tiles_c = (j.d2 + 63) >> 6;
+        const long long ntiles = (long long)j.d0 * tiles_b * tiles_c;
+        for (long long t = lb; t < ntiles; t += j.nblocks) {
+            const int a = (int)(t / (tiles_b * tiles_c)), rem = (int)(t - (long long)a * (tiles_b * tiles_c));
+            const int tb = rem / tiles_c, tc = rem - tb * tiles_c;
+#pragma unroll
+            for (int k = 0; k < 2; ++k) {
+                const int f = k * 256 + tid, bb = f >> 3, c0 = (f & 7) * 8, gb = tb * 64 + bb, gc = tc * 64 + c0;
+                u32x4 r = {0u, 0u, 0u, 0u};
+                if (gb < j.d1 && gc < j.d2) {
+                    float v[8]; Vec8<TI>::load(in + a * j.s0 + gb * j.s1 + gc, v);
+#pragma unroll
+                    for (int e = 0; e < 4; ++e) r[e] = pack_bf16(v[2 * e] * j.scale, v[2 * e + 1] * j.scale);
+                    *(u32x4*)(out + a * j.o0 + gb * j.o1 + gc) = r;
+                }
+                unsigned* d = (unsigned*)(t16 + bb * 66 + c0);
+#pragma unroll
+                for (int e = 0; e < 4; ++e) d[e] = r[e];
+            }
+            __syncthreads();
+#pragma unroll
+            for (int k = 0; k < 2; ++k) {
+                const int f = k * 256 + tid, x = f >> 3, b0 = (f & 7) * 8, gc = tc * 64 + x, gb = tb * 64 + b0;
+                if (gc < j.d2 && gb < j.d1) {
+                    u32x4 r;
+#pragma unroll
+                    for (int e = 0; e < 4; ++e) r[e] = (unsigned)t16[(b0 + 2 * e) * 66 + x] | ((unsigned)t16[(b0 + 2 * e + 1) * 66 + x] << 16);
+                    *(u32x4*)(out2 + a * j.q0 + gb + (long long)gc * j.q2) = r;
+                }
+            }
+            __syncthreads();
+        }
+        return;
+    }
+    if (!GROUPED_RMW && !out2 && !j.accumulate && j.s2 == 1 && j.s1 == j.d2 && j.o1 == j.d2 && (j.d0 == 1 || (j.s0 == (long long)j.d1 * j.d2 && j.o0 == j.s0)) &&
         j.valid1 >= j.d1 && j.valid2 >= j.d2 && (total & 7) == 0 && al16 && total < (1LL << 34)) {
         const unsigned n8 = (unsigned)(total >> 3), step = (unsigned)j.nblocks * nthreads;
         for (unsigned i = (unsigned)lb * nthreads + tid; i < n8; i += step) {
@@ -128,7 +167,9 @@
         const int dX = fx1 ? j.d1 : j.d0, dO = fx1 ? j.d0 : j.d1;
         const long long sX = fx1 ? j.s1 : j.s0, sO = fx1 ? j.s0 : j.s1, oX = fx1 ? j.o1 : j.o0, oO = fx1 ? j.o0 : j.o1;
         const int vX = fx1 ? (j.valid1 < j.d1 ? j.valid1 : j.d1) : dX, vO = fx1 ? dO : (j.valid1 < j.d1 ? j.valid1 : j.d1), vC = j.valid2 < j.d2 ? j.valid2 : j.d2;
-        if (sX == 1 && !(dX & 7) && !(j.d2 & 7) && !(sO & 7) && !(j.s2 & 7) && !(oX & 7) && !(oO & 7) && !(vX & 7) && !(vC & 7) && dX >= 64 && j.d2 >= 64) {
+        const long long qX = fx1 ? j.q1 : j.q0, qO = fx1 ? j.q0 : j.q1;
+        if (sX == 1 && !(dX & 7) && !(j.d2 & 7) && !(sO & 7) && !(j.s2 & 7) && !(oX & 7) && !(oO & 7) && !(vX & 7) && !(vC & 7) && dX >= 64 && j.d2 >= 64 &&
+            (!out2 || (qX == 1 && !(qO & 7) && !(j.q2 & 7)))) {
             unsigned short* t16 = (unsigned short*)tile;
             const int tiles_x = (dX + 63) >> 6, tiles_c = (j.d2 + 63) >> 6;
             const long long ntiles = (long long)dO * tiles_x * tiles_c;
@@ -143,8 +184,10 @@
 #pragma unroll
                         for (int e = 0; e < 8; ++e) v[e] *= j.scale; }
                     unsigned* d = (unsigned*)(t16 + cc * 66 + x0);
-#pragma unroll
-                    for (int e = 0; e < 4; ++e) d[e] = pack_bf16(v[2 * e], v[2 * e + 1]);
+                    u32x4 r;
+#pragma unroll
+                    for (int e = 0; e < 4; ++e) d[e] = r[e] = pack_bf16(v[2 * e], v[2 * e + 1]);
+                    if (TWO && out2 && gx < dX && gc < j.d2) *(u32x4*)(out2 + oi * qO + gx + (long long)gc * j.q2) = r;
                 }
                 __syncthreads();
 #pragma unroll
@@ -162,7 +205,7 @@
             return;
         }
     }
-    if (sizeof(TI) == 4 && sizeof(TO) == 4 && as2 >= 4 && (fx0 || fx1) && nthreads == 256 && al16) {
+    if (!TWO && sizeof(TI) == 4 && sizeof(TO) == 4 && as2 >= 4 && (fx0 || fx1) && nthreads == 256 && al16) {
         const int dX = fx1 ? j.d1 : j.d0, dO = fx1 ? j.d0 : j.d1;
         const long long sX = fx1 ? j.s1 : j.s0, sO = fx1 ? j.s0 : j.s1, oX = fx1 ? j.o1 : j.o0, oO = fx1 ? j.o0 : j.o1;
         const int vX = fx1 ? (j.valid1 < j.d1 ? j.valid1 : j.d1) : dX, vO = fx1 ? dO : (j.valid1 < j.d1 ? j.valid1 : j.d1), vC = j.valid2 < j.d2 ? j.valid2 : j.d2;
@@ -211,6 +254,7 @@
     if (as2 > 4 && (fx0 || fx1) && nthreads == 256 && total >= 4096 && (long long)(dXq < 64 ? dXq : 64) * (j.d2 < 64 ? j.d2 : 64) >= 192) {
         const int dX = fx1 ? j.d1 : j.d0, dO = fx1 ? j.d0 : j.d1;
         const long long sX = fx1 ? j.s1 : j.s0, sO = fx1 ? j.s0 : j.s1, oX = fx1 ? j.o1 : j.o0, oO = fx1 ? j.o0 : j.o1;
+        const long long qX = fx1 ? j.q1 : j.q0, qO = fx1 ? j.q0 : j.q1;
         const int lx = dX <= 4 ? 2 : (dX <= 16 ? 4 : (j.d2 <= 4 ? 10 : (j.d2 <= 16 ? 8 : 6)));
         const int TX = 1 << lx, lc = 12 - lx, TC = 1 << lc, P = TX + 1;
         const int tiles_x = (dX + TX - 1) >> lx, tiles_c = (j.d2 + TC - 1) >> lc;
@@ -226,6 +270,7 @@
                     const int gx = tx * TX + x, gc = tc * TC + cc, bb = fx1 ? gx : oi;
                     v[k] = 0.f;
                     if (gx < dX && gc < j.d2 && bb < j.valid1 && gc < j.valid2) v[k] = ldf(in + oi * sO + gx * sX + (long long)gc * j.s2) * j.scale;
+                    if (TWO && out2 && gx < dX && gc < j.d2) stf(out2 + oi * qO + gx * qX + (long long)gc * j.q2, v[k]);
                 }
 #pragma unroll
                 for (int k = 0; k < 16; ++k) { const int f = k * 256 + tid; tile[(f >> lx) * P + (f & (TX - 1))] = v[k]; }
@@ -266,7 +311,7 @@
         }
         return;
     }
-    if (j.s2 == 1 && !(j.d2 & 3) && !(j.s0 & 3) && !(j.s1 & 3) && !(j.o0 & 3) && !(j.o1 & 3) && !(j.valid2 & 3) &&
+    if (!out2 && j.s2 == 1 && !(j.d2 & 3) && !(j.s0 & 3) && !(j.s1 & 3) && !(j.o0 & 3) && !(j.o1 & 3) && !(j.valid2 & 3) &&
         ((uintptr_t)in % (4 * sizeof(TI))) == 0 && ((uintptr_t)out % (4 * sizeof(TO))) == 0) {
         const int c4n = j.d2 >> 2;
         for (long long i = (long long)lb * nthreads + tid; i < (total >> 2); i += (long long)j.nblocks * nthreads) {
@@ -284,6 +329,7 @@
         const int c = (int)(i % j.d2); const long long t = i / j.d2; const int b = (int)(t % j.d1); const int a = (int)(t / j.d1);
         float v = (b < j.valid1 && c < j.valid2) ? ldf(in + a * j.s0 + b * j.s1 + c * j.s2) * j.scale : 0.f;
         TO* o = out + a * j.o0 + b * j.o1 + c;
+        if (TWO && out2) stf(out2 + a * j.q0 + b * j.q1 + c * j.q2, v);
         if (j.accumulate) v += ldf(o);
         stf(o, v);
     }
@@ -307,12 +353,25 @@
     permute_job<float, float, true>(j, blockIdx.x - j.first_block, blockDim.x, threadIdx.x, tile);
 }
 
+__global__ __launch_bounds__(256) void permute3d_batch_kernel_two(const PermuteJob* __restrict__ jobs, const int* __restrict__ job_of_block)
+{
+    __shared__ float tile[1024 * 5];
+    const PermuteJob j = jobs[job_of_block[blockIdx.x]];
+    const int lb = blockIdx.x - j.first_block;
+    if (j.in_dtype == SS_F32 && j.out_dtype == SS_F32) permute_job<float, float, false, true>(j, lb, blockDim.x, threadIdx.x, tile);
+    else if (j.in_dtype == SS_F32) permute_job<float, bf16_t, false, true>(j, lb, blockDim.x, threadIdx.x, tile);
+    else if (j.out_dtype == SS_F32) permute_job<bf16_t, float, false, true>(j, lb, blockDim.x, threadIdx.x, tile);
+    else permute_job<bf16_t, bf16_t, false, true>(j, lb, blockDim.x, threadIdx.x, tile);
+}
+
 extern "C" int ss_permute3d_batch(const void* jobs_dev, const int32_t* job_of_block_dev, int total_blocks, int all_f32, void* stream)
 {
     SS_CHECK(total_blocks >= 0, "ss_permute3d_batch: negative block count");
     if (total_blocks == 0) return 0;
     SS_CHECK(jobs_dev && job_of_block_dev, "ss_permute3d_batch: null pointer");
-    if (all_f32) SS_LAUNCH(permute3d_batch_f32_kernel, dim3(total_blocks), dim3(256), 0, stream, (const PermuteJob*)jobs_dev, (const int*)job_of_block_dev);
+    SS_CHECK(all_f32 >= 0 && all_f32 <= 2, "ss_permute3d_batch: bad kernel selector %d", all_f32);
+    if (all_f32 == 2) SS_LAUNCH(permute3d_batch_kernel_two, dim3(total_blocks), dim3(256), 0, stream, (const PermuteJob*)jobs_dev, (const int*)job_of_block_dev);
+    else if (all_f32) SS_LAUNCH(permute3d_batch_f32_kernel, dim3(total_blocks), dim3(256), 0, stream, (const PermuteJob*)jobs_dev, (const int*)job_of_block_dev);
     else SS_LAUNCH(permute3d_batch_kernel, dim3(total_blocks), dim3(256), 0, stream, (const PermuteJob*)jobs_dev, (const int*)job_of_block_dev);
     SS_LAUNCH_CHECK("ss_permute3d_batch");
     return 0;
diff --git a/silent_speech_amd/engine.py b/silent_speech_amd/engine.py
--- a/silent_speech_amd/engine.py
+++ b/silent_speech_amd/engine.py
@@ -30,20 +30,23 @@
     def build(self, model):
         dt, dev = model.compute_dtype, model.w_out.weight.device
         d = model.d_model
-        b1, b2 = ops.PermuteBatch(), ops.PermuteBatch()
-        self.b1, self.b2, self.dev = b1, b2, dev
+        b1 = ops.PermuteBatch()
+        self.b1, self.dev = b1, dev
 
         def new(*shape, dtype=dt, zero=False):
             return (torch.zeros if zero else torch.empty)(*shape, dtype=dtype, device=dev)
 
-        def cast(w):
+        def cast_t(w, out=None, outT=None, ldT=None):
             w = w.detach()
+            n, k = w.shape[-2], w.shape[-1]
+            outT = new(k, n) if outT is None else outT
+            ldT = n if ldT is None else ldT
             if dt == torch.float32:
-                return w
-            return b1.add(w, new(*w.shape), (1, w.shape[0], w.shape[1]), (0, w.shape[1], 1))
-
-        def transposed(src, n, k):
-            return b2.add(src, new(k, n), (k, 1, n), (1, 0, k))
+                b1.add(w, outT, (k, 1, n), (1, 0, k), out_strides=(ldT, ldT))
+                return (w if out is None else b1.add(w, out, (1, n, k), (0, k, 1))), outT
+            out = new(n, k) if out is None else out
+            b1.add(w, out, (1, n, k), (0, k, 1), out2=outT, out2_strides=(0, 1, ldT))
+            return out, outT
 
         self.blocks = []
         for blk in model.conv_blocks:
@@ -52,29 +55,26 @@
             w1, w2 = blk.conv1.weight.detach(), blk.conv2.weight.detach()
             e['w1f'] = b1.add(w1, new(O, 3 * I), (O, 3, I), (3 * I, 1, 3))
             e['w2f'] = b1.add(w2, new(O, 3 * O), (O, 3, O), (3 * O, 1, 3))
-            e['wr'] = b1.add(blk.residual_path.weight.detach(), new(O, I), (O, 1, I), (I, 0, 1))
-            e['wrT'] = transposed(e['wr'], O, I)
+            e['wr'], e['wrT'] = cast_t(blk.residual_path.weight.view(O, I), out=new(O, I))
             e['w2b'] = b1.add(w2.view(-1)[2:], new(O, 3 * O), (O, 3, O), (3, -1, 3 * O))
             if I % 8 == 0:
                 e['w1b_even'] = b1.add(w1.view(-1)[1:], new(I, O), (I, 1, O), (3, 0, 3 * I))
                 e['w1b_odd'] = b1.add(w1.view(-1)[2:], new(I, 2 * O), (I, 2, O), (3, -2, 3 * I))
             self.blocks.append(e)
 
-        self.w_raw_in = cast(model.w_raw_in.weight)
-        self.w_raw_in_T = transposed(self.w_raw_in, d, d)
+        self.w_raw_in, self.w_raw_in_T = cast_t(model.w_raw_in.weight)
         H, dh, dp, D = model.n_head, model.d_qkv, model.dp, model.max_rel
         MPt = _round_up(2 * D - 1, 32)
         self.layers = []
         for layer in model.transformer.layers:
             a = layer.self_attn
             e = {}
-            wqkv = new(3, H, dp, d)
+            wqkv, wqkvT = new(3, H, dp, d), new(d, 3 * H * dp)
             for i, w in enumerate((a.w_q, a.w_k, a.w_v)):
-                b1.add(w.detach(), wqkv[i], (H, dp, d), (d * dh, 1, dh), valid1=dh)
-            e['wqkv'] = wqkv.view(3 * H * dp, d)
-            e['wqkvT'] = transposed(e['wqkv'], 3 * H * dp, d)
-            e['wo'] = b1.add(a.w_o.detach(), new(d, H * dp), (d, H, dp), (1, dh * d, d), valid2=dh)
-            e['woT'] = transposed(e['wo'], d, H * dp)
+                b1.add(w.detach(), wqkv[i], (H, dp, d), (d * dh, 1, dh), valid1=dh, out2=wqkvT[:, i * H * dp:], out2_strides=(dp, 1, 3 * H * dp))
+            e['wqkv'], e['wqkvT'] = wqkv.view(3 * H * dp, d), wqkvT
+            e['woT'] = new(H * dp, d)
+            e['wo'] = b1.add(a.w_o.detach(), new(d, H * dp), (d, H, dp), (1, dh * d, d), valid2=dh, out2=e['woT'], out2_strides=(1, dp * d, d))
             emb = a.relative_positional.embeddings.detach()
             e['E'] = b1.add(emb, new(H, 2 * D - 1, dp), (H, 2 * D - 1, dp), ((2 * D - 1) * dh, dh, 1), valid2=dh)
             e['ET'] = b1.add(emb, new(H, dp, MPt), (H, dp, MPt), ((2 * D - 1) * dh, 1, dh), valid1=dh, valid2=2 * D - 1)
@@ -82,29 +82,27 @@
             e['EF.x3'] = dt != torch.bfloat16 and nb > 0
             e['EF'] = new(max(nb // 2, 8), dtype=torch.bfloat16)
             e['EF.src'], e['EF.version'], e['EF.scale'] = a.relative_positional.embeddings, None, 1.0 / math.sqrt(dh)
-            e['w1'] = cast(layer.linear1.weight)
-            e['w2'] = cast(layer.linear2.weight)
-            e['w1T'] = transposed(e['w1'], layer.linear1.weight.shape[0], d)
-            e['w2T'] = transposed(e['w2'], d, layer.linear2.weight.shape[1])
+            e['w1'], e['w1T'] = cast_t(layer.linear1.weight)
+            e['w2'], e['w2T'] = cast_t(layer.linear2.weight)
             self.layers.append(e)
         n_out = model.w_out.weight.shape[0]
         n_aux = model.w_aux.weight.shape[0] if model.has_aux_out else 0
         nh = _round_up(n_out + n_aux, 8)
         wh = new(nh, d, zero=True)
         bh = new(nh, dtype=torch.float32, zero=True)
-        b1.add(model.w_out.weight.detach(), wh[:n_out], (1, n_out, d), (0, d, 1))
+        whT = new(d, nh, zero=True)
+        cast_t(model.w_out.weight, out=wh[:n_out], outT=whT, ldT=nh)
         b1.add(model.w_out.bias.detach(), bh[:n_out], (1, 1, n_out), (0, 0, 1))
         if n_aux:
-            b1.add(model.w_aux.weight.detach(), wh[n_out:n_out + n_aux], (1, n_aux, d), (0, d, 1))
+            cast_t(model.w_aux.weight, out=wh[n_out:n_out + n_aux], outT=whT[:, n_out:], ldT=nh)
             b1.add(model.w_aux.bias.detach(), bh[n_out:n_out + n_aux], (1, 1, n_aux), (0, 0, 1))
         self.w_head, self.b_head, self.n_head_cols = wh, bh, nh
-        self.w_head_T = transposed(wh, nh, d)
+        self.w_head_T = whT
         self.layout_sig = self.layout_signature(model)
         self.refresh(model)
 
     def refresh(self, model):
         self.b1.run(self.dev)
-        self.b2.run(self.dev)
         for e in self.layers:
             src = e['EF.src']
             if e['EF'].numel() > 8 and e['EF.version'] != (src._version, src.data_ptr()):
diff --git a/silent_speech_amd/ops.py b/silent_speech_amd/ops.py
--- a/silent_speech_amd/ops.py
+++ b/silent_speech_amd/ops.py
@@ -224,6 +224,26 @@
     return y
 
 
+def bn_apply_sums(xa, sa, pad_xa, y, pad_y, B, T, C, relu, n_total, xb=None, sb=None, pad_xb=0, eps=1e-5):
+    b4 = sb if sb is not None else [None] * 4
+    new = lambda: torch.empty(C, dtype=torch.float32, device=xa.device)
+    ma, ia = new(), new()
+    mb, ib = (new(), new()) if xb is not None else (None, None)
+    rc = _L().ss_bn_apply_sums(_dt(xa), _p(xa), _p(sa[0]), _p(sa[1]), _p(sa[2]), _p(sa[3]), pad_xa, _p(xb), _p(b4[0]), _p(b4[1]), _p(b4[2]), _p(b4[3]), pad_xb,
+                               float(n_total), eps, _p(ma), _p(ia), _p(mb), _p(ib), _p(y), pad_y, B, T, C, int(relu), _s(xa))
+    _lib.check(rc, 'ss_bn_apply_sums')
+    return (ma, ia), (mb, ib)
+
+
+def bn_update_running(entries, counters=(), momentum=0.1, delta=1):
+    arr = (_lib.BnRunning * max(len(entries), 1))()
+    for i, (sums, rm, rv, n) in enumerate(entries):
+        arr[i].sums, arr[i].running_mean, arr[i].running_var, arr[i].C, arr[i].n_total = _p(sums).value, _p(rm).value, _p(rv).value, rm.numel(), float(n)
+    ctr = (ctypes.c_void_p * max(len(counters), 1))(*[_p(c).value for c in counters])
+    ref = entries[0][1] if entries else counters[0]
+    _lib.check(_L().ss_bn_update_running(len(entries), arr, momentum, len(counters), ctr, delta, _s(ref)), 'ss_bn_update_running')
+
+
 def bn_backward(dy, pad_dy, y, pad_y, xa, pad_xa, sa, dxa, pad_dxa, dgamma_a, dbeta_a, scratch, B, T, C, relu,
                 xb=None, pad_xb=0, sb=None, dxb=None, pad_dxb=0, dgamma_b=None, dbeta_b=None, reduce_fn=None, beta_a=None, beta_b=None):
     b3 = sb if sb is not None else [None] * 3
@@ -375,7 +395,7 @@
     def __init__(self):
         self.jobs, self.keep, self._dev = [], [], None
 
-    def add(self, inp, out, dims, strides, valid1=None, valid2=None, scale=1.0, accumulate=False, out_strides=None):
+    def add(self, inp, out, dims, strides, valid1=None, valid2=None, scale=1.0, accumulate=False, out_strides=None, out2=None, out2_strides=None):
         d0, d1, d2 = dims
         if out_strides is None:
             assert out.is_contiguous() and out.numel() >= d0 * d1 * d2
@@ -388,10 +408,14 @@
         j.valid1 = d1 if valid1 is None else valid1
         j.valid2 = d2 if valid2 is None else valid2
         j.in_dtype, j.out_dtype, j.accumulate, j.scale = _dt(inp), _dt(out), int(accumulate), float(scale)
+        if out2 is not None:
+            assert not accumulate and out2.dtype == out.dtype and out2.device == out.device and len(out2_strides) == 3
+            j.out2, j.out2_dtype = _p(out2).value, _dt(out2)
+            j.q0, j.q1, j.q2 = [int(x) for x in out2_strides]
         total = d0 * d1 * d2
         j.nblocks = max(1, min(2048, (total + 4095) // 4096))
         self.jobs.append(j)
-        self.keep.append((inp, out))
+        self.keep.append((inp, out, out2))
         self._dev = None
         return out
 
@@ -417,7 +441,7 @@
         if self._dev is None or self._dev[0].device != device:
             self._finalize(device)
         jobs, jb, total = self._dev
-        all_f32 = int(all(j.in_dtype == 0 and j.out_dtype == 0 for j in self.jobs))
-        nbytes = sum(j.d0 * j.d1 * j.d2 * ((4 if j.in_dtype == 0 else 2) + (4 if j.out_dtype == 0 else 2)) for j in self.jobs)
+        all_f32 = 2 if any(j.out2 for j in self.jobs) else int(all(j.in_dtype == 0 and j.out_dtype == 0 for j in self.jobs))
+        nbytes = sum(j.d0 * j.d1 * j.d2 * ((4 if j.in_dtype == 0 else 2) + (4 if j.out_dtype == 0 else 2) * (2 if j.out2 else 1)) for j in self.jobs)
         timed('permute3d_batch (weight re-layout)', 0, nbytes,
               lambda: _lib.check(_L().ss_permute3d_batch(_p(jobs), _p(jb), total, all_f32, _s(jobs)), 'ss_permute3d_batch'))
```

Result: no change. 1.700 million, median of 6 (+0.3%).
